# javad-jahangiri-iau/Detecting_Cyber_Attacks_with_Distilled_Large_Language_Models_in_Distributed_Networks

Measured on AMD Instinct MI355X. Metric: batches/sec/client (DistilBERT seq128 bs32) + aggregated F1 after 1 FedAvg round, 1/2/4/8 MI355X, higher is better.
Workload: dtype bf16; 1 GPU; model=DistilBERT-base (6 layers) + Linear(768,2) DDoSClassifier, global_batch=32, seq_len=128, parallelism=fedavg1 (1 client/GPU)

## Files before the change

### csrc/binding.cpp

```cpp
#ifdef FD_HOST_VALIDATION
#include <ATen/ATen.h>
typedef struct ihipStream_t* hipStream_t;
namespace py { struct gil_scoped_release {}; }
#else
#include <torch/extension.h>
#include <c10/hip/HIPStream.h>
#include <hip/hip_runtime.h>
#endif

#include <cmath>
#include <cstdint>
#include <vector>

#include "kernels/adam_epi.h"

extern "C" {
int fd_gemm(int kind, int epi, const void* A, const void* B, void* C, int M, int N, int K, int lda, int ldb,
            int ldc, const float* bias, void* aux, int ldaux, const void* res, int ldres, float* workspace,
            long long workspace_elems, int accumulate, const FdAdamEpi* adam,
            float* colsum, int* colsum_blocks, hipStream_t st);
int fd_gemm_ex(int kind, int epi, const void* A, const void* B, void* C, int M, int N, int K, int lda, int ldb,
               int ldc, const float* bias, void* aux, int ldaux, const void* res, int ldres, float* workspace,
               long long workspace_elems, int accumulate, const FdAdamEpi* adam,
               float* colsum, int* colsum_blocks, void* aux_out, hipStream_t st);
int fd_gemm_set_cfg(int kind, int cfg, int splits);
int fd_gemm_pf(const void* pf, long long bytes);
int fd_gemm_stamps(unsigned long long* host, int nblocks);
int fd_attn_stamps(unsigned long long* host, int nblocks);
int fd_attn_set_split(int on);
int fd_gemm_dw2(const void* A0, const void* B0, float* C0, int M0, int N0, const void* A1, const void* B1, float* C1,
                int M1, int N1, int K, float* workspace, long long workspace_elems, int accumulate,
                const FdAdamEpi* adams, int defer, int* splits_out, hipStream_t st);
int fd_gemm_dw2_splits(int M0, int N0, int M1, int N1, int K);
int fd_gemm_dw_batch(int n, const FdDwProb* probs, int K, const int* step, const float* hyper, int cfg,
                     const FdAdamRest* rest, hipStream_t st);
int fd_gemm_ln_set_diag(int diag);
int fd_gemm_dwb_set_mix(int mode);
long long fd_gemm_dwb_mixed_launches();
int fd_gemm_splitk(int epi, const void* A, const void* Bt, int M, int N, int K, float* workspace,
                   long long workspace_elems, int splits, const float* bias, void* C, void* aux, void* aux_out,
                   const void* res, float* colsum, int* colsum_blocks, const FdLnEpi* ln, const FdSkHead* hd,
                   int b_mn, hipStream_t st);
int fd_gemm_ln(int bwd, const void* A, const void* Bt, void* C, int M, int N, int K, const float* bias,
               const void* res, int ldres, const FdLnEpi* ln, int cfg, int b_mn, hipStream_t st);
int fd_splitk_reduce_batched(int n, const float* const* slabs, float* const* outs, const long long* numel,
                             const int* splits, const int* accumulate, hipStream_t st);

const char* fd_comm_last_error();
int fd_comm_load(const char* path);
int fd_comm_unique_id_bytes();
int fd_comm_get_unique_id(void* out);
int fd_comm_init(void** comm, int nranks, int rank, const void* id_bytes);
int fd_comm_destroy(void* comm);
int fd_comm_async_error(void* comm);
int fd_comm_wait(void* comm, hipStream_t st, long long timeout_ms);
int fd_comm_abort(void* comm);
int fd_comm_allreduce(void* comm, const void* send, void* recv, long long count, int dtype, int op, hipStream_t st);
int fd_comm_broadcast(void* comm, void* buf, long long count, int dtype, int root, hipStream_t st);
int fd_comm_allgather(void* comm, const void* send, void* recv, long long count, int dtype, hipStream_t st);
int fd_gemm_attn_fwd(const void* x, const void* w, const float* bias, void* qkv, int M, int K, const float* kbias,
                     void* ctx, float* lse, int B, int S, int H, const uint32_t* seed_ptr, uint32_t site, uint32_t thr,
                     float drop_scale, const int* cu, int rows, uint64_t* dmask, int q_live, void* cxc, void* xc,
                     const void* xres, int Bp, uint64_t* flags, int nflags, const int* cnt, int xsite, int* err,
                     int mode, int split, hipStream_t st);
int fd_attn_bwd_proj(const void* qkv, const float* kbias, const void* ctx, const float* lse, const void* dy,
                     const void* w, int M, int K, int splits, void* dqkv, int B, int S, int H,
                     const uint32_t* seed_ptr, uint32_t site, uint32_t thr, float drop_scale, const int* cu, int rows,
                     const uint64_t* dmask, const void* dresc, void* dres, int split, hipStream_t st);
int fd_attn_fwd(const void* qkv, const float* kbias, void* ctx, float* lse, int B, int S, int H,
                const uint32_t* seed_ptr, uint32_t site, uint32_t thr, float drop_scale, const int* cu,
                int rows, uint64_t* dmask, int q_live, void* cxc, void* xc, const void* xres, int Bp,
                int split, hipStream_t st);
int fd_attn_bwd(const void* qkv, const float* kbias, const void* ctx, const float* lse, const void* dctx,
                float* delta, void* dqkv, int B, int S, int H, const uint32_t* seed_ptr, uint32_t site,
                uint32_t thr, float drop_scale, const int* cu, int rows, const uint64_t* dmask, int q_live,
                const void* dresc, void* dres, int split, hipStream_t st);
int fd_mask_to_bias(const void* mask, int mask_bytes, float* bias, long n, hipStream_t st);
int fd_ln_fwd(const void* x, const void* r, const float* gamma, const float* beta, void* y, float* mean,
              float* rstd, int T, int D, float eps, const uint32_t* seed_ptr, uint32_t site, uint32_t thr,
              float dscale, const int* row_map, hipStream_t st);
int fd_ln_bwd(const void* dy, const void* x, const void* r, const float* gamma, const float* mean,
              const float* rstd, void* dz, void* dx, float* dgamma, float* dbeta, float* dbias, float* work, int T,
              int D, const uint32_t* seed_ptr, uint32_t site, uint32_t thr, float dscale, int accumulate,
              const int* row_map, int defer, int* nblk_out, int zin, hipStream_t st);
int fd_emb_fwd(const void* ids, int ids64, const void* word, const void* pos, const float* gamma,
               const float* beta, void* y, float* mean, float* rstd, int T, int S, int D, float eps,
               const uint32_t* seed_ptr, uint32_t site, uint32_t thr, float dscale, const int* row_map, int* ln_epoch,
               unsigned long long* ln_stats, long long ln_stats_n, long long* sorted, long long* perm, hipStream_t st);
int fd_emb_bwd(const void* dy, const void* ids, int ids64, const long long* sorted, const long long* perm,
               const void* word, const void* pos, const float* gamma, const float* mean, const float* rstd,
               float* dword, float* dpos, float* dgamma, float* dbeta, float* dz_buf, float* work, int T, int S,
               int B, int P, int V, int D, const uint32_t* seed_ptr, uint32_t site, uint32_t thr, float dscale,
               int accumulate, unsigned char* now, unsigned char* ever, const int* row_map, const int* cu, int ncs, const float* const* cs_parts, float* const* cs_outs, const int* cs_nblk,
               const int* cs_stride, const int* cs_D, const int* cs_nout, const int* cs_acc, hipStream_t st);
int fd_gather_rows2(const void* a, const void* b, void* oa, void* ob, const long long* idx, int n, int d_bytes,
                    hipStream_t st);
int fd_scatter_rows2(const void* a, const void* b, void* oa, void* ob, const long long* idx, int nsrc, int T,
                     int d_bytes, hipStream_t st);
int fd_pack(const void* mask, int mask_bytes, const void* ids, int ids_bytes, int B, int S, int rows, int* row_map,
            int* cu, long long* ids_packed, int* step, uint32_t* seed, long long* cls_rows, int* cls_rmap,
            hipStream_t st);
int fd_colsum_bf16_batched(int n, const void* const* xs, const int* T, const int* N, float* const* parts,
                           hipStream_t st);
int fd_colsum_bf16(const void* x, int T, int N, float* out, float* work, int accumulate, int defer, int* nblk_out,
                   hipStream_t st);
int fd_colsum_batched(int n, const float* const* parts, float* const* outs, const int* nblk, const int* stride,
                      const int* D, const int* nout, const int* accumulate, hipStream_t st);
int fd_rank_sort(const void* ids, int ids64, int T, long long* sorted, long long* perm, hipStream_t st);
int fd_head_fwd(const void* hidden, int B, int S, int D, const float* W, const float* bias,
                const uint32_t* seed_ptr, uint32_t site, uint32_t thr, float dscale, const long long* labels,
                float* logits, float* loss, float* dlogits, float* row_loss, const int* cls, int T,
                const float* tlogits, float kd_T, float kd_alpha, float* loss_acc, hipStream_t st);
int fd_head_bwd(const void* hidden, int B, int S, int D, const float* W, const uint32_t* seed_ptr, uint32_t site,
                uint32_t thr, float dscale, const float* dlogits, float* dW, float* db, void* dhidden,
                int accumulate, const int* cls, int T, const float* gscale, const int* own, hipStream_t st);
int fd_head_ln_bwd(const void* hidden, int B, int T, int D, const float* W, const float* bias,
                   const uint32_t* seed_ptr, uint32_t hsite, uint32_t hthr, float hdscale, const long long* labels,
                   float* logits, float* loss, float* dlogits, float* row_loss, float* loss_acc, float* dW, float* db,
                   int accumulate, const int* own, const float* tlogits, float kd_T, float kd_alpha, const void* z,
                   const float* gamma, const float* mean, const float* rstd, void* dz, void* dx, float* part,
                   uint32_t site, uint32_t thr, float dscale, const int* row_map, int* nblk_out, hipStream_t st);
int fd_eval_metrics(const float* logits, const long long* labels, int B, double* acc, long long* counts,
                    float* prob1, long long* preds, hipStream_t st);
int fd_adam(float* p, const float* g, float* m, float* v, void* shadow, long long n, const int* step, float lr,
            float b1, float b2, float eps, float wd, int decoupled, const unsigned char* touched,
            const unsigned char* now, long long skip_off, long long skip_rows, int row_len, const long long* runs,
            int nruns, long long run_total4, const float* run_wd, hipStream_t st);
int fd_adam_rows(float* p, const float* g, float* m, float* v, void* shadow, int rows, int row_len, const int* step,
                 float lr, float b1, float b2, float eps, const unsigned char* ever, const unsigned char* now,
                 float wd, int decoupled, hipStream_t st);
int fd_adam_lazy_decay(float* p, void* shadow, int* done, const unsigned char* ever, int rows, int row_len,
                       const int* step, int adj, float lr, float wd, const void* ids, int ids64, long long n,
                       hipStream_t st);
int fd_step(int* step, uint32_t* seed, hipStream_t st);
int fd_scale_cast(float* p, void* shadow, long long n, float scale, hipStream_t st);
int fd_axpby(float* dst, const float* x, const float* y, float a, float b, long long n, hipStream_t st);
}

namespace {

#ifdef FD_HOST_VALIDATION
hipStream_t stream() { return nullptr; }
bool on_device(const at::Tensor&) { return true; }
#else
hipStream_t stream() { return c10::hip::getCurrentHIPStream().stream(); }
bool on_device(const at::Tensor& t) { return t.is_cuda(); }
#endif

void check_rc(int rc, const char* what) { TORCH_CHECK(rc == 0, what, ": kernel launcher rejected arguments (rc=", rc, ")"); }

void need(const at::Tensor& t, at::ScalarType dt, const char* name) {
  TORCH_CHECK(on_device(t), name, " must be a GPU tensor");
  TORCH_CHECK(t.scalar_type() == dt, name, " has dtype ", t.scalar_type(), ", expected ", dt);
  TORCH_CHECK(t.is_contiguous(), name, " must be contiguous");
}
void need_opt(const c10::optional<at::Tensor>& t, at::ScalarType dt, const char* name) {
  if (t.has_value() && t->defined()) need(*t, dt, name);
}
template <typename T>
T* ptr(const c10::optional<at::Tensor>& t) {
  return (t.has_value() && t->defined()) ? reinterpret_cast<T*>(t->data_ptr()) : nullptr;
}
const uint32_t* seedp(const at::Tensor& s) {
  TORCH_CHECK(on_device(s) && s.scalar_type() == at::kInt && s.numel() >= 1, "seed must be a GPU int32 tensor");
  return reinterpret_cast<const uint32_t*>(s.data_ptr());
}

void set_prefetch(const c10::optional<at::Tensor>& prefetch, const at::Tensor& like) {
  if (prefetch.has_value() && prefetch->defined() && prefetch->numel() > 0) {
    TORCH_CHECK(prefetch->device() == like.device() && prefetch->is_contiguous(),
                "prefetch must be a contiguous tensor on the GEMM's device");
    fd_gemm_pf(prefetch->data_ptr(), (long long)(prefetch->numel() * prefetch->element_size()));
  } else {
    fd_gemm_pf(nullptr, 0);
  }
}

void gemm(int64_t kind, int64_t epi, const at::Tensor& A, const at::Tensor& B, const at::Tensor& C,
          const c10::optional<at::Tensor>& bias, const c10::optional<at::Tensor>& aux,
          const c10::optional<at::Tensor>& res, const c10::optional<at::Tensor>& workspace, bool accumulate,
          const c10::optional<at::Tensor>& aux_out, const c10::optional<at::Tensor>& prefetch = c10::nullopt) {
  need(A, at::kBFloat16, "A");
  need(B, at::kBFloat16, "B");
  TORCH_CHECK(A.dim() == 2 && B.dim() == 2 && C.dim() == 2, "gemm operands must be 2-D");
  int64_t M, N, K;
  if (kind == 0) { M = A.size(0); K = A.size(1); N = B.size(0); TORCH_CHECK(B.size(1) == K, "NT: K mismatch"); }
  else if (kind == 1) { M = A.size(0); K = A.size(1); N = B.size(1); TORCH_CHECK(B.size(0) == K, "NN: K mismatch"); }
  else if (kind == 2) { K = A.size(0); M = A.size(1); N = B.size(1); TORCH_CHECK(B.size(0) == K, "TN: K mismatch"); }
  else TORCH_CHECK(false, "bad gemm kind");
  TORCH_CHECK(C.size(0) == M && C.size(1) == N, "C shape mismatch: got ", C.sizes(), " want [", M, ",", N, "]");
  TORCH_CHECK(K % 64 == 0, "gemm: K must be a multiple of 64, got ", K);
  TORCH_CHECK(N % 64 == 0, "gemm: N must be a multiple of 64, got ", N);
  if (kind == 2) {
    need(C, at::kFloat, "C");
    TORCH_CHECK(M % 128 == 0, "TN gemm: M must be a multiple of 128");
  } else {
    need(C, at::kBFloat16, "C");
  }
  need_opt(bias, at::kFloat, "bias");
  need_opt(aux, at::kBFloat16, "aux");
  need_opt(res, at::kBFloat16, "res");
  need_opt(workspace, at::kFloat, "workspace");
  if (epi == 1 || epi == 2) TORCH_CHECK(bias.has_value() && bias->numel() == N, "bias of size N required");
  if (epi == 3 || (epi == 2 && aux.has_value() && aux->defined()))
    TORCH_CHECK(aux.has_value() && aux->size(0) == M && aux->size(1) == N, "aux [M,N] required");
  if (epi == 4) TORCH_CHECK(res.has_value() && res->size(0) == M && res->size(1) == N, "res [M,N] required");
  need_opt(aux_out, at::kBFloat16, "aux_out");
  if (aux_out.has_value() && aux_out->defined())
    TORCH_CHECK(epi == 3 && kind != 2 && aux_out->size(0) == M && aux_out->size(1) == N,
                "aux_out [M,N] only with the GELU' epilogue");
  const long long ws = (workspace.has_value() && workspace->defined()) ? workspace->numel() : 0;
  set_prefetch(prefetch, A);
  check_rc(fd_gemm_ex((int)kind, (int)epi, A.data_ptr(), B.data_ptr(), C.data_ptr(), (int)M, (int)N, (int)K,
                      (int)A.size(1), (int)B.size(1), (int)N, ptr<float>(bias), ptr<void>(aux), (int)N,
                      ptr<void>(res), (int)N, ptr<float>(workspace), ws, accumulate ? 1 : 0, nullptr, nullptr,
                      nullptr, ptr<void>(aux_out), stream()),
           "gemm");
}

int64_t gemm_colsum(int64_t epi, const at::Tensor& A, const at::Tensor& B, const at::Tensor& C,
                    const c10::optional<at::Tensor>& aux, const c10::optional<at::Tensor>& res,
                    const at::Tensor& colsum, const c10::optional<at::Tensor>& aux_out, int64_t kind = 0,
                    const c10::optional<at::Tensor>& prefetch = c10::nullopt) {
  need(A, at::kBFloat16, "A");
  need(B, at::kBFloat16, "B");
  need(C, at::kBFloat16, "C");
  need(colsum, at::kFloat, "colsum");
  TORCH_CHECK(A.dim() == 2 && B.dim() == 2 && C.dim() == 2, "gemm_colsum operands must be 2-D");
  TORCH_CHECK(kind == 0 || kind == 1, "gemm_colsum: kind 0 (NT) or 1 (NN)");
  const int64_t M = A.size(0), K = A.size(1), N = kind == 0 ? B.size(0) : B.size(1);
  TORCH_CHECK((kind == 0 ? B.size(1) : B.size(0)) == K && C.size(0) == M && C.size(1) == N,
              "gemm_colsum: shape mismatch");
  TORCH_CHECK(K % 64 == 0 && N % 64 == 0, "gemm_colsum: K % 64 and N % 64 required");
  TORCH_CHECK(epi == 3 || epi == 4, "gemm_colsum: GELU' (3) or residual (4) epilogue");
  need_opt(aux, at::kBFloat16, "aux");
  need_opt(res, at::kBFloat16, "res");
  if (epi == 3) TORCH_CHECK(aux.has_value() && aux->size(0) == M && aux->size(1) == N, "aux [M,N] required");
  if (epi == 4) TORCH_CHECK(res.has_value() && res->size(0) == M && res->size(1) == N, "res [M,N] required");
  TORCH_CHECK(colsum.numel() >= ((M + 127) / 128) * N, "gemm_colsum: colsum needs ceil(M/128) x N floats");
  need_opt(aux_out, at::kBFloat16, "aux_out");
  if (aux_out.has_value() && aux_out->defined())
    TORCH_CHECK(epi == 3 && aux_out->size(0) == M && aux_out->size(1) == N, "aux_out [M,N] only with GELU'");
  int blocks = 0;
  set_prefetch(prefetch, A);
  check_rc(fd_gemm_ex((int)kind, (int)epi, A.data_ptr(), B.data_ptr(), C.data_ptr(), (int)M, (int)N, (int)K,
                      (int)K, (int)B.size(1), (int)N, nullptr, ptr<void>(aux), (int)N, ptr<void>(res), (int)N,
                      nullptr, 0, 0, nullptr, colsum.data_ptr<float>(), &blocks, ptr<void>(aux_out), stream()),
           "gemm_colsum");
  return blocks;
}

void adam_descs(const std::vector<at::Tensor>& st, const std::vector<double>& hp, const at::Tensor* const* grads,
                int nprob, FdAdamEpi* out) {
  TORCH_CHECK((int)st.size() == 4 * nprob + 1, "fused adam: expected ", 4 * nprob + 1, " state tensors");
// ... 288 lines not shown
                                 const c10::optional<at::Tensor>& gamma, const c10::optional<at::Tensor>& beta,
                                 const c10::optional<at::Tensor>& mean, const c10::optional<at::Tensor>& rstd,
                                 const c10::optional<at::Tensor>& z, const c10::optional<at::Tensor>& dx,
                                 const c10::optional<at::Tensor>& colpart, double eps,
                                 const c10::optional<at::Tensor>& seed, int64_t site, int64_t thr, double dscale,
                                 const c10::optional<at::Tensor>& row_map, bool b_mn = false,
                                 const std::vector<at::Tensor>& head = {}, const std::vector<double>& head_f = {},
                                 const c10::optional<at::Tensor>& head_dx = c10::nullopt,
                                 const c10::optional<at::Tensor>& head_tlogits = c10::nullopt,
                                 const c10::optional<at::Tensor>& head_own = c10::nullopt) {
  need(A, at::kBFloat16, "A");
  need(Bt, at::kBFloat16, "Bt");
  need(C, at::kBFloat16, "C");
  need(workspace, at::kFloat, "workspace");
  TORCH_CHECK(A.dim() == 2 && Bt.dim() == 2 && C.dim() == 2, "gemm_splitk operands must be 2-D");
  const int64_t M = A.size(0), K = A.size(1), N = b_mn ? Bt.size(1) : Bt.size(0);
  TORCH_CHECK(M > 0 && (b_mn ? Bt.size(0) : Bt.size(1)) == K && C.size(0) == M && C.size(1) == N,
              "gemm_splitk: shape mismatch");
  TORCH_CHECK(K % 64 == 0 && N % 64 == 0, "gemm_splitk: K % 64 and N % 64 required");
  TORCH_CHECK(epi >= 0 && epi <= 7 && epi != 5, "gemm_splitk: epilogue code");
  for (const auto* t : {&aux, &aux_out, &res, &z, &dx}) {
    need_opt(*t, at::kBFloat16, "gemm_splitk bf16 operand");
    if (t->has_value() && (*t)->defined())
      TORCH_CHECK((*t)->dim() == 2 && (*t)->size(0) == M && (*t)->size(1) == N, "gemm_splitk: [M, N] operand");
  }
  for (const auto* t : {&bias, &gamma, &beta}) {
    need_opt(*t, at::kFloat, "gemm_splitk fp32 vector");
    if (t->has_value() && (*t)->defined()) TORCH_CHECK((*t)->numel() == N, "gemm_splitk: vector of size N");
  }
  need_opt(mean, at::kFloat, "mean");
  need_opt(rstd, at::kFloat, "rstd");
  need_opt(colsum, at::kFloat, "colsum");
  need_opt(colpart, at::kFloat, "colpart");
  need_opt(row_map, at::kInt, "row_map");
  auto has = [](const c10::optional<at::Tensor>& t) { return t.has_value() && t->defined(); };
  if (epi == 1 || epi == 2 || epi == 6) TORCH_CHECK(has(bias), "gemm_splitk: bias required");
  if (epi == 2 || epi == 3) TORCH_CHECK(has(aux), "gemm_splitk: aux [M, N] required");
  if (epi == 4 || epi >= 6) TORCH_CHECK(has(res), "gemm_splitk: res [M, N] required");
  if (has(colsum)) {
    TORCH_CHECK(epi == 3 || epi == 4, "gemm_splitk: column sums only with the GELU' / residual epilogues");
    TORCH_CHECK(colsum->numel() >= ((M + 31) / 32) * N, "gemm_splitk: colsum needs ceil(M/32) x N floats");
  }
  FdLnEpi ln{};
  if (epi >= 6) {
    TORCH_CHECK(has(gamma) && has(mean) && has(rstd) && mean->numel() >= M && rstd->numel() >= M,
                "gemm_splitk LayerNorm: gamma, mean / rstd of M entries required");
    if (epi == 6) TORCH_CHECK(has(beta), "gemm_splitk LayerNorm forward: beta required");
    if (epi == 7) {
      TORCH_CHECK(has(z), "gemm_splitk LayerNorm backward: z required");
      TORCH_CHECK(has(colpart) && colpart->numel() >= M * 3 * N, "gemm_splitk LayerNorm backward: colpart M x 3N");
      if (thr) TORCH_CHECK(has(dx), "gemm_splitk LayerNorm backward with dropout: dx required");
    }
    ln.gamma = gamma->data_ptr<float>();
    ln.beta = ptr<float>(beta);
    ln.mean = mean->data_ptr<float>();
    ln.rstd = rstd->data_ptr<float>();
    ln.z = ptr<uint16_t>(z);
    ln.dx = ptr<uint16_t>(dx);
    ln.colpart = ptr<float>(colpart);
    ln.eps = (float)eps;
    ln.thr = (uint32_t)thr;
    ln.site = (uint32_t)site;
    ln.dscale = (float)dscale;
    if (thr) {
      TORCH_CHECK(seed.has_value() && seed->defined(), "gemm_splitk: dropout needs the seed tensor");
      ln.seed_ptr = seedp(*seed);
      ln.row_map = ptr<int>(row_map);
      if (has(row_map)) TORCH_CHECK(row_map->numel() >= M, "gemm_splitk: row_map needs M entries");
    }
  }
  FdSkHead hd{};
  if (!head.empty()) {
    TORCH_CHECK(epi == 6 && N == 768 && head.size() == 13 && head_f.size() == 6, "gemm_splitk head: arguments");
    need(head[11], at::kFloat, "head loss");
    need(head[12], at::kInt, "head ticket");
    TORCH_CHECK(head[11].numel() == 1 && head[12].numel() == 1, "gemm_splitk head: loss / ticket [1]");
    const int64_t Bh = (int64_t)head_f[5];
    TORCH_CHECK(Bh > 0 && Bh <= M, "gemm_splitk head: B");
    need(head[0], at::kFloat, "head W");
    need(head[1], at::kFloat, "head bias");
    need(head[2], at::kLong, "head labels");
    for (int k : {3, 4, 6, 7, 8, 9}) need(head[k], at::kFloat, "head fp32 output");
    need(head[5], at::kBFloat16, "head dz");
    TORCH_CHECK(head[0].numel() == 2 * N && head[1].numel() == 2 && head[2].numel() == Bh &&
                    head[3].numel() == 2 * Bh && head[4].numel() == 2 * Bh && head[5].numel() == M * N &&
                    head[6].numel() >= M * 3 * N && head[7].numel() >= M * 2 * N && head[8].numel() >= M * 2 &&
                    head[9].numel() >= M,
                "gemm_splitk head: sizes");
    need_opt(head_dx, at::kBFloat16, "head dx");
    need_opt(head_tlogits, at::kFloat, "head teacher logits");
    need_opt(head_own, at::kInt, "head own");
    if (thr) TORCH_CHECK(head_dx.has_value() && head_dx->defined() && head_dx->numel() == M * N, "gemm_splitk head: dx");
    if (head_tlogits.has_value() && head_tlogits->defined())
      TORCH_CHECK(head_tlogits->numel() == 2 * Bh && head_f[3] > 0.0, "gemm_splitk head: teacher logits [B, 2], T > 0");
    if (head_own.has_value() && head_own->defined()) TORCH_CHECK(head_own->numel() == Bh + 1, "gemm_splitk head: own");
    hd.W = head[0].data_ptr<float>();
    hd.bias = head[1].data_ptr<float>();
    hd.labels = reinterpret_cast<const long long*>(head[2].data_ptr());
    hd.logits = head[3].data_ptr<float>();
    hd.dlogits = head[4].data_ptr<float>();
    hd.dz = reinterpret_cast<uint16_t*>(head[5].data_ptr());
    hd.colpart = head[6].data_ptr<float>();
    hd.hpart = head[7].data_ptr<float>();
    hd.dbpart = head[8].data_ptr<float>();
    hd.lpart = head[9].data_ptr<float>();
    hd.seed_ptr = seedp(head[10]);
    hd.loss = head[11].data_ptr<float>();
    hd.ticket = reinterpret_cast<unsigned*>(head[12].data_ptr<int>());
    hd.site = (uint32_t)head_f[0];
    hd.thr = (uint32_t)head_f[1];
    hd.dscale = (float)head_f[2];
    hd.kd_T = (float)head_f[3];
    hd.kd_alpha = (float)head_f[4];
    hd.B = (int)Bh;
    hd.dx = ptr<uint16_t>(head_dx);
    hd.tlogits = ptr<const float>(head_tlogits);
    hd.own = ptr<int>(head_own);
  }
  int blocks = 0;
  const int rc = fd_gemm_splitk((int)epi, A.data_ptr(), Bt.data_ptr(), (int)M, (int)N, (int)K,
                                workspace.data_ptr<float>(), workspace.numel(), (int)splits, ptr<float>(bias),
                                C.data_ptr(), ptr<void>(aux), ptr<void>(aux_out), ptr<void>(res), ptr<float>(colsum),
                                &blocks, epi >= 6 ? &ln : nullptr, head.empty() ? nullptr : &hd, b_mn ? 1 : 0,
                                stream());
  TORCH_CHECK(rc > 0, "gemm_splitk: launcher rejected arguments (rc=", rc, ")");
  return {rc, blocks};
}

void splitk_reduce_batched(const std::vector<at::Tensor>& slabs, const std::vector<at::Tensor>& outs,
                           const std::vector<int64_t>& splits, const std::vector<int64_t>& accumulate) {
  const size_t n = slabs.size();
  TORCH_CHECK(outs.size() == n && splits.size() == n && accumulate.size() == n, "splitk_reduce_batched: ragged");
  std::vector<const float*> sp(n);
  std::vector<float*> op(n);
  std::vector<long long> ne(n);
  std::vector<int> sl(n), ac(n);
  for (size_t i = 0; i < n; ++i) {
    need(slabs[i], at::kFloat, "slabs");
    need(outs[i], at::kFloat, "out");
    TORCH_CHECK(splits[i] >= 1 && outs[i].numel() % 4 == 0 && slabs[i].numel() >= splits[i] * outs[i].numel(),
                "splitk_reduce_batched: slab buffer smaller than splits x out");
    sp[i] = slabs[i].data_ptr<float>();
    op[i] = outs[i].data_ptr<float>();
    ne[i] = outs[i].numel();
    sl[i] = (int)splits[i];
    ac[i] = accumulate[i] ? 1 : 0;
  }
  if (n) check_rc(fd_splitk_reduce_batched((int)n, sp.data(), op.data(), ne.data(), sl.data(), ac.data(), stream()),
                  "splitk_reduce_batched");
}

void pack(const at::Tensor& mask, const at::Tensor& ids, const at::Tensor& row_map, const at::Tensor& cu,
          const at::Tensor& ids_packed, const c10::optional<at::Tensor>& step, const c10::optional<at::Tensor>& seed,
          const c10::optional<at::Tensor>& cls_rows, const c10::optional<at::Tensor>& cls_rmap) {
  need_opt(cls_rmap, at::kInt, "cls_rmap");
  need_opt(step, at::kInt, "step");
  need_opt(seed, at::kInt, "seed");
  need_opt(cls_rows, at::kLong, "cls_rows");
  TORCH_CHECK(on_device(mask) && mask.is_contiguous() && on_device(ids) && ids.is_contiguous(), "pack: GPU inputs");
  TORCH_CHECK(mask.dim() == 2 && ids.sizes() == mask.sizes(), "pack: mask and ids must both be [B, S]");
  need(row_map, at::kInt, "row_map");
  need(cu, at::kInt, "cu");
  need(ids_packed, at::kLong, "ids_packed");
  const int64_t B = mask.size(0), S = mask.size(1);
  TORCH_CHECK(cu.numel() == B + 1 && ids_packed.numel() == row_map.numel() && row_map.numel() >= 1, "pack: sizes");
  if (cls_rows.has_value() && cls_rows->defined()) TORCH_CHECK(cls_rows->numel() >= B, "pack: cls_rows needs B entries");
  if (cls_rmap.has_value() && cls_rmap->defined()) TORCH_CHECK(cls_rmap->numel() >= B, "pack: cls_rmap needs B entries");
  check_rc(fd_pack(mask.data_ptr(), (int)mask.element_size(), ids.data_ptr(), (int)ids.element_size(), (int)B, (int)S,
                   (int)row_map.numel(), row_map.data_ptr<int>(), cu.data_ptr<int>(),
                   reinterpret_cast<long long*>(ids_packed.data_ptr()), ptr<int>(step), ptr<uint32_t>(seed),
                   cls_rows.has_value() && cls_rows->defined() ? reinterpret_cast<long long*>(cls_rows->data_ptr())
                                                               : nullptr,
                   ptr<int>(cls_rmap), stream()),
           "pack");
}

void gather_rows2(const at::Tensor& a, const at::Tensor& b, const at::Tensor& oa, const at::Tensor& ob,
                  const at::Tensor& idx) {
  for (const at::Tensor* t : {&a, &b, &oa, &ob}) need(*t, at::kBFloat16, "gather_rows2 operand");
  need(idx, at::kLong, "idx");
  TORCH_CHECK(a.dim() == 2 && a.sizes() == b.sizes() && oa.dim() == 2 && oa.sizes() == ob.sizes() &&
                  oa.size(1) == a.size(1) && oa.size(0) == idx.numel(), "gather_rows2: shapes");
  TORCH_CHECK((a.size(1) * 2) % 16 == 0, "gather_rows2: rows must be 16-byte multiples");
  check_rc(fd_gather_rows2(a.data_ptr(), b.data_ptr(), oa.data_ptr(), ob.data_ptr(),
                           reinterpret_cast<const long long*>(idx.data_ptr()), (int)idx.numel(), (int)(a.size(1) * 2),
                           stream()), "gather_rows2");
}

void scatter_rows2(const at::Tensor& a, const at::Tensor& b, const at::Tensor& oa, const at::Tensor& ob,
                   const at::Tensor& idx, int64_t nsrc) {
  for (const at::Tensor* t : {&a, &b, &oa, &ob}) need(*t, at::kBFloat16, "scatter_rows2 operand");
  need(idx, at::kLong, "idx");
  TORCH_CHECK(a.dim() == 2 && a.sizes() == b.sizes() && oa.dim() == 2 && oa.sizes() == ob.sizes() &&
                  oa.size(1) == a.size(1) && nsrc >= 0 && nsrc <= a.size(0) && nsrc <= idx.numel(),
              "scatter_rows2: shapes");
  TORCH_CHECK((a.size(1) * 2) % 16 == 0, "scatter_rows2: rows must be 16-byte multiples");
  check_rc(fd_scatter_rows2(a.data_ptr(), b.data_ptr(), oa.data_ptr(), ob.data_ptr(),
                            reinterpret_cast<const long long*>(idx.data_ptr()), (int)nsrc, (int)oa.size(0),
                            (int)(a.size(1) * 2), stream()), "scatter_rows2");
}

int comm_dtype(const at::Tensor& t) {
  switch (t.scalar_type()) {
    case at::kFloat: return 0;
    case at::kBFloat16: return 1;
    case at::kDouble: return 2;
    case at::kLong: return 3;
    case at::kInt: return 4;
    default: TORCH_CHECK(false, "comm: unsupported dtype ", t.scalar_type());
  }
  return 0;
}
void comm_check(int rc, const char* what) { TORCH_CHECK(rc == 0, what, " failed: ", fd_comm_last_error()); }

void comm_load(const std::string& path) { comm_check(fd_comm_load(path.c_str()), "comm_load"); }

at::Tensor comm_unique_id() {
  at::Tensor id = at::empty({fd_comm_unique_id_bytes()}, at::TensorOptions().dtype(at::kByte));
  comm_check(fd_comm_get_unique_id(id.data_ptr()), "ncclGetUniqueId");
  return id;
}
int64_t comm_init(int64_t nranks, int64_t rank, const at::Tensor& id) {
  TORCH_CHECK(!id.is_cuda() && id.scalar_type() == at::kByte && id.numel() == fd_comm_unique_id_bytes(),
              "comm_init: id must be the CPU uint8 tensor from comm_unique_id()");
  TORCH_CHECK(rank >= 0 && rank < nranks, "comm_init: bad rank");
  void* c = nullptr;
  comm_check(fd_comm_init(&c, (int)nranks, (int)rank, id.contiguous().data_ptr()), "ncclCommInitRank");
  return reinterpret_cast<int64_t>(c);
}
void comm_destroy(int64_t h) { comm_check(fd_comm_destroy(reinterpret_cast<void*>(h)), "ncclCommDestroy"); }
void comm_abort(int64_t h) { comm_check(fd_comm_abort(reinterpret_cast<void*>(h)), "ncclCommAbort"); }
std::tuple<int64_t, std::string> comm_async_error(int64_t h) {
  const int rc = fd_comm_async_error(reinterpret_cast<void*>(h));
  return {rc, rc ? std::string(fd_comm_last_error()) : std::string()};
}
std::tuple<int64_t, std::string> comm_wait(int64_t h, int64_t timeout_ms) {
  TORCH_CHECK(h != 0, "comm_wait: communicator not initialised");
  const hipStream_t st = stream();
  int rc;
  {
    py::gil_scoped_release nogil;
    rc = fd_comm_wait(reinterpret_cast<void*>(h), st, (long long)timeout_ms);
  }
  return {rc, rc ? std::string(fd_comm_last_error()) : std::string()};
}
void comm_allreduce(int64_t h, const at::Tensor& t, int64_t op) {
  TORCH_CHECK(h != 0, "comm_allreduce: communicator not initialised");
  TORCH_CHECK(on_device(t) && t.is_contiguous(), "comm_allreduce: contiguous GPU tensor required");
  TORCH_CHECK(op >= 0 && op <= 2, "comm_allreduce: op must be 0 (sum), 1 (avg) or 2 (max)");
  comm_check(fd_comm_allreduce(reinterpret_cast<void*>(h), t.data_ptr(), t.data_ptr(), t.numel(), comm_dtype(t),
                               (int)op, stream()),
             "ncclAllReduce");
}
void comm_broadcast(int64_t h, const at::Tensor& t, int64_t root) {
  TORCH_CHECK(h != 0, "comm_broadcast: communicator not initialised");
  TORCH_CHECK(on_device(t) && t.is_contiguous(), "comm_broadcast: contiguous GPU tensor required");
  comm_check(fd_comm_broadcast(reinterpret_cast<void*>(h), t.data_ptr(), t.numel(), comm_dtype(t), (int)root,
                               stream()),
             "ncclBroadcast");
}
void comm_allgather(int64_t h, const at::Tensor& send, const at::Tensor& recv) {
  TORCH_CHECK(h != 0, "comm_allgather: communicator not initialised");
  TORCH_CHECK(on_device(send) && on_device(recv) && send.is_contiguous() && recv.is_contiguous(),
              "comm_allgather: contiguous GPU tensors required");
  TORCH_CHECK(send.scalar_type() == recv.scalar_type() && recv.numel() % send.numel() == 0,
              "comm_allgather: recv must hold nranks x send");
  comm_check(fd_comm_allgather(reinterpret_cast<void*>(h), send.data_ptr(), recv.data_ptr(), send.numel(),
                               comm_dtype(send), stream()),
             "ncclAllGather");
}


int64_t gemm_stamps(at::Tensor out) {
  TORCH_CHECK(!out.is_cuda() && out.scalar_type() == at::kLong && out.is_contiguous() && out.dim() == 2 &&
                  out.size(1) == 8, "gemm_stamps: CPU int64 [n][8]");
  return fd_gemm_stamps(reinterpret_cast<unsigned long long*>(out.data_ptr()), (int)out.size(0));
}

int64_t attn_stamps(at::Tensor out) {
  TORCH_CHECK(!out.is_cuda() && out.scalar_type() == at::kLong && out.is_contiguous() && out.dim() == 2 &&
                  out.size(1) == 8, "attn_stamps: CPU int64 [n][8]");
  return fd_attn_stamps(reinterpret_cast<unsigned long long*>(out.data_ptr()), (int)out.size(0));
}

void gemm_set_cfg(int64_t kind, int64_t cfg, int64_t splits) {
  check_rc(fd_gemm_set_cfg((int)kind, (int)cfg, (int)splits), "gemm_set_cfg");
}

void check_cu(const c10::optional<at::Tensor>& cu, int64_t B, int64_t rows_qkv, int64_t rows_ctx) {
  if (!(cu.has_value() && cu->defined())) return;
  need(*cu, at::kInt, "cu");
  TORCH_CHECK(cu->numel() == B + 1, "attention: cu must have B+1 entries");
  TORCH_CHECK(rows_qkv >= 1 && rows_qkv == rows_ctx, "attention: packed qkv/ctx row counts differ");
}

const int* map_ptr(const c10::optional<at::Tensor>& m, int64_t T) {
  if (!(m.has_value() && m->defined())) return nullptr;
  need(*m, at::kInt, "row_map");
  TORCH_CHECK(m->numel() == T, "row_map must have one entry per row");
  return m->data_ptr<int>();
}

void check_dmask(const c10::optional<at::Tensor>& dmask, int64_t B, int64_t S, int64_t H, int64_t split = -1) {
  if (!dmask.has_value() || !dmask->defined()) return;
  need(*dmask, at::kLong, "dmask");
  TORCH_CHECK((S <= 128 || split == 2) && dmask->numel() == B * H * 256,
              "attention: dmask needs S <= 128 (or split 2) and B*H*256 words");
}

void attn_fwd(const at::Tensor& qkv, const at::Tensor& kbias, const at::Tensor& ctx, const at::Tensor& lse,
              int64_t B, int64_t S, int64_t H, const at::Tensor& seed, int64_t site, int64_t thr, double dscale,
              const c10::optional<at::Tensor>& cu, const c10::optional<at::Tensor>& dmask, int64_t q_live = 0,
              const c10::optional<at::Tensor>& cxc = c10::nullopt, const c10::optional<at::Tensor>& xc = c10::nullopt,
              const c10::optional<at::Tensor>& xres = c10::nullopt, int64_t split = -1) {
  need(qkv, at::kBFloat16, "qkv");
  TORCH_CHECK(q_live >= 0, "attention: q_live >= 0");
  TORCH_CHECK(split >= -1 && split <= 2, "attention: split in -1..2");
  const bool compact = cxc.has_value() && cxc->defined();
  int64_t Bp = 0;
  if (compact) {
    TORCH_CHECK(q_live == 1 && xc.has_value() && xres.has_value(), "attention: compact rows need q_live 1, xc, xres");
    need(*cxc, at::kBFloat16, "cxc");
    need(*xc, at::kBFloat16, "xc");
    need(*xres, at::kBFloat16, "xres");
    Bp = cxc->numel() / (H * 64);
    TORCH_CHECK(Bp >= B && cxc->numel() == Bp * H * 64 && xc->numel() == cxc->numel(), "attention: cxc/xc size");
    TORCH_CHECK(xres->numel() == ctx.numel(), "attention: xres size");
// ... 599 lines not shown
    TORCH_CHECK(!(touched.has_value() && touched->defined()), "adam: per-run decay takes no row flags");
    need_decays(run_wd_host, (size_t)nruns, "adam run_wd");
    rwd = run_wd->data_ptr<float>();
  } else {
    TORCH_CHECK(run_wd_host.empty(), "adam: run_wd_host without run_wd");
  }
  if (touched.has_value() && touched->defined())
    TORCH_CHECK(wd == 0.0 || decoupled, "adam: row flags with weight decay need decoupled decay");
  check_rc(fd_adam(p.data_ptr<float>(), g.data_ptr<float>(), m.data_ptr<float>(), v.data_ptr<float>(),
                   ptr<void>(shadow), n, step.data_ptr<int>(), (float)lr, (float)b1, (float)b2, (float)eps, (float)wd,
                   decoupled ? 1 : 0, ptr<const unsigned char>(touched), ptr<const unsigned char>(now), skip_off,
                   skip_rows, (int)row_len, rp, nruns, total4, rwd, stream()),
           "adam");
}

void adam_rows(const at::Tensor& p, const at::Tensor& g, const at::Tensor& m, const at::Tensor& v,
               const c10::optional<at::Tensor>& shadow, const at::Tensor& step, double lr, double b1, double b2,
               double eps, const at::Tensor& ever, const c10::optional<at::Tensor>& now, int64_t row_len,
               double wd = 0.0, bool decoupled = false) {
  TORCH_CHECK(std::isfinite(wd) && wd >= 0.0, "adam_rows: weight decay must be finite and >= 0");
  TORCH_CHECK(wd == 0.0 || decoupled, "adam_rows: weight decay needs decoupled decay");
  need(p, at::kFloat, "p");
  need(g, at::kFloat, "g");
  need(m, at::kFloat, "m");
  need(v, at::kFloat, "v");
  need_opt(shadow, at::kBFloat16, "shadow");
  need(step, at::kInt, "step");
  need(ever, at::kByte, "ever");
  need_opt(now, at::kByte, "now");
  const int64_t n = p.numel();
  TORCH_CHECK(row_len > 0 && row_len % 4 == 0 && n % row_len == 0, "adam_rows: rows of row_len (multiple of 4)");
  const int64_t rows = n / row_len;
  TORCH_CHECK(g.numel() == n && m.numel() == n && v.numel() == n, "adam_rows: sizes");
  if (shadow.has_value() && shadow->defined()) TORCH_CHECK(shadow->numel() == n, "adam_rows: shadow size");
  TORCH_CHECK(ever.numel() >= rows, "adam_rows: ever flags");
  if (now.has_value() && now->defined()) TORCH_CHECK(now->numel() >= rows, "adam_rows: now flags");
  check_rc(fd_adam_rows(p.data_ptr<float>(), g.data_ptr<float>(), m.data_ptr<float>(), v.data_ptr<float>(),
                        ptr<void>(shadow), (int)rows, (int)row_len, step.data_ptr<int>(), (float)lr, (float)b1,
                        (float)b2, (float)eps, ever.data_ptr<unsigned char>(), ptr<const unsigned char>(now),
                        (float)wd, decoupled ? 1 : 0, stream()),
           "adam_rows");
}

void adam_lazy_decay(const at::Tensor& p, const c10::optional<at::Tensor>& shadow, const at::Tensor& done,
                     const at::Tensor& ever, const at::Tensor& step, int64_t adj, double lr, double wd,
                     int64_t row_len, const c10::optional<at::Tensor>& ids) {
  need(p, at::kFloat, "p");
  need_opt(shadow, at::kBFloat16, "shadow");
  need(done, at::kInt, "done");
  need(ever, at::kByte, "ever");
  need(step, at::kInt, "step");
  TORCH_CHECK(std::isfinite(wd) && wd >= 0.0 && std::isfinite(lr), "adam_lazy_decay: lr / weight decay");
  TORCH_CHECK(adj == 0 || adj == 1, "adam_lazy_decay: adj is 0 or 1");
  const int64_t n = p.numel();
  TORCH_CHECK(row_len > 0 && row_len % 4 == 0 && n > 0 && n % row_len == 0,
              "adam_lazy_decay: rows of row_len (multiple of 4)");
  const int64_t rows = n / row_len;
  TORCH_CHECK(rows < (int64_t(1) << 31), "adam_lazy_decay: too many rows");
  if (shadow.has_value() && shadow->defined()) TORCH_CHECK(shadow->numel() == n, "adam_lazy_decay: shadow size");
  TORCH_CHECK(done.numel() >= rows && ever.numel() >= rows && step.numel() >= 1, "adam_lazy_decay: flag sizes");
  const void* idp = nullptr;
  int ids64 = 0;
  int64_t nids = 0;
  if (ids.has_value() && ids->defined()) {
    TORCH_CHECK(ids->scalar_type() == at::kLong || ids->scalar_type() == at::kInt, "adam_lazy_decay: ids int32 / int64");
    need(*ids, ids->scalar_type(), "ids");
    nids = ids->numel();
    TORCH_CHECK(nids > 0 && nids <= (int64_t(1) << 30), "adam_lazy_decay: ids count");
    idp = ids->data_ptr();
    ids64 = ids->scalar_type() == at::kLong;
  }
  check_rc(fd_adam_lazy_decay(p.data_ptr<float>(), ptr<void>(shadow), done.data_ptr<int>(),
                              ever.data_ptr<unsigned char>(), (int)rows, (int)row_len, step.data_ptr<int>(), (int)adj,
                              (float)lr, (float)wd, idp, ids64, nids, stream()),
           "adam_lazy_decay");
}

void step_inc(const c10::optional<at::Tensor>& step, const c10::optional<at::Tensor>& seed) {
  need_opt(step, at::kInt, "step");
  need_opt(seed, at::kInt, "seed");
  check_rc(fd_step(ptr<int>(step), ptr<uint32_t>(seed), stream()), "step");
}

void scale_cast(const at::Tensor& p, const c10::optional<at::Tensor>& shadow, double scale) {
  need(p, at::kFloat, "p");
  need_opt(shadow, at::kBFloat16, "shadow");
  TORCH_CHECK(p.numel() % 4 == 0, "scale_cast: numel % 4");
  if (shadow.has_value() && shadow->defined()) TORCH_CHECK(shadow->numel() == p.numel(), "scale_cast: shadow size");
  check_rc(fd_scale_cast(p.data_ptr<float>(), ptr<void>(shadow), p.numel(), (float)scale, stream()), "scale_cast");
}

void axpby(const at::Tensor& dst, const at::Tensor& x, const c10::optional<at::Tensor>& y, double a, double b) {
  need(dst, at::kFloat, "dst");
  need(x, at::kFloat, "x");
  need_opt(y, at::kFloat, "y");
  TORCH_CHECK(dst.numel() == x.numel() && dst.numel() % 4 == 0, "axpby: sizes");
  if (y.has_value() && y->defined()) TORCH_CHECK(y->numel() == x.numel(), "axpby: y size");
  check_rc(fd_axpby(dst.data_ptr<float>(), x.data_ptr<float>(), ptr<const float>(y), (float)a, (float)b, dst.numel(),
                    stream()),
           "axpby");
}

}

#ifndef FD_HOST_VALIDATION
PYBIND11_MODULE(TORCH_EXTENSION_NAME, m) {
  m.doc() = "gfx950 HIP kernels for the federated DistilBERT engine";
  m.def("gemm", &gemm, py::arg("kind"), py::arg("epi"), py::arg("A"), py::arg("B"), py::arg("C"), py::arg("bias"),
        py::arg("aux"), py::arg("res"), py::arg("workspace"), py::arg("accumulate"), py::arg("aux_out") = py::none(),
        py::arg("prefetch") = py::none());
  m.def("gemm_set_cfg", &gemm_set_cfg);
  m.def("gemm_stamps", &gemm_stamps);
  m.def("attn_stamps", &attn_stamps);
  m.def("gemm_splitk", &gemm_splitk, py::arg("epi"), py::arg("A"), py::arg("Bt"), py::arg("C"), py::arg("workspace"),
        py::arg("splits") = 0, py::arg("bias") = py::none(), py::arg("aux") = py::none(),
        py::arg("aux_out") = py::none(), py::arg("res") = py::none(), py::arg("colsum") = py::none(),
        py::arg("gamma") = py::none(), py::arg("beta") = py::none(), py::arg("mean") = py::none(),
        py::arg("rstd") = py::none(), py::arg("z") = py::none(), py::arg("dx") = py::none(),
        py::arg("colpart") = py::none(), py::arg("eps") = 1e-12, py::arg("seed") = py::none(),
        py::arg("site") = 0, py::arg("thr") = 0, py::arg("dscale") = 1.0, py::arg("row_map") = py::none(),
        py::arg("b_mn") = false, py::arg("head") = std::vector<at::Tensor>{}, py::arg("head_f") = std::vector<double>{},
        py::arg("head_dx") = py::none(), py::arg("head_tlogits") = py::none(), py::arg("head_own") = py::none());
  m.def("gemm_dw2", &gemm_dw2);
  m.def("gemm_dw", &gemm_dw);
  m.def("adam_rows", &adam_rows, py::arg("p"), py::arg("g"), py::arg("m"), py::arg("v"), py::arg("shadow"),
        py::arg("step"), py::arg("lr"), py::arg("b1"), py::arg("b2"), py::arg("eps"), py::arg("ever"), py::arg("now"),
        py::arg("row_len"), py::arg("wd") = 0.0, py::arg("decoupled") = false);
  m.def("adam_lazy_decay", &adam_lazy_decay, py::arg("p"), py::arg("shadow"), py::arg("done"), py::arg("ever"),
        py::arg("step"), py::arg("adj"), py::arg("lr"), py::arg("wd"), py::arg("row_len"),
        py::arg("ids") = py::none());
  m.def("gemm_ln", &gemm_ln, py::arg("bwd"), py::arg("A"), py::arg("Bt"), py::arg("C"), py::arg("bias"),
        py::arg("res"), py::arg("gamma"), py::arg("beta"), py::arg("mean"), py::arg("rstd"), py::arg("z"),
        py::arg("dx"), py::arg("colpart"), py::arg("stats"), py::arg("cnt"), py::arg("err"), py::arg("eps"),
        py::arg("seed"), py::arg("site"), py::arg("thr"), py::arg("dscale"), py::arg("row_map"),
        py::arg("cfg") = -1, py::arg("xsite") = 0, py::arg("b_mn") = false, py::arg("xbuf") = py::none(),
        py::arg("prefetch") = py::none());
  m.def("gemm_dw_batch", &gemm_dw_batch, py::arg("As"), py::arg("Bs"), py::arg("Cs"), py::arg("accumulate"),
        py::arg("adam"), py::arg("hp"), py::arg("cfg") = -1,
        py::arg("biases") = std::vector<at::Tensor>{}, py::arg("rest") = std::vector<at::Tensor>{},
        py::arg("rest_i") = std::vector<int64_t>{}, py::arg("decay") = std::vector<double>{},
        py::arg("bias_decay") = std::vector<double>{}, py::arg("rest_wd") = py::none(),
        py::arg("rest_wd_host") = std::vector<double>{}, py::arg("word_wd") = 0.0);
  m.def("gemm_colsum", &gemm_colsum, py::arg("epi"), py::arg("A"), py::arg("B"), py::arg("C"), py::arg("aux"),
        py::arg("res"), py::arg("colsum"), py::arg("aux_out") = py::none(), py::arg("kind") = 0,
        py::arg("prefetch") = py::none());
  m.def("splitk_reduce_batched", &splitk_reduce_batched);
  m.def("gemm_dw2_splits", [](int64_t M0, int64_t N0, int64_t M1, int64_t N1, int64_t K) {
    return (int64_t)fd_gemm_dw2_splits((int)M0, (int)N0, (int)M1, (int)N1, (int)K);
  });
  m.def("gather_rows2", &gather_rows2);
  m.def("scatter_rows2", &scatter_rows2);
  m.def("pack", &pack, py::arg("mask"), py::arg("ids"), py::arg("row_map"), py::arg("cu"), py::arg("ids_packed"),
        py::arg("step") = py::none(), py::arg("seed") = py::none(), py::arg("cls_rows") = py::none(),
        py::arg("cls_rmap") = py::none());
  m.def("comm_load", &comm_load);
  m.def("comm_unique_id", &comm_unique_id);
  m.def("comm_init", &comm_init);
  m.def("comm_destroy", &comm_destroy);
  m.def("comm_abort", &comm_abort);
  m.def("comm_async_error", &comm_async_error);
  m.def("comm_wait", &comm_wait);
  m.def("comm_allreduce", &comm_allreduce);
  m.def("comm_broadcast", &comm_broadcast);
  m.def("comm_allgather", &comm_allgather);
  m.def("gemm_attn_fwd", &gemm_attn_fwd, py::arg("x"), py::arg("w"), py::arg("bias"), py::arg("qkv"),
        py::arg("kbias"), py::arg("ctx"), py::arg("lse"), py::arg("B"), py::arg("S"), py::arg("H"), py::arg("seed"),
        py::arg("site"), py::arg("thr"), py::arg("dscale"), py::arg("cu"), py::arg("dmask"), py::arg("q_live"),
        py::arg("stats"), py::arg("cnt"), py::arg("err"), py::arg("xsite"), py::arg("cxc") = py::none(),
        py::arg("xc") = py::none(), py::arg("xres") = py::none(), py::arg("prefetch") = py::none(),
        py::arg("mode") = 1, py::arg("split") = -1);
  m.def("attn_fwd", &attn_fwd, py::arg("qkv"), py::arg("kbias"), py::arg("ctx"), py::arg("lse"), py::arg("B"),
        py::arg("S"), py::arg("H"), py::arg("seed"), py::arg("site"), py::arg("thr"), py::arg("dscale"), py::arg("cu"),
        py::arg("dmask"), py::arg("q_live") = 0, py::arg("cxc") = py::none(), py::arg("xc") = py::none(),
        py::arg("xres") = py::none(), py::arg("split") = -1);
  m.def("attn_bwd", &attn_bwd, py::arg("qkv"), py::arg("kbias"), py::arg("ctx"), py::arg("lse"), py::arg("dctx"),
        py::arg("delta"), py::arg("dqkv"), py::arg("B"), py::arg("S"), py::arg("H"), py::arg("seed"), py::arg("site"),
        py::arg("thr"), py::arg("dscale"), py::arg("cu"), py::arg("dmask"), py::arg("q_live") = 0,
        py::arg("dresc") = py::none(), py::arg("dres") = py::none(), py::arg("split") = -1);
  m.def("attn_bwd_proj", &attn_bwd_proj, py::arg("qkv"), py::arg("kbias"), py::arg("ctx"), py::arg("lse"),
        py::arg("dy"), py::arg("w"), py::arg("dqkv"), py::arg("B"), py::arg("S"), py::arg("H"), py::arg("seed"),
        py::arg("site"), py::arg("thr"), py::arg("dscale"), py::arg("cu"), py::arg("dmask"), py::arg("splits") = 1,
        py::arg("dresc") = py::none(), py::arg("dres") = py::none(), py::arg("split") = -1);
  m.def("mask_to_bias", &mask_to_bias);
  m.def("attn_set_split", [](int64_t on) { return (int64_t)fd_attn_set_split((int)on); });
  m.def("ln_fwd", &ln_fwd);
  m.def("ln_bwd", &ln_bwd);
  m.def("emb_fwd", &emb_fwd, py::arg("ids"), py::arg("word"), py::arg("pos"), py::arg("gamma"), py::arg("beta"),
        py::arg("y"), py::arg("mean"), py::arg("rstd"), py::arg("S"), py::arg("eps"), py::arg("seed"), py::arg("site"),
        py::arg("thr"), py::arg("dscale"), py::arg("row_map") = py::none(), py::arg("ln_epoch") = py::none(),
        py::arg("sorted") = py::none(), py::arg("perm") = py::none(), py::arg("ln_stats") = py::none());
  m.def("gemm_ln_set_diag", [](int64_t d) { fd_gemm_ln_set_diag((int)d); });
  m.def("gemm_dwb_set_mix", [](int64_t mode) { return (int64_t)fd_gemm_dwb_set_mix((int)mode); },
        "all-layer dW launch schedule: 0 plain, 1 mixed tiles when shorter (default), 2 forced; returns the old mode");
  m.def("gemm_dwb_mixed_launches", []() { return (int64_t)fd_gemm_dwb_mixed_launches(); });
  m.def("emb_bwd", &emb_bwd);
  m.def("colsum_bf16", &colsum_bf16);
  m.def("colsum_bf16_batched", &colsum_bf16_batched);
  m.def("colsum_batched", &colsum_batched);
  m.def("rank_sort", &rank_sort);
  m.def("head_fwd", &head_fwd, py::arg("hidden"), py::arg("B"), py::arg("S"), py::arg("W"), py::arg("bias"),
        py::arg("seed"), py::arg("site"), py::arg("thr"), py::arg("dscale"), py::arg("labels"), py::arg("logits"),
        py::arg("loss"), py::arg("dlogits"), py::arg("row_loss"), py::arg("cls"), py::arg("tlogits") = py::none(),
        py::arg("kd_T") = 1.0, py::arg("kd_alpha") = 1.0, py::arg("loss_acc") = py::none());
  m.def("head_bwd", &head_bwd, py::arg("hidden"), py::arg("B"), py::arg("S"), py::arg("W"), py::arg("seed"),
        py::arg("site"), py::arg("thr"), py::arg("dscale"), py::arg("dlogits"), py::arg("dW"), py::arg("db"),
        py::arg("dhidden"), py::arg("accumulate"), py::arg("cls") = py::none(), py::arg("gscale") = py::none(),
        py::arg("own") = py::none());
  m.def("head_ln_bwd", &head_ln_bwd);
  m.def("eval_metrics", &eval_metrics);
  m.def("adam", &adam);
  m.def("step_inc", &step_inc);
  m.def("scale_cast", &scale_cast);
  m.def("axpby", &axpby);
}
#endif
```

### csrc/host_check/binding_host_check.cpp

```cpp
#define FD_HOST_VALIDATION 1
#include <algorithm>
#include "../binding.cpp"

#include <cstdio>
#include <cstdlib>
#include <string>
#include <vector>

namespace hc {
struct Region { uintptr_t lo, hi; };
std::vector<Region> regions;
std::vector<std::string> violations;
int calls = 0;

void reg(const at::Tensor& t) {
  const uintptr_t p = reinterpret_cast<uintptr_t>(t.data_ptr());
  regions.push_back({p, p + (uintptr_t)(t.numel() * t.element_size())});
}
void span(const void* p, long long bytes, const char* what) {
  if (bytes <= 0) return;
  if (!p) { violations.push_back(std::string("null ") + what); return; }
  const uintptr_t lo = reinterpret_cast<uintptr_t>(p), hi = lo + (uintptr_t)bytes;
  for (const Region& r : regions)
    if (lo >= r.lo && hi <= r.hi) return;
// ... 284 lines not shown
  const long long D = (long long)H * 64, N = 3 * D;
  hc::span(x, (long long)M * K * 2, "gemm_attn x");
  hc::span(w, N * K * 2, "gemm_attn w");
  hc::span(bias, N * 4, "gemm_attn bias");
  hc::span(qkv, (long long)M * N * 2, "gemm_attn qkv");
  const long long tiles = ((M + 127) / 128) * (N / 192);
  if (tiles > nflags) hc::violations.push_back("gemm_attn: more tiles than flags");
  hc::span(flags, tiles * 8, "gemm_attn flags");
  hc::span(cnt, 4, "gemm_attn cnt");
  hc::span(err, 4, "gemm_attn err");
  hc::opt_span(cxc, (long long)Bp * D * 2, "gemm_attn cxc");
  hc::opt_span(xc, (long long)Bp * D * 2, "gemm_attn xc");
  hc::opt_span(xres, rows * D * 2, "gemm_attn xres");
  hc::opt_span(dmask, (long long)B * H * 256 * 8, "gemm_attn dmask");
  hc::span(ctx, rows * D * 2, "gemm_attn ctx");
  hc::span(lse, (long long)B * H * S * 4, "gemm_attn lse");
  hc::span(seed, 4, "gemm_attn seed");
  if (cu) hc::span(cu, (long long)(B + 1) * 4, "gemm_attn cu");
  else hc::span(kbias, (long long)B * S * 4, "gemm_attn kbias");
  return 0;
}
int fd_attn_bwd_proj(const void* qkv, const float* kbias, const void* ctx, const float* lse, const void* dy,
                     const void* w, int M, int K, int, void* dqkv, int B, int S, int H, const uint32_t* seed,
                     uint32_t, uint32_t, float, const int* cu, int rows, const uint64_t* dmask, const void* dresc,
                     void* dres, int, hipStream_t) {
  ++hc::calls;
  const long long D = (long long)H * 64;
  hc::opt_span(dmask, (long long)B * H * 256 * 8, "attn bwd proj dmask");
  hc::span(qkv, rows * 3 * D * 2, "attn bwd proj qkv");
  hc::span(dqkv, rows * 3 * D * 2, "attn bwd proj dqkv");
  hc::span(ctx, rows * D * 2, "attn bwd proj ctx");
  hc::span(dy, (long long)M * K * 2, "attn bwd proj dy");
  hc::span(w, (long long)K * D * 2, "attn bwd proj w");
  hc::opt_span(dresc, (long long)M * D * 2, "attn bwd proj dresc");
  hc::opt_span(dres, rows * D * 2, "attn bwd proj dres");
  hc::span(lse, (long long)B * H * S * 4, "attn bwd proj lse");
  hc::span(seed, 4, "attn bwd proj seed");
  if (cu) hc::span(cu, (long long)(B + 1) * 4, "attn bwd proj cu");
  else hc::span(kbias, (long long)B * S * 4, "attn bwd proj kbias");
  return 0;
}
int fd_attn_bwd(const void* qkv, const float* kbias, const void* ctx, const float* lse, const void* dctx, float* delta,
                void* dqkv, int B, int S, int H, const uint32_t* seed, uint32_t, uint32_t, float, const int* cu,
                int rows, const uint64_t* dmask, int, const void* dresc, void* dres, int, hipStream_t) {
  ++hc::calls;
  const long long D = (long long)H * 64;
  hc::opt_span(dmask, (long long)B * H * 256 * 8, "attn bwd dmask");
  hc::span(qkv, rows * 3 * D * 2, "attn bwd qkv");
  hc::span(dqkv, rows * 3 * D * 2, "attn bwd dqkv");
  hc::span(ctx, rows * D * 2, "attn bwd ctx");
  hc::span(dctx, (dres ? B : rows) * D * 2, "attn bwd dctx");
  hc::opt_span(dresc, (long long)B * D * 2, "attn bwd dresc");
  hc::opt_span(dres, rows * D * 2, "attn bwd dres");
  hc::span(lse, (long long)B * H * S * 4, "attn bwd lse");
  hc::span(delta, (long long)B * H * S * 4, "attn bwd delta");
  hc::span(seed, 4, "attn bwd seed");
  if (cu) hc::span(cu, (long long)(B + 1) * 4, "attn bwd cu");
  else hc::span(kbias, (long long)B * S * 4, "attn bwd kbias");
  return 0;
}
int fd_mask_to_bias(const void*, int, float*, long, hipStream_t) { ++hc::calls; return 0; }
int fd_ln_fwd(const void* x, const void* r, const float* gamma, const float* beta, void* y, float* mean, float* rstd,
              int T, int D, float, const uint32_t* seed, uint32_t, uint32_t, float, const int* row_map, hipStream_t) {
  ++hc::calls;
  const long long n = (long long)T * D;
  hc::span(x, n * 2, "ln x");
  hc::opt_span(r, n * 2, "ln r");
  hc::span(y, n * 2, "ln y");
  hc::span(gamma, (long long)D * 4, "ln gamma");
  hc::span(beta, (long long)D * 4, "ln beta");
  hc::span(mean, (long long)T * 4, "ln mean");
  hc::span(rstd, (long long)T * 4, "ln rstd");
  hc::span(seed, 4, "ln seed");
  hc::opt_span(row_map, (long long)T * 4, "ln row_map");
  return 0;
}
int fd_ln_bwd(const void* dy, const void* x, const void* r, const float* gamma, const float* mean, const float* rstd,
              void* dz, void* dx, float* dgamma, float* dbeta, float* dbias, float* work, int T, int D,
              const uint32_t* seed, uint32_t, uint32_t, float, int, const int* row_map, int, int* nblk_out,
              int, hipStream_t) {
  ++hc::calls;
  const long long n = (long long)T * D;
  hc::span(dy, n * 2, "ln bwd dy");
  hc::span(x, n * 2, "ln bwd x");
  hc::opt_span(r, n * 2, "ln bwd r");
  hc::span(dz, n * 2, "ln bwd dz");
  hc::opt_span(dx, n * 2, "ln bwd dx");
  hc::span(gamma, (long long)D * 4, "ln bwd gamma");
  hc::span(mean, (long long)T * 4, "ln bwd mean");
  hc::span(rstd, (long long)T * 4, "ln bwd rstd");
  hc::opt_span(dgamma, (long long)D * 4, "ln bwd dgamma");
  hc::opt_span(dbeta, (long long)D * 4, "ln bwd dbeta");
  hc::opt_span(dbias, (long long)D * 4, "ln bwd dbias");
  const int blocks = std::min(512, (T + 7) / 8);
  hc::span(work, (long long)blocks * 3 * D * 4, "ln bwd work");
  hc::span(seed, 4, "ln bwd seed");
  hc::opt_span(row_map, (long long)T * 4, "ln bwd row_map");
  if (nblk_out) *nblk_out = blocks;
  return 0;
}
int fd_emb_fwd(const void*, int, const void*, const void*, const float*, const float*, void*, float*, float*, int, int,
               int, float, const uint32_t*, uint32_t, uint32_t, float, const int*, int* ln_epoch,
               unsigned long long* ln_stats, long long ln_stats_n, long long* sorted, long long* perm, hipStream_t) {
  ++hc::calls;
  hc::opt_span(ln_epoch, 4, "emb ln_epoch");
  hc::opt_span(ln_stats, ln_stats_n * 8, "emb ln_stats");
  if ((sorted == nullptr) != (perm == nullptr)) hc::violations.push_back("emb_fwd: sorted without perm");
  return 0;
}
int fd_emb_bwd(const void* dy, const void*, int, const long long* sorted, const long long* perm, const void*,
               const void*, const float*, const float*, const float*, float* dword, float* dpos, float*, float*,
               float* dz, float* work, int T, int, int, int P, int V, int D, const uint32_t*, uint32_t, uint32_t, float,
               int, unsigned char* now, unsigned char* ever, const int*, const int*, int ncs,
               const float* const* cs_parts, float* const* cs_outs, const int* cs_nblk, const int* cs_stride,
               const int* cs_D, const int* cs_nout, const int*, hipStream_t) {
  ++hc::calls;
  if (ncs < 0 || ncs > 32) hc::violations.push_back("emb_bwd: column-sum job count");
  for (int i = 0; i < ncs; ++i) {
    hc::span(cs_parts[i], (long long)cs_nblk[i] * cs_stride[i] * 4, "emb_bwd colsum part");
    for (int k = 0; k < cs_nout[i]; ++k) hc::opt_span(cs_outs[3 * i + k], (long long)cs_D[i] * 4, "emb_bwd colsum out");
  }
  hc::span(dy, (long long)T * D * 2, "emb_bwd dy");
  hc::span(sorted, (long long)T * 8, "emb_bwd sorted");
  hc::span(perm, (long long)T * 8, "emb_bwd perm");
  hc::span(dz, (long long)T * D * 4, "emb_bwd dz");
  hc::span(work, ((long long)T * D + (long long)std::min(256, (T + 7) / 8) * 3 * D) * 4, "emb_bwd work");
  hc::span(dword, (long long)V * D * 4, "emb_bwd dword");
  hc::span(dpos, (long long)P * D * 4, "emb_bwd dpos");
  hc::opt_span(now, V, "emb_bwd now");
  hc::opt_span(ever, V, "emb_bwd ever");
  return 0;
}
int fd_gather_rows2(const void* a, const void* b, void* oa, void* ob, const long long* idx, int n, int d_bytes,
                    hipStream_t) {
  ++hc::calls;
  hc::span(oa, (long long)n * d_bytes, "gather_rows2 oa");
  hc::span(ob, (long long)n * d_bytes, "gather_rows2 ob");
  hc::span(idx, (long long)n * 8, "gather_rows2 idx");
  (void)a; (void)b;
  return 0;
}
int fd_scatter_rows2(const void* a, const void* b, void* oa, void* ob, const long long* idx, int nsrc, int T,
                     int d_bytes, hipStream_t) {
  ++hc::calls;
  hc::span(a, (long long)nsrc * d_bytes, "scatter_rows2 a");
  hc::span(b, (long long)nsrc * d_bytes, "scatter_rows2 b");
  hc::span(oa, (long long)T * d_bytes, "scatter_rows2 oa");
  hc::span(ob, (long long)T * d_bytes, "scatter_rows2 ob");
  hc::span(idx, (long long)nsrc * 8, "scatter_rows2 idx");
  return 0;
}
int fd_pack(const void* mask, int mask_bytes, const void* ids, int ids_bytes, int B, int S, int rows, int* row_map,
            int* cu, long long* ids_packed, int* step, uint32_t* seed, long long* cls_rows, int* cls_rmap,
            hipStream_t) {
  hc::opt_span(cls_rmap, (long long)B * 4, "pack cls_rmap");
  ++hc::calls;
  hc::opt_span(cls_rows, (long long)B * 8, "pack cls_rows");
  hc::opt_span(step, 4, "pack step");
  hc::opt_span(seed, 4, "pack seed");
  hc::span(mask, (long long)B * S * mask_bytes, "pack mask");
  hc::span(ids, (long long)B * S * ids_bytes, "pack ids");
  hc::span(row_map, (long long)rows * 4, "pack row_map");
  hc::span(cu, (long long)(B + 1) * 4, "pack cu");
  hc::span(ids_packed, (long long)rows * 8, "pack ids_packed");
  return 0;
}
int fd_colsum_bf16(const void*, int, int, float*, float*, int, int, int* nblk_out, hipStream_t) {
  ++hc::calls;
  if (nblk_out) *nblk_out = 1;
  return 0;
}
int fd_colsum_bf16_batched(int n, const void* const* xs, const int* T, const int* N, float* const* parts,
                           hipStream_t) {
  ++hc::calls;
  for (int i = 0; i < n; ++i) {
    hc::span(xs[i], (long long)T[i] * N[i] * 2, "colsum_bf16_batched x");
    hc::span(parts[i], (long long)((T[i] + 31) / 32) * N[i] * 4, "colsum_bf16_batched part");
  }
  return 0;
}
int fd_colsum_batched(int, const float* const*, float* const*, const int*, const int*, const int*, const int*,
                      const int*, hipStream_t) { ++hc::calls; return 0; }
int fd_rank_sort(const void*, int, int, long long*, long long*, hipStream_t) { ++hc::calls; return 0; }
int fd_head_fwd(const void* hidden, int B, int S, int D, const float* W, const float* bias, const uint32_t* seed,
                uint32_t, uint32_t, float, const long long* labels, float* logits, float* loss, float* dlogits,
                float* row_loss, const int* cls, int T, const float* tlogits, float, float, float* loss_acc,
                hipStream_t) {
  ++hc::calls;
  hc::opt_span(loss_acc, 4, "head loss_acc");
  hc::span(hidden, (long long)T * D * 2, "head hidden");
  hc::span(W, 2LL * D * 4, "head W");
  hc::span(bias, 8, "head bias");
  hc::span(logits, 2LL * B * 4, "head logits");
  if (!cls && (long long)B * S > T) hc::violations.push_back("head: padded rows beyond hidden");
  hc::opt_span(cls, (long long)B * 4, "head cls");
  if (labels) {
    hc::span(labels, (long long)B * 8, "head labels");
    hc::span(loss, 4, "head loss");
    hc::span(dlogits, 2LL * B * 4, "head dlogits");
    hc::span(row_loss, (long long)B * 4, "head row_loss");
  }
  hc::opt_span(tlogits, 2LL * B * 4, "head teacher logits");
  hc::span(seed, 4, "head seed");
  return 0;
}
int fd_head_bwd(const void* hidden, int B, int S, int D, const float* W, const uint32_t* seed, uint32_t, uint32_t,
                float, const float* dlogits, float* dW, float* db, void* dhidden, int, const int* cls, int T,
                const float* gscale, const int* own, hipStream_t) {
  ++hc::calls;
  hc::opt_span(own, (B + 1LL) * 4, "head bwd own");
  hc::span(hidden, (long long)T * D * 2, "head bwd hidden");
  hc::span(dhidden, (long long)T * D * 2, "head bwd dhidden");
  hc::span(W, 2LL * D * 4, "head bwd W");
  hc::span(dlogits, 2LL * B * 4, "head bwd dlogits");
  hc::span(dW, 2LL * D * 4, "head bwd dW");
  hc::span(db, 8, "head bwd db");
  hc::opt_span(cls, (long long)B * 4, "head bwd cls");
  hc::opt_span(gscale, 4, "head bwd gscale");
  hc::span(seed, 4, "head bwd seed");
  (void)S;
  return 0;
}
int fd_head_ln_bwd(const void* hidden, int B, int T, int D, const float* W, const float* bias, const uint32_t* seed,
                   uint32_t, uint32_t, float, const long long* labels, float* logits, float* loss, float* dlogits,
                   float* row_loss, float* loss_acc, float* dW, float* db, int, const int* own, const float* tlogits,
                   float, float, const void* z, const float* gamma, const float* mean, const float* rstd, void* dz,
                   void* dx, float* part, uint32_t, uint32_t thr, float, const int* row_map, int* nblk_out,
                   hipStream_t) {
  ++hc::calls;
  const long long td = (long long)T * D;
  if (B > T) hc::violations.push_back("head_ln_bwd: B > T");
  hc::span(hidden, td * 2, "head_ln hidden");
  hc::span(W, 2LL * D * 4, "head_ln W");
  hc::span(bias, 8, "head_ln bias");
  hc::span(labels, (long long)B * 8, "head_ln labels");
  hc::span(logits, 2LL * B * 4, "head_ln logits");
  hc::span(loss, 4, "head_ln loss");
  hc::span(dlogits, 2LL * B * 4, "head_ln dlogits");
  hc::span(row_loss, (long long)B * 4, "head_ln row_loss");
  hc::opt_span(loss_acc, 4, "head_ln loss_acc");
  hc::span(dW, 2LL * D * 4, "head_ln dW");
  hc::span(db, 8, "head_ln db");
  hc::opt_span(own, (B + 1LL) * 4, "head_ln own");
  hc::opt_span(tlogits, 2LL * B * 4, "head_ln teacher logits");
  hc::span(z, td * 2, "head_ln z");
  hc::span(gamma, (long long)D * 4, "head_ln gamma");
  hc::span(mean, (long long)T * 4, "head_ln mean");
  hc::span(rstd, (long long)T * 4, "head_ln rstd");
  hc::span(dz, td * 2, "head_ln dz");
  if (thr) hc::span(dx, td * 2, "head_ln dx");
  const int nlb = (T + 15) / 16;
  hc::span(part, (long long)nlb * 3 * D * 4, "head_ln part");
  hc::opt_span(row_map, (long long)T * 4, "head_ln row_map");
  hc::span(seed, 4, "head_ln seed");
  if (nblk_out) *nblk_out = nlb;
  return 0;
}
int fd_eval_metrics(const float*, const long long*, int, double*, long long*, float*, long long*, hipStream_t) {
  ++hc::calls;
  return 0;
}
int fd_adam(float* p, const float* g, float* m, float* v, void* shadow, long long n, const int* step, float, float,
            float, float, float, int, const unsigned char* touched, const unsigned char* now, long long skip_off,
            long long skip_rows, int row_len, const long long* runs, int nruns, long long run_total4,
            const float* run_wd, hipStream_t) {
  ++hc::calls;
  if (run_wd) {
    if (!runs) hc::violations.push_back("adam: run decays without a run table");
    hc::span(run_wd, (long long)nruns * 4, "adam run decays");
  }
  hc::span(p, n * 4, "adam p");
  hc::span(g, n * 4, "adam g");
  hc::span(m, n * 4, "adam m");
  hc::span(v, n * 4, "adam v");
  hc::opt_span(shadow, n * 2, "adam shadow");
  hc::span(step, 4, "adam step");
  if (touched) {
    hc::span(touched, skip_rows, "adam touched");
    hc::opt_span(now, skip_rows, "adam now");
    if (skip_off < 0 || skip_off + skip_rows * row_len > n) hc::violations.push_back("adam: skip range");
  }
  if (runs) {
    hc::span(runs, (long long)nruns * 3 * 8, "adam runs");
    long long pre = 0;
    for (int i = 0; i < nruns; ++i) {
      const long long s4 = runs[3 * i], c4 = runs[3 * i + 1], p4 = runs[3 * i + 2];
      if (s4 < 0 || c4 <= 0 || (s4 + c4) * 4 > n) hc::violations.push_back("adam: run outside the arena");
      if (p4 != pre) hc::violations.push_back("adam: run prefix");
      pre += c4;
    }
    if (pre != run_total4) hc::violations.push_back("adam: run total");
  }
  return 0;
}
int fd_step(int*, uint32_t*, hipStream_t) { ++hc::calls; return 0; }
int fd_scale_cast(float*, void*, long long, float, hipStream_t) { ++hc::calls; return 0; }
int fd_axpby(float*, const float*, const float*, float, float, long long, hipStream_t) { ++hc::calls; return 0; }
}

namespace {
int failures = 0;

at::Tensor T_(at::IntArrayRef shape, at::ScalarType dt) {
  at::Tensor t = at::zeros(shape, at::TensorOptions().dtype(dt));
  hc::reg(t);
  return t;
}

template <typename F>
void expect_ok(const char* name, F f) {
  const size_t v0 = hc::violations.size();
  const int c0 = hc::calls;
  try {
    f();
  } catch (const c10::Error& e) {
    std::printf("FAIL %s: unexpected rejection: %s\n", name, e.what_without_backtrace());
    ++failures;
// ... 210 lines not shown
                                                        none, 0, stats, cnt, err, 127, none, none, none, none, 1); });
    expect_ok("attn bwd proj", [&] { attn_bwd_proj(qkv, kb, ctx, lse, x, T_({H * 64, H * 64}, bf), dqkv, B, S, H, seed, 16,
                                                  429496730, 1.1, none, dm); });
    expect_ok("attn bwd proj varlen", [&] { attn_bwd_proj(qv, kb, cv, lse, T_({300, H * 64}, bf), T_({H * 64, H * 64}, bf),
                                                         T_({300, 3 * H * 64}, bf), B, S, H, seed, 16, 0, 1.0, cu, none); });
    expect_reject("attn bwd proj S=256", [&] { attn_bwd_proj(qkv, kb, ctx, lse, x, T_({H * 64, H * 64}, bf), dqkv, 2, 256,
                                                            H, seed, 16, 0, 1.0, none, none); });
    expect_reject("attn bwd proj w shape", [&] { attn_bwd_proj(qkv, kb, ctx, lse, x, T_({H * 64, 64}, bf), dqkv, B, S, H,
                                                              seed, 16, 0, 1.0, none, none); });
    expect_reject("qkv attn mode", [&] { gemm_attn_fwd(x, w, bq, qkv, kb, ctx, lse, B, S, H, seed, 16, 0, 1.0, none,
                                                       none, 0, stats, cnt, err, 2, none, none, none, none, 3); });
  }
  {
    const int64_t Tn = 2688, D = 768;
    auto x = T_({Tn, D}, bf), r = T_({Tn, D}, bf), ga = T_({D}, f32), be = T_({D}, f32), y = T_({Tn, D}, bf);
    auto mean = T_({Tn}, f32), rstd = T_({Tn}, f32), seed = T_({1}, i32), rm = T_({Tn}, i32);
    expect_ok("ln fwd", [&] { ln_fwd(x, r, ga, be, y, mean, rstd, 1e-12, seed, 17, 429496730, 1.1, rm); });
    auto dz = T_({Tn, D}, bf), dx = T_({Tn, D}, bf), dg = T_({D}, f32), db = T_({D}, f32), dbias = T_({D}, f32);
    auto work = T_({336 * 3 * D}, f32);
    expect_ok("ln bwd", [&] { ln_bwd(x, x, r, ga, mean, rstd, dz, dx, dg, db, dbias, work, seed, 17, 429496730, 1.1,
                                     false, rm, true, false); });
    auto small = T_({100 * 3 * D}, f32);
    expect_reject("ln bwd work", [&] { ln_bwd(x, x, r, ga, mean, rstd, dz, dx, dg, db, dbias, small, seed, 17, 0, 1.0,
                                              false, none, false, false); });
    expect_reject("ln bwd dx with dropout", [&] { ln_bwd(x, x, r, ga, mean, rstd, dz, none, dg, db, dbias, work, seed,
                                                         17, 429496730, 1.1, false, none, false, false); });
    expect_ok("ln bwd from z", [&] { ln_bwd(x, x, none, ga, mean, rstd, dz, dx, dg, db, dbias, work, seed, 17, 429496730,
                                            1.1, false, rm, true, true); });
    expect_reject("ln bwd z + residual", [&] { ln_bwd(x, x, r, ga, mean, rstd, dz, dx, dg, db, dbias, work, seed, 17, 0,
                                                      1.0, false, none, false, true); });
    auto g2 = T_({1024}, f32);
    expect_reject("ln fwd D", [&] { ln_fwd(x, r, g2, g2, y, mean, rstd, 1e-12, seed, 17, 0, 1.0, none); });
    auto rm_bad = T_({10}, i32);
    expect_reject("ln fwd row_map", [&] { ln_fwd(x, r, ga, be, y, mean, rstd, 1e-12, seed, 17, 0, 1.0, rm_bad); });
    auto a = T_({Tn, 3072}, bf), wt = T_({D, 3072}, bf), bias = T_({D}, f32), z = T_({Tn, D}, bf);
    auto stats = T_({2 * (Tn + 128) * (D / 64)}, i64), cnt = T_({2}, i32), err = T_({1}, i32);
    auto cp = T_({((Tn + 63) / 64) * 3 * D}, f32);
    expect_ok("gemm_ln fwd", [&] { gemm_ln(false, a, wt, y, bias, r, ga, be, mean, rstd, z, none, none, stats, cnt, err,
                                           1e-12, seed, 17, 429496730, 1.1, rm, -1, 0); });
    expect_ok("gemm_ln bwd", [&] { gemm_ln(true, a, wt, dz, none, r, ga, none, mean, rstd, z, dx, cp, stats, cnt, err,
                                           1e-12, seed, 17, 429496730, 1.1, rm, -1, 0); });
    expect_reject("gemm_ln bwd without z", [&] { gemm_ln(true, a, wt, dz, none, r, ga, none, mean, rstd, none, dx, cp,
                                                         stats, cnt, err, 1e-12, seed, 17, 0, 1.0, none, -1, 0); });
    expect_reject("gemm_ln bwd dropout without dx", [&] {
      gemm_ln(true, a, wt, dz, none, r, ga, none, mean, rstd, z, none, cp, stats, cnt, err, 1e-12, seed, 17, 429496730,
              1.1, rm, -1, 0); });
    auto stats_small = T_({100}, i64);
    expect_reject("gemm_ln stats size", [&] { gemm_ln(false, a, wt, y, bias, r, ga, be, mean, rstd, z, none, none,
                                                      stats_small, cnt, err, 1e-12, seed, 17, 0, 1.0, none, -1, 0); });
    expect_reject("gemm_ln fwd without beta", [&] { gemm_ln(false, a, wt, y, bias, r, ga, none, mean, rstd, z, none,
                                                            none, stats, cnt, err, 1e-12, seed, 17, 0, 1.0, none, -1, 0); });
    expect_reject("gemm_ln xsite range", [&] { gemm_ln(false, a, wt, y, bias, r, ga, be, mean, rstd, z, none, none,
                                                       stats, cnt, err, 1e-12, seed, 17, 0, 1.0, none, -1, 128); });
    auto cp_small = T_({3 * D}, f32);
    expect_reject("gemm_ln colpart size", [&] { gemm_ln(true, a, wt, dz, none, r, ga, none, mean, rstd, z, dx, cp_small,
                                                        stats, cnt, err, 1e-12, seed, 17, 0, 1.0, none, -1, 0); });
  }
  {
    const int64_t B = 32, S = 128, D = 768;
    auto hid = T_({B * S, D}, bf), W = T_({2, D}, f32), bias = T_({2}, f32), seed = T_({1}, i32);
    auto lab = T_({B}, i64), logits = T_({B, 2}, f32), loss = T_({}, f32), dlog = T_({B, 2}, f32), rl = T_({B}, f32);
    auto tl = T_({B, 2}, f32);
    expect_ok("head fwd", [&] { head_fwd(hid, B, S, W, bias, seed, 2, 0, 1.0, lab, logits, loss, dlog, rl, none,
                                         none, 1.0, 1.0, none); });
    const c10::optional<at::Tensor> lacc = T_({1}, f32);
    expect_ok("head fwd loss_acc", [&] { head_fwd(hid, B, S, W, bias, seed, 2, 0, 1.0, lab, logits, loss, dlog, rl,
                                                  none, none, 1.0, 1.0, lacc); });
    expect_ok("head fwd kd", [&] { head_fwd(hid, B, S, W, bias, seed, 2, 0, 1.0, lab, logits, loss, dlog, rl, none, tl,
                                            2.0, 0.5, none); });
    expect_reject("head kd without labels", [&] { head_fwd(hid, B, S, W, bias, seed, 2, 0, 1.0, none, logits, none,
                                                           none, none, none, tl, 2.0, 0.5, none); });
    expect_reject("head kd T <= 0", [&] { head_fwd(hid, B, S, W, bias, seed, 2, 0, 1.0, lab, logits, loss, dlog, rl,
                                                   none, tl, 0.0, 0.5, none); });
    auto dW = T_({2, D}, f32), db = T_({2}, f32), dh = T_({B * S, D}, bf);
    expect_ok("head bwd", [&] { head_bwd(hid, B, S, W, seed, 2, 0, 1.0, dlog, dW, db, dh, false, none, none, none); });
    auto hid_small = T_({B * S - 1, D}, bf);
    expect_reject("head bwd hidden size", [&] { head_bwd(hid_small, B, S, W, seed, 2, 0, 1.0, dlog, dW, db, hid_small,
                                                         false, none, none, none); });
  }
  {
    const int64_t n = 4096;
    auto p = T_({n}, f32), g = T_({n}, f32), m = T_({n}, f32), v = T_({n}, f32), sh = T_({n}, bf), step = T_({1}, i32);
    auto runs = T_({2, 3}, i64);
    auto rp = runs.data_ptr<int64_t>();
    rp[0] = 0; rp[1] = 64; rp[2] = 0; rp[3] = 512; rp[4] = 256; rp[5] = 64;
    expect_ok("adam runs", [&] { adam(p, g, m, v, sh, step, 2e-5, 0.9, 0.999, 1e-8, 0, false, none, none, 0, 0, 4,
                                      runs, 320, 768); });
    expect_reject("adam run end outside", [&] { adam(p, g, m, v, sh, step, 2e-5, 0.9, 0.999, 1e-8, 0, false, none,
                                                     none, 0, 0, 4, runs, 320, 4096); });
    auto g_small = T_({n - 4}, f32);
    expect_reject("adam sizes", [&] { adam(p, g_small, m, v, sh, step, 2e-5, 0.9, 0.999, 1e-8, 0, false, none, none,
                                           0, 0, 4, none, 0, 0); });
    auto ever = T_({64}, at::kByte), now = T_({64}, at::kByte), ever_small = T_({10}, at::kByte);
    expect_ok("adam rows", [&] { adam_rows(p, g, m, v, sh, step, 2e-5, 0.9, 0.999, 1e-8, ever, now, 64); });
    expect_reject("adam rows flags", [&] { adam_rows(p, g, m, v, sh, step, 2e-5, 0.9, 0.999, 1e-8, ever_small, now,
                                                     64); });
    expect_reject("adam rows row_len", [&] { adam_rows(p, g, m, v, sh, step, 2e-5, 0.9, 0.999, 1e-8, ever, now, 6); });
    const c10::optional<at::Tensor> rwd = T_({2}, f32), rwd3 = T_({3}, f32);
    expect_ok("adam run decays", [&] { adam(p, g, m, v, sh, step, 2e-5, 0.9, 0.999, 1e-8, 0.01, true, none, none, 0, 0,
                                            4, runs, 320, 768, rwd, {0.01, 0.0}); });
    expect_reject("adam run decays length", [&] { adam(p, g, m, v, sh, step, 2e-5, 0.9, 0.999, 1e-8, 0.01, true, none,
                                                       none, 0, 0, 4, runs, 320, 768, rwd3, {0.01, 0.0, 0.0}); });
    expect_reject("adam run decays host length", [&] { adam(p, g, m, v, sh, step, 2e-5, 0.9, 0.999, 1e-8, 0.01, true,
                                                            none, none, 0, 0, 4, runs, 320, 768, rwd, {0.01}); });
    expect_reject("adam run decay negative", [&] { adam(p, g, m, v, sh, step, 2e-5, 0.9, 0.999, 1e-8, 0.01, true, none,
                                                        none, 0, 0, 4, runs, 320, 768, rwd, {0.01, -0.01}); });
    expect_reject("adam run decay NaN", [&] { adam(p, g, m, v, sh, step, 2e-5, 0.9, 0.999, 1e-8, 0.01, true, none, none,
                                                   0, 0, 4, runs, 320, 768, rwd, {0.01, std::nan("")}); });
    expect_reject("adam run decays without runs", [&] { adam(p, g, m, v, sh, step, 2e-5, 0.9, 0.999, 1e-8, 0.01, true,
                                                             none, none, 0, 0, 4, none, 0, 0, rwd, {0.01, 0.0}); });
    expect_reject("adam weight decay negative", [&] { adam(p, g, m, v, sh, step, 2e-5, 0.9, 0.999, 1e-8, -0.01, true,
                                                           none, none, 0, 0, 4, none, 0, 0); });
    expect_ok("adam rows decoupled decay", [&] { adam_rows(p, g, m, v, sh, step, 2e-5, 0.9, 0.999, 1e-8, ever, now, 64,
                                                           0.01, true); });
    expect_reject("adam rows coupled decay", [&] { adam_rows(p, g, m, v, sh, step, 2e-5, 0.9, 0.999, 1e-8, ever, now,
                                                             64, 0.01, false); });
    expect_ok("adam flags decoupled decay", [&] { adam(p, g, m, v, sh, step, 2e-5, 0.9, 0.999, 1e-8, 0.01, true, ever,
                                                       now, 0, 64, 64, none, 0, 0); });
    expect_reject("adam flags coupled decay", [&] { adam(p, g, m, v, sh, step, 2e-5, 0.9, 0.999, 1e-8, 0.01, false, ever,
                                                         now, 0, 64, 64, none, 0, 0); });
    auto done = T_({64}, i32), done_small = T_({10}, i32), ids = T_({4, 8}, i64), ids32 = T_({32}, i32);
    expect_ok("lazy decay all rows", [&] { adam_lazy_decay(p, sh, done, ever, step, 0, 2e-5, 0.01, 64, none); });
    expect_ok("lazy decay ids", [&] { adam_lazy_decay(p, sh, done, ever, step, 1, 2e-5, 0.01, 64, ids); });
    expect_ok("lazy decay int32 ids", [&] { adam_lazy_decay(p, none, done, ever, step, 0, 2e-5, 0.01, 64, ids32); });
    expect_reject("lazy decay counters", [&] { adam_lazy_decay(p, sh, done_small, ever, step, 0, 2e-5, 0.01, 64, none); });
    expect_reject("lazy decay flags", [&] { adam_lazy_decay(p, sh, done, ever_small, step, 0, 2e-5, 0.01, 64, none); });
    expect_reject("lazy decay row_len", [&] { adam_lazy_decay(p, sh, done, ever, step, 0, 2e-5, 0.01, 6, none); });
    expect_reject("lazy decay adj", [&] { adam_lazy_decay(p, sh, done, ever, step, 2, 2e-5, 0.01, 64, none); });
    expect_reject("lazy decay negative", [&] { adam_lazy_decay(p, sh, done, ever, step, 0, 2e-5, -0.01, 64, none); });
    expect_reject("lazy decay ids dtype", [&] { adam_lazy_decay(p, sh, done, ever, step, 0, 2e-5, 0.01, 64, g); });
  }
  {
    const int64_t Tn = 2688, D = 768, V = 1000, P = 512;
    auto dy = T_({Tn, D}, bf), ids = T_({Tn}, i64), srt = T_({Tn}, i64), prm = T_({Tn}, i64);
    auto word = T_({V, D}, bf), pos = T_({P, D}, bf), ga = T_({D}, f32), mean = T_({Tn}, f32), rstd = T_({Tn}, f32);
    auto dword = T_({V, D}, f32), dpos = T_({P, D}, f32), dg = T_({D}, f32), db = T_({D}, f32), dz = T_({Tn, D}, f32);
    auto work = T_({Tn * D + 256 * 3 * D}, f32), work_small = T_({Tn * D}, f32), seed = T_({1}, i32);
    expect_ok("emb bwd", [&] { emb_bwd(dy, ids, srt, prm, word, pos, ga, mean, rstd, dword, dpos, dg, db, dz, work,
                                       128, seed, 1, 0, 1.0, false, none, none, none, none); });
    expect_reject("emb bwd work", [&] { emb_bwd(dy, ids, srt, prm, word, pos, ga, mean, rstd, dword, dpos, dg, db, dz,
                                                work_small, 128, seed, 1, 0, 1.0, false, none, none, none, none); });
    auto part = T_({21 * 3 * D}, f32), part_small = T_({20 * 3 * D}, f32);
    std::vector<std::vector<c10::optional<at::Tensor>>> outs = {{dg, db, c10::optional<at::Tensor>(T_({D}, f32))}};
    expect_ok("emb bwd + colsum jobs", [&] { emb_bwd(dy, ids, srt, prm, word, pos, ga, mean, rstd, dword, dpos, dg, db,
                                                     dz, work, 128, seed, 1, 0, 1.0, false, none, none, none, none,
                                                     {part}, outs, {21}, {3 * D}, {D}, {0}); });
    expect_reject("emb bwd colsum part", [&] { emb_bwd(dy, ids, srt, prm, word, pos, ga, mean, rstd, dword, dpos, dg,
                                                       db, dz, work, 128, seed, 1, 0, 1.0, false, none, none, none,
                                                       none, {part_small}, outs, {21}, {3 * D}, {D}, {0}); });
  }
  {
    auto mask = T_({32, 128}, i64), ids = T_({32, 128}, i64), rm = T_({2688}, i32), cu = T_({33}, i32);
    auto ip = T_({2688}, i64);
    expect_ok("pack", [&] { pack(mask, ids, rm, cu, ip, none, none, none, none); });
    {
      auto ga = T_({300, 768}, bf), gb = T_({300, 768}, bf), go = T_({64, 768}, bf), go2 = T_({64, 768}, bf);
      auto gi = T_({64}, i64);
      expect_ok("gather_rows2", [&] { gather_rows2(ga, gb, go, go2, gi); });
      expect_ok("scatter_rows2", [&] { scatter_rows2(go, go2, ga, gb, gi, 32); });
      auto gbad = T_({63, 768}, bf);
      expect_reject("gather_rows2 shapes", [&] { gather_rows2(ga, gb, gbad, go2, gi); });
      expect_reject("scatter_rows2 nsrc", [&] { scatter_rows2(go, go2, ga, gb, gi, 65); });
    }
    auto st1 = T_({1}, i32);
    expect_ok("pack + counters", [&] { pack(mask, ids, rm, cu, ip, st1, st1, none, none); });
    auto stf = T_({1}, f32);
    expect_reject("pack counter dtype", [&] { pack(mask, ids, rm, cu, ip, stf, none, none, none); });
    auto cu_bad = T_({32}, i32);
    expect_reject("pack cu", [&] { pack(mask, ids, rm, cu_bad, ip, none, none, none, none); });
  }
  if (failures) {
    std::printf("binding host check: %d failure(s)\n", failures);
    return 1;
  }
  std::printf("binding host check: ok (%d launcher calls validated)\n", hc::calls);
  return 0;
}
```

### csrc/kernels/norm.hip

```cpp
#include "common.h"

#include <cstdlib>

namespace {

struct LnArgs {
  const bf16_t* x;
  const bf16_t* r;
  const float* gamma;
  const float* beta;
  bf16_t* y;
  float* mean;
  float* rstd;
  int T, D;
  float eps;
  const uint32_t* seed_ptr;
  uint32_t site, thr;
  float dscale;
  const bf16_t* dy;
  bf16_t* dz;
  bf16_t* dx;
  float* part;
  const int* row_map;
  int zin;
};

constexpr int HL = 32, CH = 3;

DEV float half_sum(float v) {
#pragma unroll
  for (int o = 16; o > 0; o >>= 1) v += __shfl_xor(v, o, 64);
  return v;
}
DEV void unpack8(const uint4& u, float (&f)[8]) {
  f[0] = lo_bf(u.x); f[1] = hi_bf(u.x); f[2] = lo_bf(u.y); f[3] = hi_bf(u.y);
  f[4] = lo_bf(u.z); f[5] = hi_bf(u.z); f[6] = lo_bf(u.w); f[7] = hi_bf(u.w);
}
DEV uint4 pack8(const float (&f)[8]) {
  return make_uint4(pack_bf2(f[0], f[1]), pack_bf2(f[2], f[3]), pack_bf2(f[4], f[5]), pack_bf2(f[6], f[7]));
}

DEV void ln_load_sum(const LnArgs& a, int row, int hl, bool drop, uint32_t seed, float (&z)[CH][8],
                     uint32_t& keep) {
#pragma clang fp contract(off)
  uint4 xv[CH], rv[CH];
#pragma unroll
  for (int c = 0; c < CH; ++c) {
    const size_t off = (size_t)row * a.D + 8 * (hl + HL * c);
    xv[c] = *reinterpret_cast<const uint4*>(a.x + off);
    if (a.r) rv[c] = *reinterpret_cast<const uint4*>(a.r + off);
  }
  keep = 0xffffffu;
  const size_t hrow = a.row_map ? (size_t)(unsigned)a.row_map[row] : (size_t)row;
#pragma unroll
  for (int c = 0; c < CH; ++c) {
    const size_t off = hrow * a.D + 8 * (hl + HL * c);
    unpack8(xv[c], z[c]);
    if (drop) {
      const uint32_t kb = drop_keep_bits<8>(seed, (uint32_t)off, a.thr);
#pragma unroll
      for (int e = 0; e < 8; ++e) {
        const bool k = (kb >> e) & 1u;
        if (!a.zin) z[c][e] = k ? z[c][e] * a.dscale : 0.f;
        if (!k) keep &= ~(1u << (8 * c + e));
      }
    }
    if (a.r) {
      float rr[8];
      unpack8(rv[c], rr);
#pragma unroll
      for (int e = 0; e < 8; ++e) z[c][e] += rr[e];
    }
  }
}

__global__ __launch_bounds__(256) void ln_fwd_kernel(LnArgs a) {
  const int lane = threadIdx.x & 63, hl = lane & (HL - 1);
  const int row = blockIdx.x * 8 + (threadIdx.x >> 5);
  if (row >= a.T) return;
  const bool drop = a.thr != 0;
  const uint32_t seed = drop ? hash32(a.seed_ptr[0], a.site) : 0u;
  float4 gb[CH][4];
#pragma unroll
  for (int c = 0; c < CH; ++c) {
    const int col = 8 * (hl + HL * c);
    gb[c][0] = *reinterpret_cast<const float4*>(a.gamma + col);
    gb[c][1] = *reinterpret_cast<const float4*>(a.gamma + col + 4);
    gb[c][2] = *reinterpret_cast<const float4*>(a.beta + col);
    gb[c][3] = *reinterpret_cast<const float4*>(a.beta + col + 4);
  }
  float z[CH][8];
  uint32_t keep;
  ln_load_sum(a, row, hl, drop, seed, z, keep);
  float s = 0.f;
#pragma unroll
  for (int c = 0; c < CH; ++c)
#pragma unroll
    for (int e = 0; e < 8; ++e) s += z[c][e];
  const float mean = half_sum(s) / a.D;
  float q = 0.f;
#pragma unroll
  for (int c = 0; c < CH; ++c)
#pragma unroll
    for (int e = 0; e < 8; ++e) { const float d = z[c][e] - mean; q += d * d; }
  const float rstd = rsqrtf(half_sum(q) / a.D + a.eps);
#pragma unroll
  for (int c = 0; c < CH; ++c) {
    const int col = 8 * (hl + HL * c);
    const float4 g0 = gb[c][0], g1 = gb[c][1], b0 = gb[c][2], b1 = gb[c][3];
    const float g[8] = {g0.x, g0.y, g0.z, g0.w, g1.x, g1.y, g1.z, g1.w};
    const float b[8] = {b0.x, b0.y, b0.z, b0.w, b1.x, b1.y, b1.z, b1.w};
    float y[8];
#pragma unroll
    for (int e = 0; e < 8; ++e) y[e] = (z[c][e] - mean) * rstd * g[e] + b[e];
    *reinterpret_cast<uint4*>(a.y + (size_t)row * a.D + col) = pack8(y);
  }
  if (hl == 0) { a.mean[row] = mean; a.rstd[row] = rstd; }
}

template <int NC>
DEV void block_colsum(float (&acc)[NC][4], float* lds, float* out, int D) {
  const int lane = threadIdx.x & 63, w = threadIdx.x >> 6, nw = blockDim.x >> 6;
#pragma unroll
  for (int c = 0; c < NC; ++c)
#pragma unroll
    for (int e = 0; e < 4; ++e) lds[w * D + 4 * (lane + 64 * c) + e] = acc[c][e];
  __syncthreads();
  for (int col = threadIdx.x; col < D; col += blockDim.x) {
    float s = 0.f;
    for (int i = 0; i < nw; ++i) s += lds[i * D + col];
    out[col] = s;
  }
  __syncthreads();
}

DEV void ln_bwd_row(const LnArgs& a, int row, int hl, bool drop, const float4 (&gm)[CH][2], const float (&dyv)[CH][8],
                    float (&xh)[CH][8], uint32_t keep, float mean, float rstd, float (&dg)[CH][8],
                    float (&db)[CH][8], float (&dbias)[CH][8]) {
#pragma clang fp contract(off)
  const int D = a.D;
  float gd[CH][8];
  float s1 = 0.f, s2 = 0.f;
#pragma unroll
  for (int c = 0; c < CH; ++c) {
    const float4 g0 = gm[c][0], g1 = gm[c][1];
    const float g[8] = {g0.x, g0.y, g0.z, g0.w, g1.x, g1.y, g1.z, g1.w};
#pragma unroll
    for (int e = 0; e < 8; ++e) {
      xh[c][e] = (xh[c][e] - mean) * rstd;
      gd[c][e] = g[e] * dyv[c][e];
      s1 += gd[c][e];
      s2 += gd[c][e] * xh[c][e];
    }
  }
  s1 = half_sum(s1) / D;
  s2 = half_sum(s2) / D;
#pragma unroll
  for (int c = 0; c < CH; ++c) {
    const size_t off = (size_t)row * D + 8 * (hl + HL * c);
    float dz[8], dx[8];
#pragma unroll
    for (int e = 0; e < 8; ++e) {
      dz[e] = rstd * (gd[c][e] - s1 - xh[c][e] * s2);
      dx[e] = ((keep >> (8 * c + e)) & 1u) ? dz[e] * (drop ? a.dscale : 1.f) : 0.f;
      dg[c][e] += dyv[c][e] * xh[c][e];
      db[c][e] += dyv[c][e];
      dbias[c][e] += dx[e];
    }
    *reinterpret_cast<uint4*>(a.dz + off) = pack8(dz);
    if (drop && a.dx) *reinterpret_cast<uint4*>(a.dx + off) = pack8(dx);
  }
}

__global__ __launch_bounds__(512) void ln_bwd_kernel(LnArgs a) {
  extern __shared__ __attribute__((aligned(16))) float lds[];
  const int lane = threadIdx.x & 63, hl = lane & (HL - 1), w = threadIdx.x >> 6;
  const int D = a.D;
  const bool drop = a.thr != 0;
  const uint32_t seed = drop ? hash32(a.seed_ptr[0], a.site) : 0u;
  float dg[CH][8] = {}, db[CH][8] = {}, dbias[CH][8] = {};
  float4 gm[CH][2];
#pragma unroll
  for (int c = 0; c < CH; ++c) {
    const int col = 8 * (hl + HL * c);
    gm[c][0] = *reinterpret_cast<const float4*>(a.gamma + col);
    gm[c][1] = *reinterpret_cast<const float4*>(a.gamma + col + 4);
  }
  const int rows_per_iter = (blockDim.x >> 5);
  for (int row = blockIdx.x * rows_per_iter + (threadIdx.x >> 5); row < a.T; row += gridDim.x * rows_per_iter) {
    const float mean = a.mean[row], rstd = a.rstd[row];
    uint4 dv[CH];
#pragma unroll
    for (int c = 0; c < CH; ++c)
      dv[c] = *reinterpret_cast<const uint4*>(a.dy + (size_t)row * D + 8 * (hl + HL * c));
    float xh[CH][8];
    uint32_t keep;
    ln_load_sum(a, row, hl, drop, seed, xh, keep);
    float dyv[CH][8];
#pragma unroll
    for (int c = 0; c < CH; ++c) unpack8(dv[c], dyv[c]);
    ln_bwd_row(a, row, hl, drop, gm, dyv, xh, keep, mean, rstd, dg, db, dbias);
  }
  float* out = a.part + (size_t)blockIdx.x * 3 * D;
  float (*accs[3])[8] = {dg, db, dbias};
#pragma unroll
  for (int which = 0; which < 3; ++which) {
#pragma unroll
    for (int c = 0; c < CH; ++c)
#pragma unroll
      for (int e = 0; e < 8; ++e) accs[which][c][e] += __shfl_xor(accs[which][c][e], 32, 64);
    if (lane < HL) {
#pragma unroll
      for (int c = 0; c < CH; ++c) {
        float* dst = lds + w * D + 8 * (hl + HL * c);
        *reinterpret_cast<float4*>(dst) =
            make_float4(accs[which][c][0], accs[which][c][1], accs[which][c][2], accs[which][c][3]);
        *reinterpret_cast<float4*>(dst + 4) =
            make_float4(accs[which][c][4], accs[which][c][5], accs[which][c][6], accs[which][c][7]);
      }
    }
    __syncthreads();
    const int nw = blockDim.x >> 6;
    for (int col = threadIdx.x; col < D; col += blockDim.x) {
      float sum = 0.f;
      for (int i = 0; i < nw; ++i) sum += lds[i * D + col];
      out[which * D + col] = sum;
    }
    __syncthreads();
  }
}

struct EmbArgs {
  const void* ids;
  int ids64;
  const bf16_t* word;
  const bf16_t* pos;
  const float* gamma;
  const float* beta;
  bf16_t* y;
  float* mean;
  float* rstd;
  int T, S, D;
  float eps;
  const uint32_t* seed_ptr;
  uint32_t site, thr;
  float dscale;
  const bf16_t* dy;
  float* dz;
  float* part;
  const int* row_map;
  int* ln_epoch;
  unsigned long long* ln_stats;
  long long ln_stats_n;
  long long* sorted;
  long long* perm;
  int sort_blocks;
  unsigned char* now_clear;
  int V;
};

DEV int padded_row(const EmbArgs& a, int row) { return a.row_map ? max(a.row_map[row], 0) : row; }

DEV long load_id(const EmbArgs& a, int t) {
  return a.ids64 ? reinterpret_cast<const long long*>(a.ids)[t] : reinterpret_cast<const int*>(a.ids)[t];
}

template <typename I>
DEV void rank_sort_block(const I* ids, int T, long long* sorted, long long* perm, int* keys, int blk) {
  constexpr int U = 16;
  for (int i0 = threadIdx.x; i0 < T; i0 += 256 * U) {
    I v[U];
#pragma unroll
    for (int u = 0; u < U; ++u) v[u] = ids[min(i0 + u * 256, T - 1)];
#pragma unroll
    for (int u = 0; u < U; ++u)
      if (i0 + u * 256 < T) keys[i0 + u * 256] = (int)v[u];
  }
  __syncthreads();
  const int t = blk * 16 + (threadIdx.x >> 4);
  const int part = threadIdx.x & 15;
  int cnt = 0;
  int my = 0;
  if (t < T) {
    my = keys[t];
    const int T4 = T & ~63;
    for (int j = 4 * part; j < T4; j += 64) {
      const int4 k = *reinterpret_cast<const int4*>(keys + j);
      cnt += (k.x < my) | ((k.x == my) & (j < t));
      cnt += (k.y < my) | ((k.y == my) & (j + 1 < t));
      cnt += (k.z < my) | ((k.z == my) & (j + 2 < t));
      cnt += (k.w < my) | ((k.w == my) & (j + 3 < t));
    }
    for (int j = T4 + part; j < T; j += 16) {
      const int k = keys[j];
      cnt += (k < my) | ((k == my) & (j < t));
    }
  }
  cnt += __shfl_xor(cnt, 1, 64);
  cnt += __shfl_xor(cnt, 2, 64);
  cnt += __shfl_xor(cnt, 4, 64);
  cnt += __shfl_xor(cnt, 8, 64);
  if (t < T && part == 0) {
    sorted[cnt] = my;
    perm[cnt] = t;
  }
}

template <typename I>
__global__ __launch_bounds__(256) void rank_sort_kernel(const I* ids, int T, long long* sorted, long long* perm) {
  extern __shared__ __attribute__((aligned(16))) int keys[];
  rank_sort_block<I>(ids, T, sorted, perm, keys, blockIdx.x);
}

template <int NC>
__global__ __launch_bounds__(256) void emb_fwd_kernel(EmbArgs a) {
  if (a.sort_blocks && (int)blockIdx.x >= (int)gridDim.x - a.sort_blocks) {
    extern __shared__ __attribute__((aligned(16))) int keys[];
    const int blk = blockIdx.x - (gridDim.x - a.sort_blocks);
    if (a.ids64) rank_sort_block<long long>(reinterpret_cast<const long long*>(a.ids), a.T, a.sorted, a.perm, keys, blk);
    else rank_sort_block<int>(reinterpret_cast<const int*>(a.ids), a.T, a.sorted, a.perm, keys, blk);
    return;
  }
  const int lane = threadIdx.x & 63;
  const int row = blockIdx.x * 4 + (threadIdx.x >> 6);
  if (a.ln_epoch && blockIdx.x == 0) {
    const unsigned e = (unsigned)a.ln_epoch[0] + 1u;
    __syncthreads();
    if (a.ln_stats && (e & ((1u << 25) - 1u)) == 0u)
      for (long long i = threadIdx.x; i < a.ln_stats_n; i += 256) a.ln_stats[i] = 0ull;
    if (threadIdx.x == 0) a.ln_epoch[0] = (int)e;
  }
  if (row >= a.T) return;
  const int D = a.D;
  const long id = load_id(a, row);
  const int prow = padded_row(a, row);
  const int s = prow % a.S;
  const bool drop = a.thr != 0;
  const uint32_t seed = drop ? hash32(a.seed_ptr[0], a.site) : 0u;
  float z[NC][4], sum = 0.f;
#pragma unroll
  for (int c = 0; c < NC; ++c) {
    const int col = 4 * (lane + 64 * c);
    const uint2 wv = *reinterpret_cast<const uint2*>(a.word + (size_t)id * D + col);
    const uint2 pv = *reinterpret_cast<const uint2*>(a.pos + (size_t)s * D + col);
    z[c][0] = lo_bf(wv.x) + lo_bf(pv.x); z[c][1] = hi_bf(wv.x) + hi_bf(pv.x);
    z[c][2] = lo_bf(wv.y) + lo_bf(pv.y); z[c][3] = hi_bf(wv.y) + hi_bf(pv.y);
    sum += z[c][0] + z[c][1] + z[c][2] + z[c][3];
  }
  const float mean = wave_sum(sum) / D;
  float q = 0.f;
#pragma unroll
  for (int c = 0; c < NC; ++c)
#pragma unroll
    for (int e = 0; e < 4; ++e) { const float d = z[c][e] - mean; q += d * d; }
  const float rstd = rsqrtf(wave_sum(q) / D + a.eps);
#pragma unroll
  for (int c = 0; c < NC; ++c) {
    const int col = 4 * (lane + 64 * c);
    const size_t off = (size_t)row * D + col;
    const float4 g = *reinterpret_cast<const float4*>(a.gamma + col);
    const float4 b = *reinterpret_cast<const float4*>(a.beta + col);
    float y[4] = {(z[c][0] - mean) * rstd * g.x + b.x, (z[c][1] - mean) * rstd * g.y + b.y,
                  (z[c][2] - mean) * rstd * g.z + b.z, (z[c][3] - mean) * rstd * g.w + b.w};
    if (drop) {
      const uint32_t kb = drop_keep_bits<4>(seed, (uint32_t)((size_t)prow * D + col), a.thr);
#pragma unroll
      for (int e = 0; e < 4; ++e) y[e] = (kb >> e) & 1u ? y[e] * a.dscale : 0.f;
    }
    *reinterpret_cast<uint2*>(a.y + off) = make_uint2(pack_bf2(y[0], y[1]), pack_bf2(y[2], y[3]));
  }
  if (lane == 0) { a.mean[row] = mean; a.rstd[row] = rstd; }
}

template <int NC>
__global__ __launch_bounds__(512) void emb_bwd_kernel(EmbArgs a) {
  extern __shared__ __attribute__((aligned(16))) float lds[];
  const int lane = threadIdx.x & 63, w = threadIdx.x >> 6;
  const int D = a.D;
  const bool drop = a.thr != 0;
  const uint32_t seed = drop ? hash32(a.seed_ptr[0], a.site) : 0u;
  float dg[NC][4] = {}, db[NC][4] = {};
  const int nw = blockDim.x >> 6;
  if (a.now_clear)
    for (int i = blockIdx.x * blockDim.x + threadIdx.x; i < a.V; i += gridDim.x * blockDim.x) a.now_clear[i] = 0;
  for (int row = blockIdx.x * nw + w; row < a.T; row += gridDim.x * nw) {
    const long id = load_id(a, row);
    const int prow = padded_row(a, row);
    const int s = prow % a.S;
    const float mean = a.mean[row], rstd = a.rstd[row];
    float xh[NC][4], gd[NC][4], s1 = 0.f, s2 = 0.f;
#pragma unroll
    for (int c = 0; c < NC; ++c) {
      const int col = 4 * (lane + 64 * c);
      const size_t off = (size_t)row * D + col;
      const uint2 wv = *reinterpret_cast<const uint2*>(a.word + (size_t)id * D + col);
      const uint2 pv = *reinterpret_cast<const uint2*>(a.pos + (size_t)s * D + col);
      const float z[4] = {lo_bf(wv.x) + lo_bf(pv.x), hi_bf(wv.x) + hi_bf(pv.x), lo_bf(wv.y) + lo_bf(pv.y),
                          hi_bf(wv.y) + hi_bf(pv.y)};
      const uint2 dv = *reinterpret_cast<const uint2*>(a.dy + off);
      float d4[4] = {lo_bf(dv.x), hi_bf(dv.x), lo_bf(dv.y), hi_bf(dv.y)};
      if (drop) {
        const uint32_t kb = drop_keep_bits<4>(seed, (uint32_t)((size_t)prow * D + col), a.thr);
#pragma unroll
        for (int e = 0; e < 4; ++e) d4[e] = (kb >> e) & 1u ? d4[e] * a.dscale : 0.f;
      }
      const float4 g = *reinterpret_cast<const float4*>(a.gamma + col);
      const float g4[4] = {g.x, g.y, g.z, g.w};
#pragma unroll
      for (int e = 0; e < 4; ++e) {
        xh[c][e] = (z[e] - mean) * rstd;
        gd[c][e] = g4[e] * d4[e];
        s1 += gd[c][e];
        s2 += gd[c][e] * xh[c][e];
        dg[c][e] += d4[e] * xh[c][e];
        db[c][e] += d4[e];
      }
    }
    s1 = wave_sum(s1) / D;
    s2 = wave_sum(s2) / D;
#pragma unroll
    for (int c = 0; c < NC; ++c) {
      const int col = 4 * (lane + 64 * c);
      float4 o;
      o.x = rstd * (gd[c][0] - s1 - xh[c][0] * s2);
      o.y = rstd * (gd[c][1] - s1 - xh[c][1] * s2);
      o.z = rstd * (gd[c][2] - s1 - xh[c][2] * s2);
      o.w = rstd * (gd[c][3] - s1 - xh[c][3] * s2);
      *reinterpret_cast<float4*>(a.dz + (size_t)row * D + col) = o;
    }
  }
  float* out = a.part + (size_t)blockIdx.x * 3 * D;
  block_colsum<NC>(dg, lds, out, D);
  block_colsum<NC>(db, lds, out + D, D);
}

constexpr int PG_GROUPS = 4, PG_COLS = 64;
DEV void pos_grad_block(int s, int cy, int gy, const float* dz, float* dpos, int B, int S, int D, int accumulate,
                        const int* cu) {
  if (s >= S) {
    for (int col = cy * 256 + threadIdx.x; col < D; col += gy * 256) dpos[(size_t)s * D + col] = 0.f;
    return;
  }
  __shared__ int s_cu[257];
  __shared__ float4 red[PG_GROUPS][PG_COLS];
  if (cu)
    for (int b = threadIdx.x; b <= B && b < 257; b += 256) s_cu[b] = cu[b];
  __syncthreads();
  const int c4 = cy * PG_COLS + (threadIdx.x % PG_COLS), grp = threadIdx.x / PG_COLS;
  const bool live = c4 < D / 4;
  float4 acc = make_float4(0.f, 0.f, 0.f, 0.f);
  for (int b0 = grp; b0 < B; b0 += PG_GROUPS * 8) {
    float4 v[8];
#pragma unroll
    for (int u = 0; u < 8; ++u) {
      const int b = b0 + u * PG_GROUPS;
      long long row = -1;
      if (b < B) {
        if (!cu) row = (long long)b * S + s;
        else if (B < 257 && s < s_cu[b + 1] - s_cu[b]) row = (long long)s_cu[b] + s;
        else if (B >= 257 && s < cu[b + 1] - cu[b]) row = (long long)cu[b] + s;
      }
      v[u] = (row >= 0 && live) ? reinterpret_cast<const float4*>(dz + (size_t)row * D)[c4] : make_float4(0.f, 0.f, 0.f, 0.f);
    }
#pragma unroll
    for (int u = 0; u < 8; ++u) { acc.x += v[u].x; acc.y += v[u].y; acc.z += v[u].z; acc.w += v[u].w; }
  }
  red[grp][threadIdx.x % PG_COLS] = acc;
  __syncthreads();
  if (grp == 0 && live) {
    float4 t = accumulate ? reinterpret_cast<const float4*>(dpos + (size_t)s * D)[c4] : make_float4(0.f, 0.f, 0.f, 0.f);
#pragma unroll
    for (int g = 0; g < PG_GROUPS; ++g) {
      const float4 r = red[g][threadIdx.x];
      t.x += r.x; t.y += r.y; t.z += r.z; t.w += r.w;
    }
    reinterpret_cast<float4*>(dpos + (size_t)s * D)[c4] = t;
  }
}

constexpr int WCH = 16;
DEV void word_row_store(float* dword, long long id, int col, float acc, bool add) {
  float* dst = dword + (size_t)id * 768 + col;
  *dst = add ? *dst + acc : acc;
}

DEV void word_pieces_block(int bx, const long long* sorted, const long long* perm, const float* dz, float* piece,
                          float* dword, int T, int accumulate, unsigned char* now, unsigned char* ever) {
  constexpr int D = 768;
  __shared__ long long sid[WCH + 2];
  __shared__ long long sperm[WCH];
  const int c0 = bx * WCH, c1 = min(T, c0 + WCH), n = c1 - c0;
  if (threadIdx.x < n) {
    sid[threadIdx.x + 1] = sorted[c0 + threadIdx.x];
    sperm[threadIdx.x] = perm[c0 + threadIdx.x];
  }
  if (threadIdx.x == 0) sid[0] = c0 > 0 ? sorted[c0 - 1] : -1;
  if (threadIdx.x == 1) sid[n + 1] = c1 < T ? sorted[c1] : -1;
  __syncthreads();
  float v[3][WCH];
#pragma unroll
  for (int i = 0; i < WCH; ++i)
#pragma unroll
    for (int c = 0; c < 3; ++c) v[c][i] = i < n ? dz[(size_t)sperm[i] * D + threadIdx.x + 256 * c] : 0.f;
  float acc[3] = {0.f, 0.f, 0.f};
  int start = 0;
#pragma unroll
  for (int i = 0; i < WCH; ++i) {
    if (i < n) {
#pragma unroll
      for (int c = 0; c < 3; ++c) acc[c] += v[c][i];
      const long long id = sid[i + 1];
      if (sid[i + 2] != id || i + 1 == n) {
        const bool run_starts_here = sid[start] != id;
        const bool run_ends_here = i + 1 < n || sid[n + 1] != id;
        if (run_starts_here && run_ends_here) {
          const bool add = accumulate && (now ? now[id] != 0 : true);
#pragma unroll
          for (int c = 0; c < 3; ++c) word_row_store(dword, id, threadIdx.x + 256 * c, acc[c], add);
          if (threadIdx.x == 0 && now) { now[id] = 1; ever[id] = 1; }
        } else {
#pragma unroll
          for (int c = 0; c < 3; ++c) piece[(size_t)(c0 + start) * D + threadIdx.x + 256 * c] = acc[c];
        }
        acc[0] = acc[1] = acc[2] = 0.f;
        start = i + 1;
      }
    }
  }
}

DEV void word_combine_block(int bx, const long long* sorted, const float* piece, float* dword, int T, int accumulate,
                           unsigned char* now, unsigned char* ever) {
  constexpr int D = 768;
  const int c0 = bx * WCH, c1 = min(T, c0 + WCH);
  if (c1 >= T || sorted[c1] != sorted[c1 - 1]) return;
  const long long id = sorted[c1 - 1];
  __shared__ int s_cnt, s_end;
  if (threadIdx.x == 0) { s_cnt = 0; s_end = T; }
  __syncthreads();
  if ((int)threadIdx.x < c1 - c0 && sorted[c0 + threadIdx.x] == id) atomicAdd(&s_cnt, 1);
  for (int base = c1;; base += 256) {
    const int j = base + (int)threadIdx.x;
    if (j < T && sorted[j] != id) atomicMin(&s_end, j);
    __syncthreads();
    const bool done = s_end < T || base + 256 >= T;
    __syncthreads();
    if (done) break;
  }
  const int a = c1 - s_cnt;
  if (a == c0 && c0 > 0 && sorted[c0 - 1] == id) return;
  const bool add = accumulate && (now ? now[id] != 0 : true);
  const int npieces = (s_end - c1 + WCH - 1) / WCH;
  for (int col = threadIdx.x; col < D; col += 256) {
    float acc = piece[(size_t)a * D + col];
    for (int p0 = 0; p0 < npieces; p0 += 16) {
      float v[16];
#pragma unroll
      for (int u = 0; u < 16; ++u) v[u] = p0 + u < npieces ? piece[(size_t)(c1 + (p0 + u) * WCH) * D + col] : 0.f;
#pragma unroll
      for (int u = 0; u < 16; ++u) acc += v[u];
    }
    word_row_store(dword, id, col, acc, add);
  }
  if (threadIdx.x == 0 && now) { now[id] = 1; ever[id] = 1; }
}

template <int UNR>
DEV void colsum_block(int bx, int k, const float* part, int nblk, int stride_blk, int D, float* o0, float* o1,
                      float* o2, int accumulate) {
  __shared__ float red[4][64];
  const int lane = threadIdx.x & 63, grp = threadIdx.x >> 6;
  const int j = bx * 64 + lane;
  float* out = k == 0 ? o0 : (k == 1 ? o1 : o2);
  if (!out) return;
  float s = 0.f;
  if (j < D) {
    const float* p = part + k * D + j;
    for (int b0 = grp; b0 < nblk; b0 += 4 * UNR) {
      float v[UNR];
#pragma unroll
      for (int u = 0; u < UNR; ++u) {
        const int b = b0 + 4 * u;
// ... 304 lines not shown
      const uint32_t kb = hdrop ? drop_keep_bits<8>(hseed, (uint32_t)(row * D + col0), h.thr) : 0xffu;
      const float wa[8] = {w0v[c][0].x, w0v[c][0].y, w0v[c][0].z, w0v[c][0].w,
                           w0v[c][1].x, w0v[c][1].y, w0v[c][1].z, w0v[c][1].w};
      const float wb[8] = {w1v[c][0].x, w1v[c][0].y, w1v[c][0].z, w1v[c][0].w,
                           w1v[c][1].x, w1v[c][1].y, w1v[c][1].z, w1v[c][1].w};
#pragma unroll
      for (int e = 0; e < 8; ++e) {
        const float sc = hdrop ? (((kb >> e) & 1u) ? h.dscale : 0.f) : 1.f;
        dyv[c][e] = grad_row ? bf2f(head_dh(d0, d1, wa[e], wb[e], sc)) : 0.f;
      }
    }
    ln_bwd_row(a, row, hl, drop, gm, dyv, xh, keep, mean, rstd, dg, db, dbias);
  }
  float* out = a.part + (size_t)blockIdx.x * 3 * D;
  float (*accs[3])[8] = {dg, db, dbias};
#pragma unroll
  for (int which = 0; which < 3; ++which) {
#pragma unroll
    for (int c = 0; c < CH; ++c)
#pragma unroll
      for (int e = 0; e < 8; ++e) accs[which][c][e] += __shfl_xor(accs[which][c][e], 32, 64);
    if (lane < HL) {
#pragma unroll
      for (int c = 0; c < CH; ++c) {
        float* dst = lds + w * D + 8 * (hl + HL * c);
        *reinterpret_cast<float4*>(dst) =
            make_float4(accs[which][c][0], accs[which][c][1], accs[which][c][2], accs[which][c][3]);
        *reinterpret_cast<float4*>(dst + 4) =
            make_float4(accs[which][c][4], accs[which][c][5], accs[which][c][6], accs[which][c][7]);
      }
    }
    __syncthreads();
    const int nw = blockDim.x >> 6;
    for (int col = threadIdx.x; col < D; col += blockDim.x) {
      float sum = 0.f;
      for (int i = 0; i < nw; ++i) sum += lds[i * D + col];
      out[which * D + col] = sum;
    }
    __syncthreads();
  }
}

constexpr int LN_GRID = 256;
constexpr int LN_BWD_THREADS = 512;
constexpr int LN_BWD_GRID_MAX = 512;
int ln_bwd_threads() { return LN_BWD_THREADS; }

}

extern "C" {

int fd_ln_fwd(const void* x, const void* r, const float* gamma, const float* beta, void* y, float* mean,
              float* rstd, int T, int D, float eps, const uint32_t* seed_ptr, uint32_t site, uint32_t thr,
              float dscale, const int* row_map, hipStream_t st) {
  if (D != 768) return 1;
  LnArgs a{};
  a.x = (const bf16_t*)x; a.r = (const bf16_t*)r; a.gamma = gamma; a.beta = beta; a.y = (bf16_t*)y;
  a.mean = mean; a.rstd = rstd; a.T = T; a.D = D; a.eps = eps;
  a.seed_ptr = seed_ptr; a.site = site; a.thr = thr; a.dscale = dscale; a.row_map = row_map;
  hipLaunchKernelGGL(ln_fwd_kernel, dim3((T + 7) / 8), dim3(256), 0, st, a);
  return 0;
}

int fd_ln_bwd(const void* dy, const void* x, const void* r, const float* gamma, const float* mean,
              const float* rstd, void* dz, void* dx, float* dgamma, float* dbeta, float* dbias, float* work,
              int T, int D, const uint32_t* seed_ptr, uint32_t site, uint32_t thr, float dscale,
              int accumulate, const int* row_map, int defer, int* nblk_out, int zin, hipStream_t st) {
  if (D != 768 || (zin && r)) return 1;
  LnArgs a{};
  a.zin = zin;
  a.dy = (const bf16_t*)dy; a.x = (const bf16_t*)x; a.r = (const bf16_t*)r; a.gamma = gamma;
  a.mean = (float*)mean; a.rstd = (float*)rstd; a.dz = (bf16_t*)dz; a.dx = (bf16_t*)dx; a.part = work;
  a.T = T; a.D = D; a.seed_ptr = seed_ptr; a.site = site; a.thr = thr; a.dscale = dscale; a.row_map = row_map;
  const int thr_n = ln_bwd_threads(), rows = thr_n / 32;
  const int grid = std::min(thr_n == 256 ? LN_BWD_GRID_MAX : LN_GRID, (T + rows - 1) / rows);
  if (nblk_out) *nblk_out = grid;
  hipLaunchKernelGGL(ln_bwd_kernel, dim3(grid), dim3(thr_n), (thr_n / 64) * D * sizeof(float),
                     st, a);
  if (!defer) hipLaunchKernelGGL(colsum_kernel<16>, dim3((D + 63) / 64, 3), dim3(256), 0, st, work, grid, 3 * D, D, dgamma,
                     dbeta, dbias, accumulate);
  return 0;
}


int fd_head_ln_bwd(const void* hidden, int B, int T, int D, const float* W, const float* bias,
                   const uint32_t* seed_ptr, uint32_t hsite, uint32_t hthr, float hdscale, const long long* labels,
                   float* logits, float* loss, float* dlogits, float* row_loss, float* loss_acc, float* dW, float* db,
                   int accumulate, const int* own, const float* tlogits, float kd_T, float kd_alpha, const void* z,
                   const float* gamma, const float* mean, const float* rstd, void* dz, void* dx, float* part,
                   uint32_t site, uint32_t thr, float dscale, const int* row_map, int* nblk_out, hipStream_t st) {
  if (D != 768 || B <= 0 || B > T || B > 1024 || !labels || !row_loss) return 1;
  if (tlogits && !(kd_T > 0.f)) return 3;
  HeadLnArgs x{};
  HeadArgs& h = x.h;
  h.hidden = (const bf16_t*)hidden; h.B = B; h.S = 1; h.D = D; h.W = W; h.bias = bias;
  h.seed_ptr = seed_ptr; h.site = hsite; h.thr = hthr; h.dscale = hdscale; h.labels = labels;
  h.logits = logits; h.loss = loss; h.dlogits = dlogits; h.row_loss = row_loss; h.loss_acc = loss_acc;
  h.dW = dW; h.db = db; h.accumulate = accumulate; h.cls = nullptr; h.T = T; h.own = own;
  h.tlogits = tlogits; h.kd_T = kd_T; h.kd_alpha = kd_alpha;
  LnArgs& a = x.ln;
  a.zin = 1;
  a.x = (const bf16_t*)z; a.gamma = gamma; a.mean = (float*)mean; a.rstd = (float*)rstd;
  a.dz = (bf16_t*)dz; a.dx = (bf16_t*)dx; a.part = part; a.T = T; a.D = D;
  a.seed_ptr = seed_ptr; a.site = site; a.thr = thr; a.dscale = dscale; a.row_map = row_map;
  const int rows = LN_BWD_THREADS / 32;
  x.nlb = std::min(LN_GRID, (T + rows - 1) / rows);
  if (nblk_out) *nblk_out = x.nlb;
  const size_t smem = std::max<size_t>((LN_BWD_THREADS / 64) * D * sizeof(float),
                                       (2 * ((B + 3) & ~3) + 2 * 2 * HLB_GROUPS * HLB_COLS + B) * sizeof(float));
  hipLaunchKernelGGL(head_ln_bwd_kernel, dim3(x.nlb + D / (2 * HLB_COLS)), dim3(LN_BWD_THREADS), smem, st, x);
  return 0;
}

int fd_emb_fwd(const void* ids, int ids64, const void* word, const void* pos, const float* gamma,
               const float* beta, void* y, float* mean, float* rstd, int T, int S, int D, float eps,
               const uint32_t* seed_ptr, uint32_t site, uint32_t thr, float dscale, const int* row_map,
               int* ln_epoch, unsigned long long* ln_stats, long long ln_stats_n, long long* sorted,
               long long* perm, hipStream_t st) {
  if (D != 768) return 1;
  if ((sorted == nullptr) != (perm == nullptr) || (sorted && T > 16384)) return 2;
  if (ln_stats && (!ln_epoch || ln_stats_n <= 0)) return 3;
  EmbArgs a{};
  a.ln_epoch = ln_epoch;
  a.ln_stats = ln_stats;
  a.ln_stats_n = ln_stats_n;
  a.sorted = sorted; a.perm = perm;
  a.sort_blocks = sorted ? (T + 15) / 16 : 0;
  a.ids = ids; a.ids64 = ids64; a.word = (const bf16_t*)word; a.pos = (const bf16_t*)pos; a.gamma = gamma;
  a.beta = beta; a.y = (bf16_t*)y; a.mean = mean; a.rstd = rstd; a.T = T; a.S = S; a.D = D; a.eps = eps;
  a.seed_ptr = seed_ptr; a.site = site; a.thr = thr; a.dscale = dscale; a.row_map = row_map;
  hipLaunchKernelGGL(emb_fwd_kernel<3>, dim3((T + 3) / 4 + a.sort_blocks), dim3(256),
                     sorted ? (size_t)T * sizeof(int) : 0, st, a);
  return 0;
}

int fd_emb_bwd(const void* dy, const void* ids, int ids64, const long long* sorted, const long long* perm,
               const void* word, const void* pos, const float* gamma, const float* mean, const float* rstd,
               float* dword, float* dpos, float* dgamma, float* dbeta, float* dz_buf, float* work, int T, int S,
               int B, int P, int V, int D, const uint32_t* seed_ptr, uint32_t site, uint32_t thr, float dscale,
               int accumulate, unsigned char* now, unsigned char* ever, const int* row_map, const int* cu,
               int ncs, const float* const* cs_parts, float* const* cs_outs, const int* cs_nblk, const int* cs_stride,
               const int* cs_D, const int* cs_nout, const int* cs_acc, hipStream_t st) {
  if (D != 768) return 1;
  if (ncs < 0 || ncs > COLSUM_MAXJ) return 5;
  EmbArgs a{};
  a.dy = (const bf16_t*)dy; a.ids = ids; a.ids64 = ids64; a.word = (const bf16_t*)word;
  a.pos = (const bf16_t*)pos; a.gamma = gamma; a.mean = (float*)mean; a.rstd = (float*)rstd; a.dz = dz_buf;
  a.part = work; a.T = T; a.S = S; a.D = D; a.seed_ptr = seed_ptr; a.site = site; a.thr = thr; a.dscale = dscale;
  a.row_map = row_map;
  a.part = work + (size_t)T * D;
  a.now_clear = !accumulate ? now : nullptr;
  a.V = V;
  const int grid = std::min(LN_GRID, (T + 7) / 8);
  hipLaunchKernelGGL(emb_bwd_kernel<3>, dim3(grid), dim3(LN_BWD_THREADS), (LN_BWD_THREADS / 64) * D * sizeof(float),
                     st, a);
  if (!accumulate && !now) hipMemsetAsync(dword, 0, (size_t)V * D * sizeof(float), st);
  EmbTail t{};
  t.sorted = sorted; t.perm = perm; t.dz = dz_buf; t.piece = work; t.lnpart = a.part;
  t.dword = dword; t.dpos = dpos; t.dgamma = dgamma; t.dbeta = dbeta; t.cu = cu; t.now = now; t.ever = ever;
  t.T = T; t.B = B; t.S = S; t.D = D;
  t.chunks = (T + WCH - 1) / WCH;
  t.pos_gy = (D / 4 + PG_COLS - 1) / PG_COLS;
  t.cs_gx = (D + 63) / 64;
  t.lnblk = grid;
  t.acc_mode = now ? accumulate : 1;
  t.accumulate = accumulate;
  const int pos_rows = !accumulate && P > S ? P : S;
  t.pos_blocks = pos_rows * t.pos_gy;
  int cs_blocks = 0;
  t.cs.n = ncs;
  for (int i = 0; i < ncs; ++i) {
    if (cs_nout[i] < 1 || cs_nout[i] > 3 || cs_D[i] <= 0) return 6;
    t.cs.j[i] = ColsumJob{cs_parts[i], {cs_outs[3 * i], cs_outs[3 * i + 1], cs_outs[3 * i + 2]}, cs_nblk[i],
                          cs_stride[i], cs_D[i], cs_nout[i], cs_acc[i]};
    t.cs.start[i] = cs_blocks;
    cs_blocks += ((cs_D[i] + 63) / 64) * cs_nout[i];
  }
  t.cs.start[ncs] = cs_blocks;
  hipLaunchKernelGGL(emb_tail_a_kernel, dim3(t.chunks + t.pos_blocks + cs_blocks), dim3(256), 0, st, t);
  hipLaunchKernelGGL(emb_tail_b_kernel, dim3(t.chunks + 2 * t.cs_gx), dim3(256), 0, st, t);
  return 0;
}

int fd_rank_sort(const void* ids, int ids64, int T, long long* sorted, long long* perm, hipStream_t st) {
  if (T > 16384) return 1;
  const size_t lds = (size_t)T * sizeof(int);
  if (ids64)
    hipLaunchKernelGGL(rank_sort_kernel<long long>, dim3((T + 15) / 16), dim3(256), lds, st, (const long long*)ids, T,
                       sorted, perm);
  else
    hipLaunchKernelGGL(rank_sort_kernel<int>, dim3((T + 15) / 16), dim3(256), lds, st, (const int*)ids, T, sorted,
                       perm);
  return 0;
}

int fd_colsum_bf16(const void* x, int T, int N, float* out, float* work, int accumulate, int defer, int* nblk_out,
                   hipStream_t st) {
  if (N % 4 != 0) return 1;
  const int rows = 32;
  const int nblk = (T + rows - 1) / rows;
  if (nblk_out) *nblk_out = nblk;
  hipLaunchKernelGGL(colsum_bf16_partial_kernel, dim3(nblk, (N / 4 + 255) / 256), dim3(256), 0, st,
                     (const bf16_t*)x, T, N, rows, work);
  if (!defer)
    hipLaunchKernelGGL(colsum_kernel<16>, dim3((N + 63) / 64, 1), dim3(256), 0, st, work, nblk, N, N, out,
                       (float*)nullptr, (float*)nullptr, accumulate);
  return 0;
}

int fd_colsum_bf16_batched(int n, const void* const* xs, const int* T, const int* N, float* const* parts,
                           hipStream_t st) {
  for (int base = 0; base < n; base += CSB_MAXJ) {
    ColsumBf16Batch cb{};
    cb.n = std::min(CSB_MAXJ, n - base);
    cb.rows = 32;
    int blocks = 0;
    for (int i = 0; i < cb.n; ++i) {
      const int g = base + i;
      if (N[g] <= 0 || N[g] % 4 != 0 || T[g] <= 0) return 1;
      cb.x[i] = (const bf16_t*)xs[g];
      cb.part[i] = parts[g];
      cb.T[i] = T[g];
      cb.N[i] = N[g];
      cb.start[i] = blocks;
      blocks += ((T[g] + 31) / 32) * ((N[g] / 4 + 255) / 256);
    }
    cb.start[cb.n] = blocks;
    hipLaunchKernelGGL(colsum_bf16_partial_batched_kernel, dim3(blocks), dim3(256), 0, st, cb);
  }
  return 0;
}

int fd_colsum_batched(int n, const float* const* parts, float* const* outs , const int* nblk,
                      const int* stride, const int* D, const int* nout, const int* accumulate, hipStream_t st) {
  for (int base = 0; base < n; base += COLSUM_MAXJ) {
    ColsumBatch cb{};
    cb.n = std::min(COLSUM_MAXJ, n - base);
    int blocks = 0;
    for (int i = 0; i < cb.n; ++i) {
      const int g = base + i;
      if (nout[g] < 1 || nout[g] > 3 || D[g] <= 0) return 1;
      cb.j[i] = ColsumJob{parts[g], {outs[3 * g], outs[3 * g + 1], outs[3 * g + 2]}, nblk[g], stride[g], D[g],
                          nout[g], accumulate[g]};
      cb.start[i] = blocks;
      blocks += ((D[g] + 63) / 64) * nout[g];
    }
    cb.start[cb.n] = blocks;
    hipLaunchKernelGGL(colsum_batched_kernel<16>, dim3(blocks), dim3(256), 0, st, cb);
  }
  return 0;
}

}
```

### csrc/kernels/packing.hip

```cpp
#include "common.h"

namespace {

template <typename M, typename I>
__global__ __launch_bounds__(1024) void pack_kernel(const M* mask, const I* ids, int n, int S, int B, int rows,
                                                    int* row_map, int* cu, long long* ids_packed, int* step,
                                                    uint32_t* seed, long long* cls_rows, int* cls_rmap) {
  __shared__ int wsum[16];
  __shared__ int carry_s;
  const int tid = threadIdx.x, lane = tid & 63, w = tid >> 6;
  if (tid == 0) carry_s = 0;
  __syncthreads();
  for (int base = 0; base < n; base += 4096) {
    int f[4], local = 0;
#pragma unroll
    for (int j = 0; j < 4; ++j) {
      const int p = base + 4 * tid + j;
      f[j] = (p < n && mask[p] != 0) ? 1 : 0;
      local += f[j];
    }
    int incl = local;
#pragma unroll
    for (int o = 1; o < 64; o <<= 1) {
      const int v = __shfl_up(incl, o, 64);
      if (lane >= o) incl += v;
    }
    if (lane == 63) wsum[w] = incl;
    __syncthreads();
    int before = 0;
    for (int i = 0; i < w; ++i) before += wsum[i];
    const int carry = carry_s;
    int off = carry + before + incl - local;
#pragma unroll
    for (int j = 0; j < 4; ++j) {
      const int p = base + 4 * tid + j;
      if (p < n && p % S == 0) {
        cu[p / S] = off;
        if (cls_rows) cls_rows[p / S] = off;
      }
      if (f[j]) {
        if (off < rows) {
          row_map[off] = p;
          ids_packed[off] = (long long)ids[p];
        }
        ++off;
      }
    }
    __syncthreads();
    if (tid == 1023) carry_s = off;
    __syncthreads();
  }
  const int total = carry_s;
  if (tid == 0) {
    cu[B] = total;
    if (step) step[0] += 1;
    if (seed) seed[0] += 1;
  }
  const long long id0 = (long long)ids[0];
  for (int r = total + tid; r < rows; r += 1024) {
    row_map[r] = -1;
    ids_packed[r] = id0;
  }
  if (cls_rmap) {
    __syncthreads();
    for (int b = tid; b < B; b += 1024) {
      const int r = cu[b];
      cls_rmap[b] = r < total && r < rows ? max(row_map[r], 0) : 0;
    }
  }
}

__global__ __launch_bounds__(256) void gather_rows2_kernel(const uint4* a, const uint4* b, uint4* oa, uint4* ob,
                                                           const long long* idx, int n, int d16) {
  const long long i = blockIdx.x * 256ll + threadIdx.x;
  if (i >= (long long)n * d16) return;
  const long long r = i / d16, c = i - r * d16;
  const long long src = idx[r] * d16 + c;
  oa[i] = a[src];
  ob[i] = b[src];
}
constexpr int SCATTER_LDS_IDX = 512;
__global__ __launch_bounds__(256) void scatter_rows2_kernel(const uint4* a, const uint4* b, uint4* oa, uint4* ob,
                                                            const long long* idx, int nsrc, int T, int d16) {
  __shared__ long long sidx[SCATTER_LDS_IDX];
  const bool lds = nsrc <= SCATTER_LDS_IDX;
  if (lds)
    for (int k = threadIdx.x; k < nsrc; k += 256) sidx[k] = idx[k];
  __syncthreads();
  const int i = blockIdx.x * 256 + threadIdx.x;
  if (i >= T * d16) return;
  const int r = i / d16, c = i - r * d16;
  int lo = 0, hi = nsrc;
  bool hit;
  if (lds) {
    while (lo < hi) {
      const int mid = (lo + hi) >> 1;
      if (sidx[mid] <= r) lo = mid + 1; else hi = mid;
    }
    hit = lo > 0 && sidx[lo - 1] == r;
  } else {
    while (lo < hi) {
      const int mid = (lo + hi) >> 1;
      if (idx[mid] <= r) lo = mid + 1; else hi = mid;
    }
    hit = lo > 0 && idx[lo - 1] == r;
  }
  const int k = lo - 1;
  if (hit) {
    oa[i] = a[(long long)k * d16 + c];
    ob[i] = b[(long long)k * d16 + c];
  } else {
    oa[i] = make_uint4(0, 0, 0, 0);
    ob[i] = make_uint4(0, 0, 0, 0);
  }
}

}

extern "C" {

int fd_gather_rows2(const void* a, const void* b, void* oa, void* ob, const long long* idx, int n, int d_bytes,
                    hipStream_t st) {
  if (n <= 0 || d_bytes <= 0 || d_bytes % 16) return 1;
  const long long tot = (long long)n * (d_bytes / 16);
  hipLaunchKernelGGL(gather_rows2_kernel, dim3((unsigned)((tot + 255) / 256)), dim3(256), 0, st, (const uint4*)a,
                     (const uint4*)b, (uint4*)oa, (uint4*)ob, idx, n, d_bytes / 16);
  return 0;
}

int fd_scatter_rows2(const void* a, const void* b, void* oa, void* ob, const long long* idx, int nsrc, int T,
                     int d_bytes, hipStream_t st) {
  if (nsrc < 0 || T <= 0 || d_bytes <= 0 || d_bytes % 16) return 1;
  const long long tot = (long long)T * (d_bytes / 16);
  if (tot >= (1ll << 31)) return 1;
  hipLaunchKernelGGL(scatter_rows2_kernel, dim3((unsigned)((tot + 255) / 256)), dim3(256), 0, st, (const uint4*)a,
                     (const uint4*)b, (uint4*)oa, (uint4*)ob, idx, nsrc, T, d_bytes / 16);
  return 0;
}


int fd_pack(const void* mask, int mask_bytes, const void* ids, int ids_bytes, int B, int S, int rows, int* row_map,
            int* cu, long long* ids_packed, int* step, uint32_t* seed, long long* cls_rows, int* cls_rmap,
            hipStream_t st) {
  const int n = B * S;
  if (B <= 0 || S <= 0 || rows <= 0 || n > (1 << 20)) return 1;
#define FD_PACK(MT, IT)                                                                                        \
  hipLaunchKernelGGL((pack_kernel<MT, IT>), dim3(1), dim3(1024), 0, st, (const MT*)mask, (const IT*)ids, n, S, B, \
                     rows, row_map, cu, ids_packed, step, seed, cls_rows, cls_rmap)
  if (mask_bytes == 8 && ids_bytes == 8) FD_PACK(long long, long long);
  else if (mask_bytes == 8 && ids_bytes == 4) FD_PACK(long long, int);
  else if (mask_bytes == 4 && ids_bytes == 8) FD_PACK(int, long long);
  else if (mask_bytes == 4 && ids_bytes == 4) FD_PACK(int, int);
  else if (mask_bytes == 1 && ids_bytes == 8) FD_PACK(unsigned char, long long);
  else if (mask_bytes == 1 && ids_bytes == 4) FD_PACK(unsigned char, int);
  else return 2;
#undef FD_PACK
  return 0;
}

}
```

### detecting_cyber_attacks_with_distilled_large_language_models_in_distributed_networks_amd/engine/graph.py

```python
from __future__ import annotations

import gc
from typing import Callable, Dict, Optional

import torch

from ..data.dataset import PackedTokens, short_batch
from ..ops.graph_split import GRAPH_SPLIT, _Capture, split_point


class no_gc:

    def __enter__(self):
        self.was = gc.isenabled()
        gc.collect()
        gc.disable()
        return self

    def __exit__(self, *exc):
        if self.was:
            gc.enable()
        return False


def contiguous_block(*ts: torch.Tensor) -> Optional[torch.Tensor]:
    t0 = ts[0]
    es = t0.element_size()
    ptr = t0.data_ptr()
    for t in ts:
        if not t.is_contiguous() or t.dtype != t0.dtype or t.device != t0.device or t.data_ptr() != ptr:
            return None
        if t.untyped_storage().data_ptr() != t0.untyped_storage().data_ptr():
            return None
        ptr += t.numel() * es
    n = sum(t.numel() for t in ts)
    return torch.as_strided(t0, (n,), (1,))


def static_block(*ts: torch.Tensor):
    if any(t.dtype != ts[0].dtype for t in ts):
        return [t.clone() for t in ts], None
    flat = torch.empty(sum(t.numel() for t in ts), dtype=ts[0].dtype, device=ts[0].device)
    out, off = [], 0
    for t in ts:
        v = flat[off:off + t.numel()].view(t.shape)
        v.copy_(t)
        out.append(v)
        off += t.numel()
    return out, flat


def key_tokens(key):
    if key[1] is None:
        return None
    return PackedTokens(key[1], 128) if key[2] else int(key[1])


class GraphedTrainStep:
    def __init__(self, step_fn: Callable[..., torch.Tensor], warmup: int = 2, enabled: bool = True,
                 bucket: Optional[Callable[[int, int, int], int]] = None, max_graphs: int = 16):
        self.step_fn = step_fn
        self.warmup = warmup
        self.enabled = enabled and torch.cuda.is_available()
        self.bucket = bucket
        self.max_graphs = max_graphs
        self.calls = 0
        self.graphs: Dict[tuple, tuple] = {}
        self.failed: Optional[str] = None
        self.split = GRAPH_SPLIT
        self._stream: Optional[torch.cuda.Stream] = None

    @property
    def graph(self) -> Optional[torch.cuda.CUDAGraph]:
        return next(iter(self.graphs.values()))[0][0] if self.graphs else None

    @property
    def graph_count(self) -> int:
        return len(next(iter(self.graphs.values()))[0]) if self.graphs else 0

    def _key(self, ids, tokens):
        if tokens is None or self.bucket is None:
            return tuple(ids.shape), None, False
        B, S = ids.shape[0], ids.shape[1]
        return tuple(ids.shape), int(self.bucket(tokens, B, S)), short_batch(tokens, S)

    def __call__(self, ids: torch.Tensor, mask: torch.Tensor, labels: torch.Tensor,
                 tokens: Optional[int] = None) -> torch.Tensor:
        self.calls += 1
        if not self.enabled or self.failed:
            return self.step_fn(ids, mask, labels, tokens)
        key = self._key(ids, tokens)
        hit = self.graphs.get(key)
        prepare = getattr(self.step_fn, "prepare", None)
        if hit is not None:
            if prepare is not None:
                prepare()
            chain, static, loss = hit
            blk = contiguous_block(ids, mask, labels) if static["flat"] is not None else None
            if blk is not None:
                static["flat"].copy_(blk)
            else:
                static["ids"].copy_(ids)
                static["mask"].copy_(mask)
                static["labels"].copy_(labels)
            for g in chain:
                g.replay()
            return loss
        if self.calls <= self.warmup or len(self.graphs) >= self.max_graphs:
            s = torch.cuda.Stream()
            s.wait_stream(torch.cuda.current_stream())
            with torch.cuda.stream(s):
                loss = self.step_fn(ids, mask, labels, tokens)
            torch.cuda.current_stream().wait_stream(s)
            return loss
        (s_ids, s_mask, s_lab), flat = static_block(ids, mask, labels)
        static = {"ids": s_ids, "mask": s_mask, "labels": s_lab, "flat": flat}
        if prepare is not None:
            prepare()
        chain = [torch.cuda.CUDAGraph()]
        try:
            torch.cuda.synchronize()
            with no_gc():
                if not self.split:
                    with torch.cuda.graph(chain[0]):
                        loss = self.step_fn(static["ids"], static["mask"], static["labels"], key_tokens(key))
                else:
                    loss = self._capture_split(chain, static, key_tokens(key))
        except Exception as e:
            self.failed = f"{type(e).__name__}: {e}"
            torch.cuda.synchronize()
            return self.step_fn(ids, mask, labels, tokens)
        self.graphs[key] = (chain, static, loss)
        for g in chain:
            g.replay()
        return loss

    def _capture_split(self, chain, static, tokens):
        if self._stream is None:
            self._stream = torch.cuda.Stream()
        cs, pool = self._stream, torch.cuda.graph_pool_handle()
        torch.cuda.empty_cache()
        cs.wait_stream(torch.cuda.current_stream())
        with torch.cuda.stream(cs):
            _Capture.active = _Capture(chain, pool, self.split)
            chain[0].capture_begin(pool=pool)
            try:
                loss = self.step_fn(static["ids"], static["mask"], static["labels"], tokens)
            finally:
                _Capture.active = None
                chain[-1].capture_end()
        torch.cuda.current_stream().wait_stream(cs)
        return loss
```

### detecting_cyber_attacks_with_distilled_large_language_models_in_distributed_networks_amd/models/distilbert.py

```python
from __future__ import annotations

import math
import os
from dataclasses import dataclass
from typing import Dict, List, Optional, Tuple

import torch
import torch.nn as nn

from ..ops import reference as R
from ..data.dataset import short_batch
from .arena import ParamArena


@dataclass
class DistilBertConfig:
    vocab_size: int = 30522
    dim: int = 768
    n_layers: int = 6
    n_heads: int = 12
    hidden_dim: int = 3072
    max_position_embeddings: int = 512
    dropout: float = 0.1
    attention_dropout: float = 0.1
# ... 248 lines not shown
    def layer_span(self, i: int) -> Tuple[int, int]:
        pre = f"distilbert.transformer.layer.{i}."
        offs = [(o, math.prod(sh)) for nm, (o, sh) in self.arena.offsets.items() if nm.startswith(pre)]
        lo = min(o for o, _ in offs)
        hi = max(o + n for o, n in offs)
        return lo, (hi - lo + 63) // 64 * 64

    def word_embedding_span(self):
        off, shape = self.arena.offsets["distilbert.embeddings.word_embeddings.weight"]
        return off, shape[0], shape[1]

    def dense_grad(self, name: str) -> torch.Tensor:
        g = self.arena.gview(name)
        if name.endswith("word_embeddings.weight") and self.emb_now is not None and self.sparse_word_grad \
                and self.impl == "hip":
            g = g * self.emb_now.to(g.dtype)[:, None]
        return g

    def zero_grad(self, set_to_none: bool = False):
        self.arena.zero_grad(zero_buffer=(self.impl == "torch"))
        for m in self.modules():
            if isinstance(m, _P):
                for n, key in m._arena_keys.items():
                    getattr(m, n).grad = self.arena.gview(key)

    def _param_version(self) -> int:
        return self.arena.master._version + sum(p._version for p in self.parameters())

    def sync_shadow(self, force: bool = False):
        v = self._param_version()
        if force or v != self._synced_version:
            self.arena.sync_shadow()
            self._synced_version = self._param_version()

    def mark_shadow_synced(self):
        self._synced_version = self._param_version()

    def prepare_replay(self):
        self.sync_shadow()

    def _hip_handles(self):
        if self._hip_cache is not None:
            return self._hip_cache
        from ..ops.functional import GradSink
        A = self.arena
        pre = "distilbert."
        tt_name = pre + "embeddings.token_type_embeddings.weight"
        if tt_name in A.offsets:
            pos_tab = torch.empty_like(A.sview(pre + "embeddings.position_embeddings.weight"))
        else:
            pos_tab = A.sview(pre + "embeddings.position_embeddings.weight")
        emb = {
            "word": A.sview(pre + "embeddings.word_embeddings.weight"),
            "pos": pos_tab,
            "ln_w": A.view(pre + "embeddings.LayerNorm.weight"),
            "ln_b": A.view(pre + "embeddings.LayerNorm.bias"),
            "sinks": {
                "word": GradSink(A, pre + "embeddings.word_embeddings.weight"),
                "pos": GradSink(A, pre + "embeddings.position_embeddings.weight"),
                "ln_w": GradSink(A, pre + "embeddings.LayerNorm.weight"),
                "ln_b": GradSink(A, pre + "embeddings.LayerNorm.bias"),
                "flags": (self.emb_now, self.emb_ever) if self.sparse_word_grad else None,
            },
        }
        if tt_name in A.offsets:
            emb["sinks"]["type"] = GradSink(A, tt_name)
        layers = []
        for i in range(self.config.n_layers):
            lp = f"{pre}transformer.layer.{i}."
            qkv_w = [lp + f"attention.{n}_lin.weight" for n in "qkv"]
            qkv_b = [lp + f"attention.{n}_lin.bias" for n in "qkv"]
            names = {
                "o_w": lp + "attention.out_lin.weight", "o_b": lp + "attention.out_lin.bias",
                "ln1_w": lp + "sa_layer_norm.weight", "ln1_b": lp + "sa_layer_norm.bias",
                "l1_w": lp + "ffn.lin1.weight", "l1_b": lp + "ffn.lin1.bias",
                "l2_w": lp + "ffn.lin2.weight", "l2_b": lp + "ffn.lin2.bias",
                "ln2_w": lp + "output_layer_norm.weight", "ln2_b": lp + "output_layer_norm.bias",
            }
            L = {"qkv_w": A.span(qkv_w, "shadow"), "qkv_b": A.span(qkv_b, "master")}
            sinks = {"qkv_w": _SpanSink(A, qkv_w), "qkv_b": _SpanSink(A, qkv_b)}
            for k, nm in names.items():
                L[k] = A.sview(nm) if k.endswith("_w") and not k.startswith("ln") else A.view(nm)
                sinks[k] = GradSink(A, nm)
            L["sinks"] = sinks
            layers.append(L)
        head = {"w": A.view("classifier.weight"), "b": A.view("classifier.bias"),
                "sinks": {"w": GradSink(A, "classifier.weight"), "b": GradSink(A, "classifier.bias")}}
        self._hip_cache = (emb, layers, head)
        return self._hip_cache

    def forward(self, input_ids: torch.Tensor, attention_mask: torch.Tensor,
                tokens: Optional[int] = None) -> torch.Tensor:
        return self._run(input_ids, attention_mask, None, tokens)[1]

    def forward_loss(self, input_ids, attention_mask, labels,
                     tokens: Optional[int] = None, kd=None,
                     unit_backward: bool = False) -> Tuple[torch.Tensor, torch.Tensor]:
        return self._run(input_ids, attention_mask, labels, tokens, kd, unit_backward)

    def _run(self, input_ids, attention_mask, labels, tokens=None, kd=None, unit_backward=False):
        if self.impl == "hip":
            return self._run_hip(input_ids, attention_mask, labels, tokens, kd, unit_backward)
        loss, logits = self._run_torch(input_ids, attention_mask, labels if kd is None else None)
        if kd is not None and labels is not None:
            from .bert import kd_loss
            loss = kd_loss(logits, kd[0], labels, kd[1], kd[2])
        return loss, logits

    def packed_rows(self, tokens: int, B: int, S: int) -> int:
        q = self.pack_quantum
        return min(B * S, (int(tokens) + q - 1) // q * q)

    def _run_hip(self, ids, mask, labels, tokens=None, kd=None, unit_backward=False):
        from ..ops import kernels as K
        from ..ops.functional import EmbeddingFn, HeadFn, LayerFn, RunCtx
        self.sync_shadow()
        B, S = ids.shape
        if S % 64:
            pad = 64 - S % 64
            ids = torch.nn.functional.pad(ids, (0, pad))
            mask = torch.nn.functional.pad(mask, (0, pad))
            S += pad
        emb, layers, head = self._hip_handles()
        cfg = self.config
        if self.TOKEN_TYPES:
            A = self.arena
            emb["pos"].copy_(A.view("distilbert.embeddings.position_embeddings.weight")
                             + A.view("distilbert.embeddings.token_type_embeddings.weight")[0])
        grad = torch.is_grad_enabled()
        packed = tokens is not None and self.unpad and self.packed_rows(tokens, B, S) < B * S
        kbias = self._no_bias() if packed else K.mask_bias(mask)
        rc = RunCtx(B=B, S=S, H=cfg.n_heads, kbias=kbias, seed=self.rng, training=self.training,
                    eps=cfg.layer_norm_eps, p_hidden=cfg.dropout, p_attn=cfg.attention_dropout, p_head=self.dropout.p,
                    on_layer_grads=self.layer_grads_hook if grad else None, group_dw=self.group_dw,
                    loss_acc=getattr(self, "loss_acc", None), unit_backward=bool(unit_backward and grad))
        if grad and self.defer_colsum and self.layer_grads_hook is None:
            rc.colsum_jobs = []
        if grad and self.defer_dw_reduce and self.layer_grads_hook is None:
            rc.dw_jobs = []
        if grad and self.batch_dw and self.layer_grads_hook is None:
            rc.dw_batch = []
            if rc.colsum_jobs is not None and self.batch_colsum:
                rc.colsum_pending = []
        rc.fuse_colsum = self.fuse_colsum
        rc.attn_short = packed and short_batch(tokens, S)
        rc.qkv_ws = [L["qkv_w"] for L in layers]
        rc.remat_gelu = self.remat_gelu
        rc.fuse_ln = self.fuse_ln and cfg.dim % 64 == 0 and cfg.dim <= 2048
        rc.fuse_ln_bwd = rc.fuse_ln and K.ln_fusable(
            1, cfg.dim, concurrent_collectives=bool(grad and getattr(self, "collectives_in_backward", False)))
        if grad and self.training and self.fused_opt is not None and self.layer_grads_hook is None:
            rc.fused_adam = self.fused_opt
        plan = self._prune_plan(rc, layers, grad)
        if grad and self.training:
            lazy = getattr(self, "_lazy_decay_opt", None)
            lazy = lazy() if lazy is not None else None
            if lazy is not None:
                lazy.lazy_catchup(ids)
        incs = [] if packed and self.fold_step_counters else None
        if self.training:
            if grad and self.step_opt is not None:
                self.step_opt._begin(seed=self.rng, defer=incs)
            elif incs is not None:
                incs.append((None, self.rng))
            else:
                K.step_inc(None, self.rng)
        token = self._grad_token if torch.is_grad_enabled() else None
        if packed:
            incs = incs or []
            st_inc = next((a for a, _ in incs if a is not None), None)
            sd_inc = next((b for _, b in incs if b is not None), None)
            if len([a for a, _ in incs if a is not None]) > 1 or len([b for _, b in incs if b is not None]) > 1:
                raise RuntimeError("a counter deferred twice in one forward")
            rc.row_map, rc.cu, ids = K.pack(mask, ids, self.packed_rows(tokens, B, S), step=st_inc, seed=sd_inc,
                                            cls_rows=plan[4] if plan is not None else None,
                                            cls_rmap=plan[5] if plan is not None else None)
        x = EmbeddingFn.apply(token, ids, emb["word"], emb["pos"], emb["ln_w"], emb["ln_b"], emb["sinks"], rc)
        self._setup_prune(rc, plan, len(layers), packed)
        if (labels is not None and grad and self.training and rc.unit_backward and rc.prune_idx >= 0
                and rc.colsum_jobs is not None and rc.head_rows is not None):
            rc.head_req = (head, labels.to(torch.int64), kd)
        for i, L in enumerate(layers):
            x = LayerFn.apply(x, L, rc, i)
        if labels is not None:
            loss, logits = HeadFn.apply(x, head["w"], head["b"], head["sinks"], rc, labels.to(torch.int64), kd)
            return loss, logits
        logits, _ = HeadFn.apply(x, head["w"], head["b"], head["sinks"], rc, None)
        return None, logits

    def _prune_plan(self, rc, layers, grad: bool):
        from ..ops import kernels as K
        B, S, D = rc.B, rc.S, self.config.dim
        Bp = (B + 63) // 64 * 64
        if not (self.prune_last and rc.fuse_ln and layers and K.ln_fusable(Bp, D) and Bp <= rc.B * rc.S):
            return None
        if grad and rc.dw_batch is None:
            return None
        dev = self.arena.device
        key = (B, S, Bp, str(dev))
        caches = self.__dict__.setdefault("_prune_caches", {})
        cache = caches.get(key)
        if cache is None:
            rmap = torch.zeros(Bp, dtype=torch.int32, device=dev)
            rmap[:B] = torch.arange(B, dtype=torch.int32, device=dev) * S
            padded_rows = rmap.to(torch.int64)
            cache = (key, rmap, padded_rows, torch.arange(B, dtype=torch.int32, device=dev),
                     torch.zeros(Bp, dtype=torch.int64, device=dev), torch.zeros(Bp, dtype=torch.int32, device=dev))
            caches[key] = cache
        return cache

    @staticmethod
    def _setup_prune(rc, plan, n_layers: int, packed: bool):
        if plan is None:
            return
        _, rmap, padded_rows, head_rows, packed_rows, packed_rmap = plan
        rc.cls_rows = packed_rows if packed else padded_rows
        rc.cls_rmap = packed_rmap if packed else rmap
        rc.head_rows, rc.prune_idx = head_rows, n_layers - 1

    def _no_bias(self) -> torch.Tensor:
        t = getattr(self, "_nobias", None)
        if t is None or t.device != self.arena.device:
            t = torch.zeros(1, dtype=torch.float32, device=self.arena.device)
            self._nobias = t
        return t

    def _run_torch(self, ids, mask, labels):
        cfg = self.config
        tr = self.training
        counter = None
        if tr:
            self.torch_counter += 1
            counter = self.torch_counter
        B, S = ids.shape
        e = self.distilbert.embeddings
        pos = e.position_embeddings.weight
        if hasattr(e, "token_type_embeddings"):
            pos = pos + e.token_type_embeddings.weight[0]
        x = R.embedding_ref(ids, e.word_embeddings.weight, pos, e.LayerNorm.weight,
                            e.LayerNorm.bias, cfg.layer_norm_eps, cfg.dropout if tr else 0.0, counter, 1)
        for i, blk in enumerate(self.distilbert.transformer.layer):
            a = blk.attention
            P = {
                "qkv_w": torch.cat([a.q_lin.weight, a.k_lin.weight, a.v_lin.weight]),
                "qkv_b": torch.cat([a.q_lin.bias, a.k_lin.bias, a.v_lin.bias]),
                "o_w": a.out_lin.weight, "o_b": a.out_lin.bias,
                "ln1_w": blk.sa_layer_norm.weight, "ln1_b": blk.sa_layer_norm.bias,
                "l1_w": blk.ffn.lin1.weight, "l1_b": blk.ffn.lin1.bias,
                "l2_w": blk.ffn.lin2.weight, "l2_b": blk.ffn.lin2.bias,
                "ln2_w": blk.output_layer_norm.weight, "ln2_b": blk.output_layer_norm.bias,
            }
            x = R.layer_ref(x, P, B, S, cfg.n_heads, mask, cfg.layer_norm_eps,
                            cfg.attention_dropout if tr else 0.0, cfg.dropout if tr else 0.0, counter,
                            16 + 4 * i, 17 + 4 * i)
        logits = R.head_ref(x, B, S, self.classifier.weight, self.classifier.bias, self.dropout.p if tr else 0.0,
                            counter, 2)
        if labels is None:
            return None, logits
        return torch.nn.functional.cross_entropy(logits, labels), logits


class _SpanSink:

    def __init__(self, arena, names):
        self.arena, self.names = arena, list(names)

    @property
    def buf(self):
        return self.arena.span(self.names, "grad")

    def accumulate(self) -> bool:
        acc = False
        for n in self.names:
            acc = self.arena.mark_written(n)
        return acc


def reference_state_dict_keys(cfg: Optional[DistilBertConfig] = None) -> List[str]:
    cfg = cfg or DistilBertConfig()
    keys = ["distilbert.embeddings.word_embeddings.weight", "distilbert.embeddings.position_embeddings.weight",
            "distilbert.embeddings.LayerNorm.weight", "distilbert.embeddings.LayerNorm.bias"]
    for i in range(cfg.n_layers):
        keys += [f"distilbert.transformer.layer.{i}.{k}" for k, _ in LAYER_KEYS]
    return keys + ["classifier.weight", "classifier.bias"]
```

### detecting_cyber_attacks_with_distilled_large_language_models_in_distributed_networks_amd/ops/kernels.py

```python
from __future__ import annotations

from typing import Optional, Tuple

import torch

from ._ext import ext
from .dropout import threshold

D_MODEL = 768
LN_GRID = 256
LN_BWD_PARTS = 512

_WS = {}
_WS_RETIRED = []


def workspace(device, name: str, numel: int, dtype=torch.float32) -> torch.Tensor:
    key = (str(device), name, dtype)
    t = _WS.get(key)
    if t is None or t.numel() < numel:
        if t is not None:
            _WS_RETIRED.append(t)
            numel_alloc = max(numel, t.numel() + t.numel() // 2)
        else:
# ... 69 lines not shown
        if colsum is not None:
            jobs, out, acc = colsum
            cs = workspace(dy.device, f"colsum_job{len(jobs)}", ((M + 31) // 32) * N)
            _, nblk = _splitk(epi, dy, B, dx, aux=gelu_u, aux_out=ao, res=res, colsum=cs, b_mn=bmn)
            jobs.append((cs, [out], nblk, N, N, acc))
            return dx
        _splitk(epi, dy, B, dx, aux=gelu_u, aux_out=ao, res=res, b_mn=bmn)
        return dx
    if colsum is not None:
        jobs, out, acc = colsum
        ws = workspace(dy.device, f"colsum_job{len(jobs)}", ((M + 127) // 128) * N)
        nblk = ext().gemm_colsum(epi, dy, B, dx, gelu_u, res, ws, ao, kind, _pf(prefetch))
        if nblk:
            jobs.append((ws, [out], nblk, N, N, acc))
            return dx
        ext().gemm(kind, epi, dy, B, dx, None, gelu_u, res, None, False, ao, _pf(prefetch))
        _colsum_pass(dx, out, acc, jobs)
        return dx
    ext().gemm(kind, epi, dy, B, dx, None, gelu_u, res, None, False, ao, _pf(prefetch))
    return dx


def linear_dw(dy: torch.Tensor, x: torch.Tensor, out: torch.Tensor, accumulate: bool = False,
              adam=None) -> torch.Tensor:
    M, N = dy.shape[1], x.shape[1]
    ws = workspace(dy.device, "splitk", 8 * M * N)
    st, hp = adam if adam is not None else ([], [])
    ext().gemm_dw(dy, x, out, ws, accumulate, st, hp)
    return out


def linear_dw2(dy0: torch.Tensor, x0: torch.Tensor, out0: torch.Tensor, dy1: torch.Tensor, x1: torch.Tensor,
               out1: torch.Tensor, accumulate: bool = False, adam=None, jobs: Optional[list] = None):
    n = out0.numel() + out1.numel()
    defer = False
    if jobs is not None and adam is None:
        planned = ext().gemm_dw2_splits(dy0.shape[1], x0.shape[1], dy1.shape[1], x1.shape[1], dy0.shape[0])
        defer = planned > 1
    ws = workspace(dy0.device, f"splitk_def{len(jobs)}", planned * n) if defer else \
        workspace(dy0.device, "splitk", 8 * n)
    st, hp = adam if adam is not None else ([], [])
    splits = ext().gemm_dw2(dy0, x0, out0, dy1, x1, out1, ws, accumulate, st, hp, defer)
    if splits:
        s0 = splits * out0.numel()
        jobs.append((ws[:s0], out0, splits, accumulate))
        jobs.append((ws[s0:s0 + splits * out1.numel()], out1, splits, accumulate))


DW_BATCH_MAX = 32


ADAM_IN_DW = _os.environ.get("FD_ADAM_IN_DW", "1") != "0"


DWB_ORDER = int(_os.environ.get("FD_DWB_ORDER", "0"))


def linear_dw_batch(jobs: list, adam=None, cfg: int = -1, opt=None):
    if DWB_ORDER == 1 and len(jobs) <= DW_BATCH_MAX:
        jobs = jobs[::-1]
    starts = list(range(0, len(jobs), DW_BATCH_MAX))
    for i in starts:
        chunk = jobs[i:i + DW_BATCH_MAX]
        outs = [j[2] for j in chunk]
        st, hp = adam(outs) if adam is not None else ([], [])
        bias = [j[4] if len(j) > 4 else None for j in chunk]
        rest = None
        groups = opt is not None and adam is not None and getattr(opt, "grouped_decay", False)
        extra = {"decay": opt.decays_of(outs)} if groups else {}
        if adam is not None and opt is not None and ADAM_IN_DW and i == starts[-1]:
            sums = [b for b in bias if b is not None]
            done0 = len(opt._done)
            opt.mark_done(sums)
            rest = opt.rest_args()
            if rest is None:
                del opt._done[done0:]
            else:
                if groups:
                    extra["bias_decay"] = [opt.decays_of([b])[0] if b is not None else 0.0 for b in bias]
                extra.update(opt.rest_decay_args())
        if any(b is not None for b in bias):
            none = torch.empty(0, dtype=torch.float32, device=outs[0].device)
            bias = [b if b is not None else none for b in bias]
        else:
            bias = []
        ext().gemm_dw_batch([j[0] for j in chunk], [j[1] for j in chunk], outs, [int(j[3]) for j in chunk],
                            st, hp, cfg, bias, *(rest if rest is not None else ([], [])), **extra)


DW_QKV_BIAS = _os.environ.get("FD_DW_QKV_BIAS", "1") != "0"


def dw_flush(jobs: list):
    if jobs:
        ext().splitk_reduce_batched([j[0] for j in jobs], [j[1] for j in jobs], [j[2] for j in jobs],
                                    [int(j[3]) for j in jobs])
        jobs.clear()


def _colsum_pass(x, out, accumulate, jobs):
    return colsum(x, out, accumulate, jobs)


def colsum(x: torch.Tensor, out: torch.Tensor, accumulate: bool = False, jobs: Optional[list] = None) -> torch.Tensor:
    N = out.numel()
    T = x.numel() // N
    if jobs is None:
        ws = workspace(x.device, "colsum", ((T + 31) // 32) * N)
        ext().colsum_bf16(x, out, ws, accumulate, False)
        return out
    ws = workspace(x.device, f"colsum_job{len(jobs)}", ((T + 31) // 32) * N)
    nblk = ext().colsum_bf16(x, out, ws, accumulate, True)
    jobs.append((ws, [out], nblk, N, N, accumulate))
    return out


def gather_rows2(a: torch.Tensor, b: torch.Tensor, idx: torch.Tensor):
    oa = torch.empty(idx.numel(), a.shape[1], dtype=a.dtype, device=a.device)
    ob = torch.empty_like(oa)
    ext().gather_rows2(a, b, oa, ob, idx)
    return oa, ob


def scatter_rows2(a: torch.Tensor, b: torch.Tensor, idx: torch.Tensor, nsrc: int, T: int):
    oa = torch.empty(T, a.shape[1], dtype=a.dtype, device=a.device)
    ob = torch.empty_like(oa)
    ext().scatter_rows2(a, b, oa, ob, idx, nsrc)
    return oa, ob


def colsum_partials_batched(pending: list, jobs: list):
    if not pending:
        return
    xs, parts, ns = [], [], []
    for x, out, acc in pending:
        N = out.numel()
        T = x.numel() // N
        ws = workspace(x.device, f"colsum_job{len(jobs)}", ((T + 31) // 32) * N)
        jobs.append((ws, [out], (T + 31) // 32, N, N, acc))
        xs.append(x)
        parts.append(ws)
        ns.append(N)
    ext().colsum_bf16_batched(xs, parts, ns)
    pending.clear()


def colsum_flush(jobs: list):
    if jobs:
        ext().colsum_batched([j[0] for j in jobs], [j[1] for j in jobs], [j[2] for j in jobs],
                             [j[3] for j in jobs], [j[4] for j in jobs], [int(j[5]) for j in jobs])
        jobs.clear()


def pack(mask: torch.Tensor, ids: torch.Tensor, rows: int, step=None, seed=None, cls_rows=None, cls_rmap=None):
    B = mask.shape[0]
    row_map = torch.empty(rows, dtype=torch.int32, device=mask.device)
    cu = torch.empty(B + 1, dtype=torch.int32, device=mask.device)
    ids_packed = torch.empty(rows, dtype=torch.int64, device=mask.device)
    m = mask if mask.dtype != torch.bool else mask.to(torch.uint8)
    ext().pack(m.contiguous(), ids.contiguous(), row_map, cu, ids_packed, step, seed, cls_rows, cls_rmap)
    return row_map, cu, ids_packed


def mask_bias(mask: torch.Tensor) -> torch.Tensor:
    m = mask.contiguous()
    if m.dtype == torch.bool:
        m = m.to(torch.uint8)
    bias = torch.empty(m.shape, dtype=torch.float32, device=m.device)
    ext().mask_to_bias(m, bias)
    return bias


def attn_keep_bits(B, S, H, p, device, short: bool = False) -> Optional[torch.Tensor]:
    if not threshold(p) or (S > 128 and not short):
        return None
    return torch.empty(B * H * 256, dtype=torch.int64, device=device)


ATTN_CLS_COMPACT = _os.environ.get("FD_ATTN_CLS_COMPACT", "1") != "0"


def attn_cls_compact_ok(S: int, short: bool = False) -> bool:
    return ATTN_CLS_COMPACT and (S <= 128 or short) and _os.environ.get("FD_ATTN_S128", "1") != "0"


def attn_fwd(qkv, kbias, B, S, H, seed, site, p, cu=None, dmask=None, q_live: int = 0, cls=None, short=False):
    rows = qkv.shape[0] if cu is not None else B * S
    ctx = torch.empty(rows, H * 64, dtype=torch.bfloat16, device=qkv.device)
    lse = torch.empty(B, H, S, dtype=torch.float32, device=qkv.device)
    thr, sc = _drop(p)
    if cls is None:
        ext().attn_fwd(qkv, kbias, ctx, lse, B, S, H, seed, site, thr, sc, cu, dmask if thr else None, q_live,
                       split=2 if short and cu is not None else -1)
        return ctx, lse
    x, Bp = cls
    cxc = torch.empty(Bp, H * 64, dtype=torch.bfloat16, device=qkv.device)
    xc = torch.empty_like(cxc)
    ext().attn_fwd(qkv, kbias, ctx, lse, B, S, H, seed, site, thr, sc, cu, dmask if thr else None, q_live,
                   cxc, xc, x, split=2 if short and cu is not None else -1)
    return ctx, lse, cxc, xc


FUSE_QKV_ATTN = int(_os.environ.get("FD_FUSE_QKV_ATTN", "2"))


ATTN_SHORT_FUSED = _os.environ.get("FD_ATTN_SHORT_FUSED", "0") != "0"


def qkv_attn_ok(M: int, D: int, S: int, short: bool = False) -> bool:
    short = short and ATTN_SHORT_FUSED
    return (FUSE_QKV_ATTN and not _SHARED_DEVICE and _os.environ.get("FD_ATTN_S128", "1") != "0"
            and (S in (64, 128) or (short and FUSE_QKV_ATTN == 2 and S % 64 == 0 and S <= 512)) and D % 64 == 0 and M > 0 and M * 3 * D * 2 < 2 ** 31
            and ((M + 127) // 128) * (3 * D // 192) <= QA_FLAGS)


def qkv_attn_fwd(x, w, b, kbias, B, S, H, seed, site, p, cu=None, dmask=None, q_live: int = 0, cls=None,
                 xsite: int = 0, prefetch=None, mode=None, short: bool = False):
    M, D = x.shape[0], H * 64
    qkv = torch.empty(M, 3 * D, dtype=torch.bfloat16, device=x.device)
    rows = M if cu is not None else B * S
    ctx = torch.empty(rows, D, dtype=torch.bfloat16, device=x.device)
    lse = torch.empty(B, H, S, dtype=torch.float32, device=x.device)
    thr, sc = _drop(p)
    stats, cnt, err = _ln_state(x.device, M, D)
    kw = {}
    if cls is not None:
        xr, Bp = cls
        kw = dict(cxc=torch.empty(Bp, D, dtype=torch.bfloat16, device=x.device), xres=xr)
        kw["xc"] = torch.empty_like(kw["cxc"])
    ext().gemm_attn_fwd(x, w, b, qkv, kbias, ctx, lse, B, S, H, seed, site, thr, sc, cu, dmask if thr else None,
                        q_live, stats, cnt, err, int(xsite), prefetch=_pf(prefetch),
                        mode=int(mode if mode is not None else (FUSE_QKV_ATTN or 1)),
                        split=2 if short and cu is not None else -1, **kw)
    if cls is None:
        return qkv, ctx, lse
    return qkv, ctx, lse, kw["cxc"], kw["xc"]


FUSE_ATTN_BWD = int(_os.environ.get("FD_FUSE_ATTN_BWD", "1"))


FUSE_ATTN_BWD_CLS = int(_os.environ.get("FD_FUSE_ATTN_BWD_CLS", "1"))


def attn_bwd_proj_ok(S: int, cls: bool = False, short: bool = False) -> bool:
    short = short and ATTN_SHORT_FUSED
    return (bool(FUSE_ATTN_BWD) and (not cls or bool(FUSE_ATTN_BWD_CLS)) and (S in (64, 128) or short)
            and _os.environ.get("FD_ATTN_S128", "1") != "0")


def _dx_splits(M: int, N: int, K: int) -> int:
    if not _splitk_ok(M, N, K):
        return 1
    tiles = ((M + (63 if M <= 64 else 127)) // (64 if M <= 64 else 128)) * (N // 64)
    nkt, s = K // 64, 1
    for c in range(1, nkt + 1):
        if nkt % c == 0 and tiles * c <= 256 and nkt // c >= 2:
            s = c
    return s


def attn_bwd_proj(qkv, kbias, ctx, lse, dy, w, B, S, H, seed, site, p, cu=None, dmask=None, dresc=None,
                  short: bool = False):
    dqkv = torch.empty_like(qkv)
    thr, sc = _drop(p)
    splits = _dx_splits(dy.shape[0], w.shape[1], dy.shape[1])
    if dresc is None:
        ext().attn_bwd_proj(qkv, kbias, ctx, lse, dy, w, dqkv, B, S, H, seed, site, thr, sc, cu,
                            dmask if thr else None, splits, split=2 if short and cu is not None else -1)
        return dqkv
    dres = torch.empty_like(ctx)
    ext().attn_bwd_proj(qkv, kbias, ctx, lse, dy, w, dqkv, B, S, H, seed, site, thr, sc, cu,
                        dmask if thr else None, splits, dresc.contiguous(), dres,
                        split=2 if short and cu is not None else -1)
    return dqkv, dres


def attn_bwd(qkv, kbias, ctx, lse, dctx, B, S, H, seed, site, p, cu=None, dmask=None, q_live: int = 0, dresc=None,
             short=False):
    dqkv = torch.empty_like(qkv)
    delta = workspace(qkv.device, "attn_delta", B * H * S)
    thr, sc = _drop(p)
    if dresc is None:
        ext().attn_bwd(qkv, kbias, ctx, lse, dctx.contiguous(), delta, dqkv, B, S, H, seed, site, thr, sc, cu,
                       dmask if thr else None, q_live, split=2 if short and cu is not None else -1)
        return dqkv
    dres = torch.empty_like(ctx)
    ext().attn_bwd(qkv, kbias, ctx, lse, dctx.contiguous(), delta, dqkv, B, S, H, seed, site, thr, sc, cu,
                   dmask if thr else None, q_live, dresc.contiguous(), dres, split=2 if short and cu is not None else -1)
    return dqkv, dres


def ln_fwd(x, r, gamma, beta, eps, seed, site, p, row_map=None):
    T = x.numel() // gamma.numel()
    y = torch.empty_like(x)
    mean = torch.empty(T, dtype=torch.float32, device=x.device)
    rstd = torch.empty(T, dtype=torch.float32, device=x.device)
    thr, sc = _drop(p)
    ext().ln_fwd(x, r, gamma, beta, y, mean, rstd, eps, seed, site, thr, sc, row_map if thr else None)
    return y, mean, rstd


def ln_bwd(dy, x, r, gamma, mean, rstd, dgamma, dbeta, dbias, seed, site, p, accumulate=False, row_map=None,
           jobs: Optional[list] = None, zin: bool = False):
    D = gamma.numel()
    T = x.numel() // D
    dz = torch.empty_like(x)
    thr, sc = _drop(p)
    dx = torch.empty_like(x) if thr else None
    key = "ln_part" if jobs is None else f"ln_part_job{len(jobs)}"
    ws = workspace(x.device, key, LN_BWD_PARTS * 3 * D)
    nblk = ext().ln_bwd(dy.contiguous(), x, r, gamma, mean, rstd, dz, dx, dgamma, dbeta, dbias, ws, seed, site, thr,
                        sc, accumulate, row_map if thr else None, jobs is not None, zin)
    if jobs is not None:
# ... 394 lines not shown
```

Before: 693.2 batches/s (sum over clients; bs32 x seq128).

## Read graph inputs through a device descriptor instead of copying into static buffers

```diff
diff --git a/csrc/binding.cpp b/csrc/binding.cpp
--- a/csrc/binding.cpp
+++ b/csrc/binding.cpp
@@ -99,7 +99,8 @@
                      int d_bytes, hipStream_t st);
 int fd_pack(const void* mask, int mask_bytes, const void* ids, int ids_bytes, int B, int S, int rows, int* row_map,
             int* cu, long long* ids_packed, int* step, uint32_t* seed, long long* cls_rows, int* cls_rmap,
-            hipStream_t st);
+            long long* desc, void* wt, hipStream_t st);
+int fd_pack_desc(long long* desc, long long addr, long long stride, hipStream_t st);
 int fd_colsum_bf16_batched(int n, const void* const* xs, const int* T, const int* N, float* const* parts,
                            hipStream_t st);
 int fd_colsum_bf16(const void* x, int T, int N, float* out, float* work, int accumulate, int defer, int* nblk_out,
@@ -694,11 +695,13 @@
 
 void pack(const at::Tensor& mask, const at::Tensor& ids, const at::Tensor& row_map, const at::Tensor& cu,
           const at::Tensor& ids_packed, const c10::optional<at::Tensor>& step, const c10::optional<at::Tensor>& seed,
-          const c10::optional<at::Tensor>& cls_rows, const c10::optional<at::Tensor>& cls_rmap) {
+          const c10::optional<at::Tensor>& cls_rows, const c10::optional<at::Tensor>& cls_rmap,
+          const c10::optional<at::Tensor>& src_desc, const c10::optional<at::Tensor>& static_block) {
   need_opt(cls_rmap, at::kInt, "cls_rmap");
   need_opt(step, at::kInt, "step");
   need_opt(seed, at::kInt, "seed");
   need_opt(cls_rows, at::kLong, "cls_rows");
+  need_opt(src_desc, at::kLong, "src_desc");
   TORCH_CHECK(on_device(mask) && mask.is_contiguous() && on_device(ids) && ids.is_contiguous(), "pack: GPU inputs");
   TORCH_CHECK(mask.dim() == 2 && ids.sizes() == mask.sizes(), "pack: mask and ids must both be [B, S]");
   need(row_map, at::kInt, "row_map");
@@ -708,13 +711,31 @@
   TORCH_CHECK(cu.numel() == B + 1 && ids_packed.numel() == row_map.numel() && row_map.numel() >= 1, "pack: sizes");
   if (cls_rows.has_value() && cls_rows->defined()) TORCH_CHECK(cls_rows->numel() >= B, "pack: cls_rows needs B entries");
   if (cls_rmap.has_value() && cls_rmap->defined()) TORCH_CHECK(cls_rmap->numel() >= B, "pack: cls_rmap needs B entries");
+  const bool has_desc = src_desc.has_value() && src_desc->defined();
+  const bool has_blk = static_block.has_value() && static_block->defined();
+  TORCH_CHECK(has_desc == has_blk, "pack: src_desc and static_block go together");
+  if (has_desc) {
+    TORCH_CHECK(src_desc->numel() == 4, "pack: src_desc is int64 {address, stride, index, ticket}");
+    need(*static_block, ids.scalar_type(), "static_block");
+    TORCH_CHECK(mask.scalar_type() == ids.scalar_type(), "pack: a source descriptor needs ids and mask of one dtype");
+    TORCH_CHECK(static_block->numel() == B * (2 * S + 1), "pack: static_block must hold ids | mask | labels");
+  }
   check_rc(fd_pack(mask.data_ptr(), (int)mask.element_size(), ids.data_ptr(), (int)ids.element_size(), (int)B, (int)S,
                    (int)row_map.numel(), row_map.data_ptr<int>(), cu.data_ptr<int>(),
                    reinterpret_cast<long long*>(ids_packed.data_ptr()), ptr<int>(step), ptr<uint32_t>(seed),
                    cls_rows.has_value() && cls_rows->defined() ? reinterpret_cast<long long*>(cls_rows->data_ptr())
                                                                : nullptr,
-                   ptr<int>(cls_rmap), stream()),
+                   ptr<int>(cls_rmap), ptr<long long>(src_desc), has_blk ? static_block->data_ptr() : nullptr,
+                   stream()),
            "pack");
+}
+
+void pack_desc_set(const at::Tensor& desc, int64_t address, int64_t stride) {
+  need(desc, at::kLong, "src_desc");
+  TORCH_CHECK(desc.numel() == 4, "pack_desc_set: src_desc is int64 {address, stride, index, ticket}");
+  TORCH_CHECK(address != 0 && stride >= 0, "pack_desc_set: address / stride");
+  check_rc(fd_pack_desc(reinterpret_cast<long long*>(desc.data_ptr()), (long long)address, (long long)stride, stream()),
+           "pack_desc_set");
 }
 
 void gather_rows2(const at::Tensor& a, const at::Tensor& b, const at::Tensor& oa, const at::Tensor& ob,
@@ -1620,7 +1641,8 @@
   m.def("scatter_rows2", &scatter_rows2);
   m.def("pack", &pack, py::arg("mask"), py::arg("ids"), py::arg("row_map"), py::arg("cu"), py::arg("ids_packed"),
         py::arg("step") = py::none(), py::arg("seed") = py::none(), py::arg("cls_rows") = py::none(),
-        py::arg("cls_rmap") = py::none());
+        py::arg("cls_rmap") = py::none(), py::arg("src_desc") = py::none(), py::arg("static_block") = py::none());
+  m.def("pack_desc_set", &pack_desc_set, py::arg("desc"), py::arg("address"), py::arg("stride"));
   m.def("comm_load", &comm_load);
   m.def("comm_unique_id", &comm_unique_id);
   m.def("comm_init", &comm_init);
diff --git a/csrc/host_check/binding_host_check.cpp b/csrc/host_check/binding_host_check.cpp
--- a/csrc/host_check/binding_host_check.cpp
+++ b/csrc/host_check/binding_host_check.cpp
@@ -460,9 +460,12 @@
 }
 int fd_pack(const void* mask, int mask_bytes, const void* ids, int ids_bytes, int B, int S, int rows, int* row_map,
             int* cu, long long* ids_packed, int* step, uint32_t* seed, long long* cls_rows, int* cls_rmap,
-            hipStream_t) {
+            long long* desc, void* wt, hipStream_t) {
   hc::opt_span(cls_rmap, (long long)B * 4, "pack cls_rmap");
   ++hc::calls;
+  hc::opt_span(desc, 32, "pack src_desc");
+  hc::opt_span(wt, (long long)B * (2 * S + 1) * ids_bytes, "pack static_block");
+  if ((desc != nullptr) != (wt != nullptr)) hc::violations.push_back("pack: descriptor without its static block");
   hc::opt_span(cls_rows, (long long)B * 8, "pack cls_rows");
   hc::opt_span(step, 4, "pack step");
   hc::opt_span(seed, 4, "pack seed");
@@ -471,6 +474,11 @@
   hc::span(row_map, (long long)rows * 4, "pack row_map");
   hc::span(cu, (long long)(B + 1) * 4, "pack cu");
   hc::span(ids_packed, (long long)rows * 8, "pack ids_packed");
+  return 0;
+}
+int fd_pack_desc(long long* desc, long long, long long, hipStream_t) {
+  ++hc::calls;
+  hc::span(desc, 32, "pack_desc_set desc");
   return 0;
 }
 int fd_colsum_bf16(const void*, int, int, float*, float*, int, int, int* nblk_out, hipStream_t) {
@@ -987,7 +995,7 @@
   {
     auto mask = T_({32, 128}, i64), ids = T_({32, 128}, i64), rm = T_({2688}, i32), cu = T_({33}, i32);
     auto ip = T_({2688}, i64);
-    expect_ok("pack", [&] { pack(mask, ids, rm, cu, ip, none, none, none, none); });
+    expect_ok("pack", [&] { pack(mask, ids, rm, cu, ip, none, none, none, none, none, none); });
     {
       auto ga = T_({300, 768}, bf), gb = T_({300, 768}, bf), go = T_({64, 768}, bf), go2 = T_({64, 768}, bf);
       auto gi = T_({64}, i64);
@@ -998,11 +1006,26 @@
       expect_reject("scatter_rows2 nsrc", [&] { scatter_rows2(go, go2, ga, gb, gi, 65); });
     }
     auto st1 = T_({1}, i32);
-    expect_ok("pack + counters", [&] { pack(mask, ids, rm, cu, ip, st1, st1, none, none); });
+    expect_ok("pack + counters", [&] { pack(mask, ids, rm, cu, ip, st1, st1, none, none, none, none); });
     auto stf = T_({1}, f32);
-    expect_reject("pack counter dtype", [&] { pack(mask, ids, rm, cu, ip, stf, none, none, none); });
+    expect_reject("pack counter dtype", [&] { pack(mask, ids, rm, cu, ip, stf, none, none, none, none, none); });
     auto cu_bad = T_({32}, i32);
-    expect_reject("pack cu", [&] { pack(mask, ids, rm, cu_bad, ip, none, none, none, none); });
+    expect_reject("pack cu", [&] { pack(mask, ids, rm, cu_bad, ip, none, none, none, none, none, none); });
+    auto desc = T_({4}, i64), blk = T_({32 * (2 * 128 + 1)}, i64);
+    expect_ok("pack + descriptor", [&] { pack(mask, ids, rm, cu, ip, st1, st1, none, none, desc, blk); });
+    expect_ok("pack_desc_set", [&] { pack_desc_set(desc, 4096, 32 * (2 * 128 + 1) * 8); });
+    expect_reject("pack descriptor alone", [&] { pack(mask, ids, rm, cu, ip, none, none, none, none, desc, none); });
+    expect_reject("pack static block alone", [&] { pack(mask, ids, rm, cu, ip, none, none, none, none, none, blk); });
+    auto desc3 = T_({3}, i64), desc_i32 = T_({4}, i32), blk_small = T_({32 * 2 * 128}, i64);
+    expect_reject("pack descriptor numel", [&] { pack(mask, ids, rm, cu, ip, none, none, none, none, desc3, blk); });
+    expect_reject("pack descriptor dtype", [&] { pack(mask, ids, rm, cu, ip, none, none, none, none, desc_i32, blk); });
+    expect_reject("pack static block numel",
+                  [&] { pack(mask, ids, rm, cu, ip, none, none, none, none, desc, blk_small); });
+    auto blk_i32 = T_({32 * (2 * 128 + 1)}, i32), mask_i32 = T_({32, 128}, i32);
+    expect_reject("pack static block dtype", [&] { pack(mask, ids, rm, cu, ip, none, none, none, none, desc, blk_i32); });
+    expect_reject("pack descriptor mixed dtypes",
+                  [&] { pack(mask_i32, ids, rm, cu, ip, none, none, none, none, desc, blk); });
+    expect_reject("pack_desc_set null address", [&] { pack_desc_set(desc, 0, 8); });
   }
   if (failures) {
     std::printf("binding host check: %d failure(s)\n", failures);
diff --git a/csrc/kernels/norm.hip b/csrc/kernels/norm.hip
--- a/csrc/kernels/norm.hip
+++ b/csrc/kernels/norm.hip
@@ -123,8 +123,7 @@
   const int lane = threadIdx.x & 63, w = threadIdx.x >> 6, nw = blockDim.x >> 6;
 #pragma unroll
   for (int c = 0; c < NC; ++c)
-#pragma unroll
-    for (int e = 0; e < 4; ++e) lds[w * D + 4 * (lane + 64 * c) + e] = acc[c][e];
+    *reinterpret_cast<float4*>(lds + w * D + 4 * (lane + 64 * c)) = make_float4(acc[c][0], acc[c][1], acc[c][2], acc[c][3]);
   __syncthreads();
   for (int col = threadIdx.x; col < D; col += blockDim.x) {
     float s = 0.f;
@@ -372,7 +371,35 @@
   if (lane == 0) { a.mean[row] = mean; a.rstd[row] = rstd; }
 }
 
+struct EmbBwdHead {
+  long id;
+  int prow;
+  float mean, rstd;
+};
 template <int NC>
+struct EmbBwdRow {
+  uint2 wv[NC], pv[NC], dv[NC];
+};
+template <bool IDS64, bool RMAP>
+DEV void emb_bwd_head(const EmbArgs& a, int row, EmbBwdHead& h) {
+  h.id = IDS64 ? reinterpret_cast<const long long*>(a.ids)[row] : reinterpret_cast<const int*>(a.ids)[row];
+  h.prow = RMAP ? max(a.row_map[row], 0) : row;
+  h.mean = a.mean[row];
+  h.rstd = a.rstd[row];
+}
+template <int NC>
+DEV void emb_bwd_load(const EmbArgs& a, int row, int lane, const EmbBwdHead& h, EmbBwdRow<NC>& r) {
+  const int s = h.prow % a.S;
+#pragma unroll
+  for (int c = 0; c < NC; ++c) {
+    const int col = 4 * (lane + 64 * c);
+    r.wv[c] = *reinterpret_cast<const uint2*>(a.word + (size_t)h.id * a.D + col);
+    r.pv[c] = *reinterpret_cast<const uint2*>(a.pos + (size_t)s * a.D + col);
+    r.dv[c] = *reinterpret_cast<const uint2*>(a.dy + (size_t)row * a.D + col);
+  }
+}
+
+template <int NC, bool IDS64, bool RMAP>
 __global__ __launch_bounds__(512) void emb_bwd_kernel(EmbArgs a) {
   extern __shared__ __attribute__((aligned(16))) float lds[];
   const int lane = threadIdx.x & 63, w = threadIdx.x >> 6;
@@ -383,21 +410,29 @@
   const int nw = blockDim.x >> 6;
   if (a.now_clear)
     for (int i = blockIdx.x * blockDim.x + threadIdx.x; i < a.V; i += gridDim.x * blockDim.x) a.now_clear[i] = 0;
-  for (int row = blockIdx.x * nw + w; row < a.T; row += gridDim.x * nw) {
-    const long id = load_id(a, row);
-    const int prow = padded_row(a, row);
-    const int s = prow % a.S;
-    const float mean = a.mean[row], rstd = a.rstd[row];
+  const int stride = gridDim.x * nw;
+  int row = blockIdx.x * nw + w;
+  EmbBwdHead hc{}, hn{}, hnn{};
+  EmbBwdRow<NC> cur, nxt;
+  if (row < a.T) {
+    emb_bwd_head<IDS64, RMAP>(a, row, hc);
+    emb_bwd_head<IDS64, RMAP>(a, min(row + stride, a.T - 1), hn);
+    emb_bwd_load<NC>(a, row, lane, hc, cur);
+  }
+  for (; row < a.T; row += stride) {
+    const bool more = row + stride < a.T;
+    if (more) emb_bwd_load<NC>(a, row + stride, lane, hn, nxt);
+    emb_bwd_head<IDS64, RMAP>(a, min(row + 2 * stride, a.T - 1), hnn);
+    const int prow = hc.prow;
+    const float mean = hc.mean, rstd = hc.rstd;
     float xh[NC][4], gd[NC][4], s1 = 0.f, s2 = 0.f;
 #pragma unroll
     for (int c = 0; c < NC; ++c) {
       const int col = 4 * (lane + 64 * c);
-      const size_t off = (size_t)row * D + col;
-      const uint2 wv = *reinterpret_cast<const uint2*>(a.word + (size_t)id * D + col);
-      const uint2 pv = *reinterpret_cast<const uint2*>(a.pos + (size_t)s * D + col);
+      const uint2 wv = cur.wv[c], pv = cur.pv[c];
       const float z[4] = {lo_bf(wv.x) + lo_bf(pv.x), hi_bf(wv.x) + hi_bf(pv.x), lo_bf(wv.y) + lo_bf(pv.y),
                           hi_bf(wv.y) + hi_bf(pv.y)};
-      const uint2 dv = *reinterpret_cast<const uint2*>(a.dy + off);
+      const uint2 dv = cur.dv[c];
       float d4[4] = {lo_bf(dv.x), hi_bf(dv.x), lo_bf(dv.y), hi_bf(dv.y)};
       if (drop) {
         const uint32_t kb = drop_keep_bits<4>(seed, (uint32_t)((size_t)prow * D + col), a.thr);
@@ -428,6 +463,9 @@
       o.w = rstd * (gd[c][3] - s1 - xh[c][3] * s2);
       *reinterpret_cast<float4*>(a.dz + (size_t)row * D + col) = o;
     }
+    if (more) cur = nxt;
+    hc = hn;
+    hn = hnn;
   }
   float* out = a.part + (size_t)blockIdx.x * 3 * D;
   block_colsum<NC>(dg, lds, out, D);
@@ -1038,8 +1076,14 @@
   a.now_clear = !accumulate ? now : nullptr;
   a.V = V;
   const int grid = std::min(LN_GRID, (T + 7) / 8);
-  hipLaunchKernelGGL(emb_bwd_kernel<3>, dim3(grid), dim3(LN_BWD_THREADS), (LN_BWD_THREADS / 64) * D * sizeof(float),
-                     st, a);
+  const size_t lds = (LN_BWD_THREADS / 64) * D * sizeof(float);
+#define FD_EMB_BWD(I64, RM) \
+  hipLaunchKernelGGL((emb_bwd_kernel<3, I64, RM>), dim3(grid), dim3(LN_BWD_THREADS), lds, st, a)
+  if (ids64 && row_map) FD_EMB_BWD(true, true);
+  else if (ids64) FD_EMB_BWD(true, false);
+  else if (row_map) FD_EMB_BWD(false, true);
+  else FD_EMB_BWD(false, false);
+#undef FD_EMB_BWD
   if (!accumulate && !now) hipMemsetAsync(dword, 0, (size_t)V * D * sizeof(float), st);
   EmbTail t{};
   t.sorted = sorted; t.perm = perm; t.dz = dz_buf; t.piece = work; t.lnpart = a.part;
diff --git a/csrc/kernels/packing.hip b/csrc/kernels/packing.hip
--- a/csrc/kernels/packing.hip
+++ b/csrc/kernels/packing.hip
@@ -1,14 +1,138 @@
 #include "common.h"
 
+#include <cstdlib>
+
 namespace {
+
+#define RLX_AGENT __ATOMIC_RELAXED, __HIP_MEMORY_SCOPE_AGENT
+
+template <typename M, typename I>
+DEV long long desc_source(long long* desc, int n, const M*& mask, const I*& ids) {
+  const long long addr = __hip_atomic_load(desc, RLX_AGENT), stride = __hip_atomic_load(desc + 1, RLX_AGENT);
+  const long long idx = __hip_atomic_load(desc + 2, RLX_AGENT);
+  const char* src = reinterpret_cast<const char*>(addr + idx * stride);
+  ids = reinterpret_cast<const I*>(src);
+  mask = reinterpret_cast<const M*>(src + (size_t)n * sizeof(I));
+  return idx;
+}
+
+constexpr int PACK_GRID_CHUNKS = 128;
+
+template <typename M, typename I>
+__global__ __launch_bounds__(1024) void pack_grid_kernel(const M* mask, const I* ids, int S, int B, int rows,
+                                                         int* row_map, int* cu, long long* ids_packed, int* step,
+                                                         uint32_t* seed, long long* cls_rows, int* cls_rmap,
+                                                         long long* desc, I* wt) {
+  __shared__ unsigned long long msk_s[PACK_GRID_CHUNKS];
+  __shared__ int pre_s[PACK_GRID_CHUNKS + 1];
+  const int tid = threadIdx.x, lane = tid & 63, w = tid >> 6, b = blockIdx.x;
+  const int CS = (S + 63) >> 6, nch = B * CS, n = B * S;
+  long long idx = 0;
+  if (desc) idx = desc_source(desc, n, mask, ids);
+  const bool thru = wt && (const void*)ids != (const void*)wt;
+  const I id0 = ids[0];
+  I id_first = 0;
+  M m_first = 0;
+  if (tid < S) {
+    id_first = ids[b * S + tid];
+    if (thru) m_first = mask[b * S + tid];
+  }
+#pragma unroll 4
+  for (int j = w; j < nch; j += 16) {
+    const int q = j / CS, s = (j - q * CS) * 64 + lane;
+    const unsigned long long m = __ballot(s < S && mask[q * S + s] != 0);
+    if (lane == 0) msk_s[j] = m;
+  }
+  __syncthreads();
+  if (tid == 1023) {
+    bool last = b == 0;
+    if (desc) {
+      unsigned long long* ticket = reinterpret_cast<unsigned long long*>(desc + 3);
+      last = __hip_atomic_fetch_add(ticket, 1ull, RLX_AGENT) == (unsigned long long)gridDim.x - 1ull;
+      if (last) {
+        __hip_atomic_store(ticket, 0ull, RLX_AGENT);
+        __hip_atomic_store(desc + 2, idx + 1, RLX_AGENT);
+      }
+    }
+    if (last) {
+      if (step) step[0] += 1;
+      if (seed) seed[0] += 1;
+    }
+  }
+  if (w == 0) {
+    int carry = 0;
+    for (int base = 0; base < nch; base += 64) {
+      const int j = base + lane;
+      const int c = j < nch ? __popcll(msk_s[j]) : 0;
+      int incl = c;
+#pragma unroll
+      for (int o = 1; o < 64; o <<= 1) {
+        const int v = __shfl_up(incl, o, 64);
+        if (lane >= o) incl += v;
+      }
+      if (j < nch) pre_s[j] = carry + incl - c;
+      carry += __shfl(incl, 63, 64);
+    }
+    if (lane == 0) pre_s[nch] = carry;
+  }
+  __syncthreads();
+  const int total = pre_s[nch], cub = pre_s[b * CS];
+  if (tid == 0) {
+    cu[b] = cub;
+    if (cls_rows) cls_rows[b] = cub;
+    if (b == B - 1) cu[B] = total;
+    if (thru) wt[2 * n + b] = ids[2 * n + b];
+  }
+  for (int s = tid; s < S; s += 1024) {
+    const int p = b * S + s, j = b * CS + (s >> 6);
+    const I id = s == tid ? id_first : ids[p];
+    if (thru) {
+      wt[p] = id;
+      reinterpret_cast<M*>(wt)[n + p] = s == tid ? m_first : mask[p];
+    }
+    const unsigned long long m = msk_s[j];
+    if ((m >> lane) & 1ull) {
+      const int off = pre_s[j] + __popcll(m & ((1ull << lane) - 1ull));
+      if (off < rows) {
+        row_map[off] = p;
+        ids_packed[off] = (long long)id;
+      }
+    }
+  }
+  for (int r = total + b * 1024 + tid; r < rows; r += B * 1024) {
+    row_map[r] = -1;
+    ids_packed[r] = (long long)id0;
+  }
+  if (cls_rmap && w == 1) {
+    int found = -1;
+    for (int base = b * CS; base < nch && found < 0; base += 64) {
+      const int j = base + lane;
+      const unsigned long long nz = __ballot(j < nch && msk_s[j] != 0ull);
+      if (nz) found = base + __ffsll((long long)nz) - 1;
+    }
+    if (lane == 0) {
+      int v = 0;
+      if (found >= 0 && cub < rows) {
+        const int q = found / CS;
+        v = q * S + (found - q * CS) * 64 + __ffsll((long long)msk_s[found]) - 1;
+      }
+      cls_rmap[b] = v;
+    }
+  }
+}
 
 template <typename M, typename I>
 __global__ __launch_bounds__(1024) void pack_kernel(const M* mask, const I* ids, int n, int S, int B, int rows,
                                                     int* row_map, int* cu, long long* ids_packed, int* step,
-                                                    uint32_t* seed, long long* cls_rows, int* cls_rmap) {
+                                                    uint32_t* seed, long long* cls_rows, int* cls_rmap,
+                                                    long long* desc, I* wt) {
   __shared__ int wsum[16];
   __shared__ int carry_s;
   const int tid = threadIdx.x, lane = tid & 63, w = tid >> 6;
+  long long idx = 0;
+  if (desc) idx = desc_source(desc, n, mask, ids);
+  if (wt && (const void*)ids != (const void*)wt)
+    for (int i = tid; i < 2 * n + B; i += 1024) wt[i] = ids[i];
   if (tid == 0) carry_s = 0;
   __syncthreads();
   for (int base = 0; base < n; base += 4096) {
@@ -55,6 +179,7 @@
     cu[B] = total;
     if (step) step[0] += 1;
     if (seed) seed[0] += 1;
+    if (desc) __hip_atomic_store(desc + 2, idx + 1, RLX_AGENT);
   }
   const long long id0 = (long long)ids[0];
   for (int r = total + tid; r < rows; r += 1024) {
@@ -139,14 +264,36 @@
 }
 
 
+__global__ void pack_desc_kernel(long long* desc, long long addr, long long stride) {
+  desc[0] = addr;
+  desc[1] = stride;
+  desc[2] = 0;
+  desc[3] = 0;
+}
+
+int fd_pack_desc(long long* desc, long long addr, long long stride, hipStream_t st) {
+  if (!desc || !addr || stride < 0) return 1;
+  hipLaunchKernelGGL(pack_desc_kernel, dim3(1), dim3(1), 0, st, desc, addr, stride);
+  return 0;
+}
+
 int fd_pack(const void* mask, int mask_bytes, const void* ids, int ids_bytes, int B, int S, int rows, int* row_map,
             int* cu, long long* ids_packed, int* step, uint32_t* seed, long long* cls_rows, int* cls_rmap,
-            hipStream_t st) {
+            long long* desc, void* wt, hipStream_t st) {
   const int n = B * S;
   if (B <= 0 || S <= 0 || rows <= 0 || n > (1 << 20)) return 1;
-#define FD_PACK(MT, IT)                                                                                        \
-  hipLaunchKernelGGL((pack_kernel<MT, IT>), dim3(1), dim3(1024), 0, st, (const MT*)mask, (const IT*)ids, n, S, B, \
-                     rows, row_map, cu, ids_packed, step, seed, cls_rows, cls_rmap)
+  if ((desc || wt) && (!desc || !wt || mask_bytes != ids_bytes)) return 3;
+  static const bool grid_on = [] { const char* e = getenv("FD_PACK_GRID"); return !e || atoi(e) != 0; }();
+  const bool grid = grid_on && (long long)B * ((S + 63) / 64) <= PACK_GRID_CHUNKS;
+#define FD_PACK(MT, IT)                                                                                          \
+  do {                                                                                                           \
+    if (grid)                                                                                                    \
+      hipLaunchKernelGGL((pack_grid_kernel<MT, IT>), dim3(B), dim3(1024), 0, st, (const MT*)mask, (const IT*)ids, S, \
+                         B, rows, row_map, cu, ids_packed, step, seed, cls_rows, cls_rmap, desc, (IT*)wt);       \
+    else                                                                                                         \
+      hipLaunchKernelGGL((pack_kernel<MT, IT>), dim3(1), dim3(1024), 0, st, (const MT*)mask, (const IT*)ids, n, S, \
+                         B, rows, row_map, cu, ids_packed, step, seed, cls_rows, cls_rmap, desc, (IT*)wt);       \
+  } while (0)
   if (mask_bytes == 8 && ids_bytes == 8) FD_PACK(long long, long long);
   else if (mask_bytes == 8 && ids_bytes == 4) FD_PACK(long long, int);
   else if (mask_bytes == 4 && ids_bytes == 8) FD_PACK(int, long long);
diff --git a/detecting_cyber_attacks_with_distilled_large_language_models_in_distributed_networks_amd/engine/graph.py b/detecting_cyber_attacks_with_distilled_large_language_models_in_distributed_networks_amd/engine/graph.py
--- a/detecting_cyber_attacks_with_distilled_large_language_models_in_distributed_networks_amd/engine/graph.py
+++ b/detecting_cyber_attacks_with_distilled_large_language_models_in_distributed_networks_amd/engine/graph.py
@@ -7,6 +7,7 @@
 
 from ..data.dataset import PackedTokens, short_batch
 from ..ops.graph_split import GRAPH_SPLIT, _Capture, split_point
+from ..ops.input_source import INPUT_CURSOR, InputCursor, InputSource
 
 
 class no_gc:
@@ -69,6 +70,12 @@
         self.failed: Optional[str] = None
         self.split = GRAPH_SPLIT
         self._stream: Optional[torch.cuda.Stream] = None
+        self.input_cursor = INPUT_CURSOR
+        self.cursor = InputCursor()
+        self.desc: Optional[torch.Tensor] = None
+        self.replays_no_copy = 0
+        self.desc_rewrites = 0
+        self.replays_copied = 0
 
     @property
     def graph(self) -> Optional[torch.cuda.CUDAGraph]:
@@ -96,13 +103,7 @@
             if prepare is not None:
                 prepare()
             chain, static, loss = hit
-            blk = contiguous_block(ids, mask, labels) if static["flat"] is not None else None
-            if blk is not None:
-                static["flat"].copy_(blk)
-            else:
-                static["ids"].copy_(ids)
-                static["mask"].copy_(mask)
-                static["labels"].copy_(labels)
+            self._feed(static, ids, mask, labels)
             for g in chain:
                 g.replay()
             return loss
@@ -114,12 +115,18 @@
             torch.cuda.current_stream().wait_stream(s)
             return loss
         (s_ids, s_mask, s_lab), flat = static_block(ids, mask, labels)
-        static = {"ids": s_ids, "mask": s_mask, "labels": s_lab, "flat": flat}
+        static = {"ids": s_ids, "mask": s_mask, "labels": s_lab, "flat": flat, "cursor": False}
         if prepare is not None:
             prepare()
         chain = [torch.cuda.CUDAGraph()]
+        offer = None
+        if self.input_cursor and flat is not None:
+            if self.desc is None:
+                self.desc = torch.zeros(4, dtype=torch.int64, device=flat.device)
+            offer = InputSource(self.desc, flat, s_ids, s_mask)
         try:
             torch.cuda.synchronize()
+            InputSource.active = offer
             with no_gc():
                 if not self.split:
                     with torch.cuda.graph(chain[0]):
@@ -127,13 +134,44 @@
                 else:
                     loss = self._capture_split(chain, static, key_tokens(key))
         except Exception as e:
+            InputSource.active = None
             self.failed = f"{type(e).__name__}: {e}"
             torch.cuda.synchronize()
             return self.step_fn(ids, mask, labels, tokens)
+        InputSource.active = None
+        static["cursor"] = offer is not None and offer.taken == 1
         self.graphs[key] = (chain, static, loss)
+        self._feed(static, ids, mask, labels)
         for g in chain:
             g.replay()
         return loss
+
+    def _feed(self, static, ids, mask, labels):
+        flat = static["flat"]
+        blk = contiguous_block(ids, mask, labels) if flat is not None else None
+        if blk is not None and (blk.dtype != flat.dtype or blk.numel() != flat.numel()):
+            blk = None
+        if static["cursor"]:
+            if blk is not None:
+                write = self.cursor.advance(blk.data_ptr(), blk.numel() * blk.element_size())
+                if write is None:
+                    self.replays_no_copy += 1
+            else:
+                static["ids"].copy_(ids)
+                static["mask"].copy_(mask)
+                static["labels"].copy_(labels)
+                self.replays_copied += 1
+                write = self.cursor.pin(flat.data_ptr())
+            if write is not None:
+                from ..ops import kernels as K
+                K.pack_desc_set(self.desc, *write)
+                self.desc_rewrites += 1
+        elif blk is not None:
+            flat.copy_(blk)
+        else:
+            static["ids"].copy_(ids)
+            static["mask"].copy_(mask)
+            static["labels"].copy_(labels)
 
     def _capture_split(self, chain, static, tokens):
         if self._stream is None:
diff --git a/detecting_cyber_attacks_with_distilled_large_language_models_in_distributed_networks_amd/models/distilbert.py b/detecting_cyber_attacks_with_distilled_large_language_models_in_distributed_networks_amd/models/distilbert.py
--- a/detecting_cyber_attacks_with_distilled_large_language_models_in_distributed_networks_amd/models/distilbert.py
+++ b/detecting_cyber_attacks_with_distilled_large_language_models_in_distributed_networks_amd/models/distilbert.py
@@ -424,6 +424,7 @@
         if grad and self.training and self.fused_opt is not None and self.layer_grads_hook is None:
             rc.fused_adam = self.fused_opt
         plan = self._prune_plan(rc, layers, grad)
+        lazy = None
         if grad and self.training:
             lazy = getattr(self, "_lazy_decay_opt", None)
             lazy = lazy() if lazy is not None else None
@@ -444,9 +445,14 @@
             sd_inc = next((b for _, b in incs if b is not None), None)
             if len([a for a, _ in incs if a is not None]) > 1 or len([b for _, b in incs if b is not None]) > 1:
                 raise RuntimeError("a counter deferred twice in one forward")
+            src = None
+            if grad and self.training and kd is None and not (lazy is not None and lazy.lazy_active()):
+                from ..ops.input_source import InputSource
+                src = InputSource.take(ids, mask)
             rc.row_map, rc.cu, ids = K.pack(mask, ids, self.packed_rows(tokens, B, S), step=st_inc, seed=sd_inc,
                                             cls_rows=plan[4] if plan is not None else None,
-                                            cls_rmap=plan[5] if plan is not None else None)
+                                            cls_rmap=plan[5] if plan is not None else None,
+                                            src_desc=src[0] if src else None, static_block=src[1] if src else None)
         x = EmbeddingFn.apply(token, ids, emb["word"], emb["pos"], emb["ln_w"], emb["ln_b"], emb["sinks"], rc)
         self._setup_prune(rc, plan, len(layers), packed)
         if (labels is not None and grad and self.training and rc.unit_backward and rc.prune_idx >= 0
diff --git a/detecting_cyber_attacks_with_distilled_large_language_models_in_distributed_networks_amd/ops/input_source.py b/detecting_cyber_attacks_with_distilled_large_language_models_in_distributed_networks_amd/ops/input_source.py
--- /dev/null
+++ b/detecting_cyber_attacks_with_distilled_large_language_models_in_distributed_networks_amd/ops/input_source.py
@@ -0,0 +1,53 @@
+from __future__ import annotations
+
+import os
+from typing import Optional, Tuple
+
+INPUT_CURSOR = os.environ.get("FD_INPUT_CURSOR", "1") != "0"
+
+
+class InputCursor:
+
+    def __init__(self):
+        self.base = 0
+        self.stride = 0
+        self.index = 0
+        self.valid = False
+
+    @property
+    def next(self) -> Optional[int]:
+        return self.base + self.index * self.stride if self.valid else None
+
+    def advance(self, address: int, nbytes: int) -> Optional[Tuple[int, int]]:
+        if self.valid and self.stride == nbytes and self.base + self.index * self.stride == address:
+            self.index += 1
+            return None
+        self.base, self.stride, self.index, self.valid = int(address), int(nbytes), 1, True
+        return self.base, self.stride
+
+    def pin(self, address: int) -> Optional[Tuple[int, int]]:
+        if self.valid and self.stride == 0 and self.base == address:
+            self.index += 1
+            return None
+        self.base, self.stride, self.index, self.valid = int(address), 0, 1, True
+        return self.base, 0
+
+
+class InputSource:
+
+    active: Optional["InputSource"] = None
+
+    def __init__(self, desc, flat, ids, mask):
+        self.desc, self.flat, self.ids, self.mask = desc, flat, ids, mask
+        self.taken = 0
+
+    @classmethod
+    def take(cls, ids, mask):
+        src = cls.active
+        if src is None or src.taken:
+            return None
+        for t, s in ((ids, src.ids), (mask, src.mask)):
+            if t.data_ptr() != s.data_ptr() or t.shape != s.shape or t.dtype != s.dtype or not t.is_contiguous():
+                return None
+        src.taken += 1
+        return src.desc, src.flat
diff --git a/detecting_cyber_attacks_with_distilled_large_language_models_in_distributed_networks_amd/ops/kernels.py b/detecting_cyber_attacks_with_distilled_large_language_models_in_distributed_networks_amd/ops/kernels.py
--- a/detecting_cyber_attacks_with_distilled_large_language_models_in_distributed_networks_amd/ops/kernels.py
+++ b/detecting_cyber_attacks_with_distilled_large_language_models_in_distributed_networks_amd/ops/kernels.py
@@ -245,14 +245,20 @@
         jobs.clear()
 
 
-def pack(mask: torch.Tensor, ids: torch.Tensor, rows: int, step=None, seed=None, cls_rows=None, cls_rmap=None):
+def pack(mask: torch.Tensor, ids: torch.Tensor, rows: int, step=None, seed=None, cls_rows=None, cls_rmap=None,
+         src_desc=None, static_block=None):
     B = mask.shape[0]
     row_map = torch.empty(rows, dtype=torch.int32, device=mask.device)
     cu = torch.empty(B + 1, dtype=torch.int32, device=mask.device)
     ids_packed = torch.empty(rows, dtype=torch.int64, device=mask.device)
     m = mask if mask.dtype != torch.bool else mask.to(torch.uint8)
-    ext().pack(m.contiguous(), ids.contiguous(), row_map, cu, ids_packed, step, seed, cls_rows, cls_rmap)
+    ext().pack(m.contiguous(), ids.contiguous(), row_map, cu, ids_packed, step, seed, cls_rows, cls_rmap,
+               src_desc, static_block)
     return row_map, cu, ids_packed
+
+
+def pack_desc_set(desc: torch.Tensor, address: int, stride: int):
+    ext().pack_desc_set(desc, int(address), int(stride))
 
 
 def mask_bias(mask: torch.Tensor) -> torch.Tensor:
```

Result: no change. 693.0 batches/s (sum over clients; bs32 x seq128), median of 6 (-0.0%).
